# nubcico/EAV

Measured on AMD Instinct MI355X. Metric: EEGNet training samples/sec (fwd+CE+bwd+Adam), whole job, higher is better.
Workload: dtype f32; 1 GPU; EEGNet_tor(5, Chans=30, Samples=10000, kernLength=300, F1=8, D=8, F2=64) train step on x[64,1,30,10000] fp32 per GPU (BASELINE.json configs[1]); global_batch=64, per_gpu_batch=64, parallelism=dp1

## Files before the change

eav_amd/_lib.py:

```python
from __future__ import annotations

import ctypes as C
import os

_HERE = os.path.dirname(os.path.abspath(__file__))
LIB_PATH = os.environ.get("EAV_LIB_PATH") or os.path.join(_HERE, "libeav_hip.so")


class EavError(RuntimeError):
    pass


_p = C.c_void_p
_i = C.c_int
_i64 = C.c_int64
_u64 = C.c_uint64
_f = C.c_float
_d = C.c_double

SIGNATURES = {
    "eav_reduce_partials": [_p, _i, _i64, _i, _f, _p, _p],
    "eav_bn_finalize": [_p, _i, _i, _d, _p, _p, _p, _p, _i, _f, _f, _p, _p, _p, _p, _p],
    "eav_bn_bwd_finalize": [_p, _i, _i, _d, _i, _p, _p, _p, _p, _p],
    "eav_reduce_and_bn_bwd_finalize": [_p, _i, _i64, _i, _p, _p, _i, _i, _d, _i, _p, _p, _p, _p, _p, _i, _i, _d, _i, _p, _p, _p,
                                       _p, _p],
    "eav_renorm_rows": [_p, _i, _i, _f, _p],
    "eav_renorm_rows2": [_p, _i, _i, _p, _i, _i, _f, _p],
    "eav_eegnet_step_prologue": [_p, _p, _p, _p, _p, _p, _p, _p],
    "eav_eegnet_fir_fwd": [_p, _p, _p, _p, _i, _i, _i, _i, _p],
    "eav_eegnet_fir_wgrad": [_p, _p, _p, _p, _p, _i, _i, _i, _i, _p],
    "eav_eegnet_fir_fwd_indexed": [_p, _p, _p, _p, _p, _i, _i, _i, _i, _p],
    "eav_eegnet_fir_fwd_fft": [_p, _p, _p, _p, _p, _i, _i, _i, _i, _p],
    "eav_eegnet_fir_wgrad_fft": [_p, _p, _p, _p, _p, _p, _p, _i, _i, _i, _i, _p],
    "eav_eegnet_fir_wgrad_indexed": [_p, _p, _p, _p, _p, _p, _i, _i, _i, _i, _p],
    "eav_eegnet_dw_fwd": [_p, _p, _p, _p, _p, _i, _i, _i, _p],
    "eav_eegnet_dw_fwd_pool_eval": [_p, _p, _p, _p, _p, _p, _p, _i, _i, _i, _p],
    "eav_eegnet_dw_bwd": [_p, _p, _p, _p, _p, _p, _p, _i, _i, _i, _p],
    "eav_eegnet_dw_bwd_fused": [_p, _p, _p, _p, _p, _p, _p, _p, _p, _i, _i, _i, _f, _u64, _p, _p, _p],
    "eav_eegnet_dw_bwd_fused_eval": [_p, _p, _p, _p, _p, _p, _p, _p, _p, _p, _i, _i, _i, _f, _u64, _p, _p, _p],
    "eav_bn_elu_pool_fwd": [_p, _p, _p, _i, _i, _i, _i, _f, _u64, _p, _p, _p],
    "eav_bn_elu_pool_bwd_reduce": [_p, _p, _p, _p, _i, _i, _i, _i, _f, _u64, _p, _p, _p],
    "eav_bn_elu_pool_bwd_apply": [_p, _p, _p, _p, _p, _i, _i, _i, _i, _f, _u64, _p, _p, _p],
    "eav_bn_elu_pool_bwd_eval": [_p, _p, _p, _p, _p, _i, _i, _i, _i, _f, _u64, _p, _p, _p],
    "eav_conv64_prep_weights": [_p, _p, _p, _p],
    "eav_conv64_fwd": [_p, _p, _p, _p, _i, _i, _i, _p],
    "eav_conv64_wgrad": [_p, _p, _p, _i, _i, _i, _p],
    "eav_conv64_fft_fwd": [_p, _p, _p, _p, _p, _i, _i, _i, _p],
    "eav_conv64_fft_wgrad": [_p, _p, _p, _i, _i, _p],
    "eav_dense_softmax_fwd": [_p, _p, _p, _p, _p, _i, _i, _i, _p],
    "eav_dense_softmax_bwd": [_p, _p, _p, _p, _p, _p, _p, _i, _i, _i, _p],
    "eav_ce_fwd_bwd": [_p, _p, _p, _p, _p, _p, _i, _i, _p],
    "eav_scale_by_scalar": [_p, _p, _i64, _p],
    "eav_adam_step": [_p, _p, _p, _p, _i64, _f, _f, _f, _f, _f, _i64, _i, _p, _p],
    "eav_counter_inc": [_p, _p],
    "eav_counter_inc4": [_p, _p, _p, _p, _p],
    "eav_step_begin": [_p, _p, _p, _p, _p, _p, _p, _p, _i, _p],
    "eav_gather_rows": [_p, _p, _p, _i, _i64, _p],
    "eav_gather_i64": [_p, _p, _p, _i, _p],
    "eav_gemm_f32": [_p, _p, _p, _i, _i, _i, _i, _i, _i, _i, _i, _i, _i, _i64, _i64, _i64, _i64, _i64, _i64, _f, _p,
                     _i, _p, _p, _i, _i, _p],
    "eav_gemm_f32_splitk": [_p, _p, _p, _p, _i, _i, _i, _i, _i, _i, _i, _p],
    "eav_sp_absmax": [_p, _i, _i, _i64, _p, _p],
    "eav_sp_convert": [_p, _i, _i, _i64, _p, _p, _p, _p],
    "eav_sp_convert_gelu": [_p, _i, _i, _i64, _p, _p, _p, _p],
    "eav_sp_convert_colsum": [_p, _i, _i, _i64, _p, _p, _p, _p, _p],
    "eav_layernorm_fwd_amax": [_p, _p, _p, _p, _p, _p, _i, _i, _f, _p, _p],
    "eav_layernorm_bwd_amax": [_p, _p, _p, _p, _p, _p, _i, _p, _i, _i, _p, _p],
    "eav_layernorm_bwd_planes": [_p, _p, _p, _p, _p, _p, _i, _p, _i, _i, _p, _p, _p, _p, _p, _p],
    "eav_layernorm_bwd_bound": [_p, _p, _p, _p, _p, _i, _i, _p, _p],
    "eav_gelu_bwd_amax": [_p, _p, _i64, _p, _p],
    "eav_gemm_sp": [_p, _p, _p, _p, _p, _i, _i, _i, _i, _i, _i64, _i64, _f, _p, _i, _p, _p, _i, _i, _p, _p],
    "eav_gemm_sp_x1": [_p, _p, _p, _p, _p, _i, _i, _i, _i, _i, _i64, _i64, _f, _p, _i, _p, _p, _i, _i, _p, _p],
    "eav_gemm_sp_splitk_x1": [_p, _p, _p, _p, _p, _p, _i, _i, _i, _i, _p],
    "eav_gemm_sp_splitk_x2": [_p, _p, _p, _p, _p, _p, _i, _i, _i, _i, _p],
    "eav_gemm_sp_ex": [_p, _p, _p, _p, _p, _i, _i, _i, _i, _i, _i64, _i64, _f, _p, _i, _p, _p, _i, _i, _p, _p, _p, _p, _i, _p],
    "eav_colnorm_max": [_p, _i, _i, _i64, _p, _p],
    "eav_norm_max_multi": [_p, _i, _i, _p],
    "eav_sp_bound_scale": [_p, _p, _p, _f, _p],
    "eav_gemm_sp_planes": [_p, _p, _p, _p, _p, _i, _i, _i, _i, _i, _i64, _i64, _f, _p, _i, _p, _p, _i, _i, _p, _p, _p, _p],
    "eav_layernorm_fwd_planes": [_p, _p, _p, _p, _p, _p, _p, _p, _i, _i, _f, _p],
    "eav_sp_refresh_planes": [_p, _i, _i, _i, _p],
    "eav_rownorm_max": [_p, _i, _i, _i64, _p, _p],
    "eav_tf_forward_scales": [_p, _i64, _i, _i, _i, _i, _i, _i, _i, _i, _p, _p, _i64, _i, _i, _i, _p],
    "eav_gemm_sp_splitk": [_p, _p, _p, _p, _p, _p, _i, _i, _i, _i, _p],
    "eav_attn_sp_prep": [_p, _p, _p, _p, _i, _i, _i, _i, C.c_uint, _p],
    "eav_attn_fwd_sp": [_p, _p, _p, _p, _p, _p, _i, _i, _i, _i, _f, _p],
    "eav_tf_forward_scales_qkv": [_p, _i64, _i, _i, _i, _i, _i, _i, _i, _i, _i, _p, _p, _p, _i64, _i, _i, _i, _i, _p],
    "eav_attn_fwd_sp_planes": [_p, _p, _p, _p, _p, _p, _p, _p, _i, _i, _i, _i, _f, _p],
    "eav_attn_bwd_sp": [_p, _p, _p, _p, _p, _p, _p, _p, _p, _p, _p, _p, _p, _i, _i, _i, _i, _f, _p],
    "eav_attn_bwd_sp_planes": [_p, _p, _p, _p, _p, _p, _p, _p, _p, _p, _p, _p, _p, _p, _p, _p, _p, _p, _i, _i, _i, _i, _f, _p],
    "eav_attn_dqkv_bound": [_p, _p, _p, _i, _f, _p],
    "eav_attn_fwd": [_p, _p, _p, _i, _i, _i, _i, _f, _p],
    "eav_attn_bwd": [_p, _p, _p, _p, _p, _p, _i, _i, _i, _i, _f, _p],
    "eav_attn_fwd_dropout": [_p, _p, _p, _i, _i, _i, _i, _f, _f, _u64, _p, _p, _p],
    "eav_attn_bwd_dropout": [_p, _p, _p, _p, _p, _p, _i, _i, _i, _i, _f, _f, _u64, _p, _p, _p],
    "eav_attn_fwd_sp_dropout": [_p, _p, _p, _p, _p, _i, _i, _i, _i, _f, _f, _u64, _p, _p, _p],
    "eav_attn_bwd_sp_dropout": [_p, _p, _p, _p, _p, _p, _p, _p, _p, _p, _p, _i, _i, _i, _i, _f, _f, _u64, _p, _p, _p],
    "eav_tf_dropout_mask": [_p, _i64, _f, _u64, _p, _p],
    "eav_tf_dropout_add": [_p, _p, _p, _i64, _f, _u64, _p, _p, _p],
    "eav_softmax_dropout_fwd": [_p, _p, _i64, _i, _i, _f, _u64, _p, _p, _p],
    "eav_softmax_dropout_bwd": [_p, _p, _p, _i64, _i, _i, _f, _u64, _p, _p, _p],
    "eav_layernorm_fwd": [_p, _p, _p, _p, _p, _p, _i, _i, _f, _p],
    "eav_layernorm_bwd": [_p, _p, _p, _p, _p, _p, _i, _p, _i, _i, _p],
    "eav_softmax_fwd": [_p, _i64, _i, _i, _p],
    "eav_softmax_bwd": [_p, _p, _i64, _i, _i, _p],
    "eav_gelu_bwd": [_p, _p, _i64, _p],
    "eav_colsum": [_p, _p, _i, _i, _i, _p],
    "eav_im2col": [_p, _p, _i, _i, _i, _i, _i, _i, _i, _i, _p],
    "eav_embed_finish": [_p, _p, _p, _p, _i, _i, _i, _i, _p],
    "eav_embed_bwd": [_p, _p, _p, _i, _i, _i, _i, _p],
    "eav_token_rows": [_p, _p, _i, _i, _i, _i, _i, _p],
    "eav_pair_mean": [_p, _p, _i, _i, _i, _p],
    "eav_ast_fbank": [_p, _p, _p, _p, _p, _i, _i, _i, _i, _d, _d, _f, _f, _p],
    "eav_decimate_fir_f64": [_p, _p, _p, _i, _i64, _i64, _i, _i, _i, _p],
    "eav_sosfilt_f64": [_p, _p, _p, _p, _p, _p, _p, _i, _i64, _i, _i, _p],
    "eav_eegnet_block1_infer": [_p, _p, _p, _p, _p, _p, _p, _i, _i, _i, _i, _p],
    "eav_tconv_fwd": [_p, _p, _p, _p, _i, _i, _i, _i, _i, _p],
    "eav_tconv_wgrad": [_p, _p, _p, _p, _p, _i, _i, _i, _i, _i, _p],
    "eav_spatial_fwd": [_p, _p, _p, _p, _p, _i, _i, _i, _i, _i, _i, _p],
    "eav_spatial_bwd": [_p, _p, _p, _p, _p, _p, _p, _i, _i, _i, _i, _i, _i, _p],
    "eav_dconv_fwd": [_p, _p, _p, _p, _i, _i, _i, _i, _i, _i, _p],
    "eav_dconv_wgrad": [_p, _p, _p, _i, _i, _i, _i, _i, _p],
    "eav_sepconv_fwd": [_p, _p, _p, _p, _p, _p, _i, _i, _i, _i, _i, _p],
    "eav_pointwise_bwd": [_p, _p, _p, _p, _p, _i, _i, _i, _i, _p],
    "eav_dwt_bwd": [_p, _p, _p, _p, _p, _i, _i, _i, _i, _p],
    "eav_shallow_embed_fwd": [_p, _p, _p, _i, _p, _p, _i, _i, _i, _i, _i, _p],
    "eav_shallow_embed_bwd": [_p, _p, _p, _p, _p, _p, _i, _i, _i, _i, _i, _p],
    "eav_relu_dropout": [_p, _i64, _f, _u64, _p, _p, _p],
    "eav_relu_dropout_bwd": [_p, _p, _i64, _f, _p],
    "eav_dropout_add": [_p, _p, _p, _i64, _f, _u64, _p, _p, _p],
    "eav_add_strided": [_p, _i, _p, _i, _p, _i, _i64, _i, _p],
    "eav_colstats": [_p, _p, _i64, _i, _i, _p],
    "eav_sqpool_log_fwd": [_p, _p, _p, _p, _i, _i, _i, _i, _i, _i, _f, _f, _f, _u64, _p, _p, _p],
    "eav_sqpool_log_bwd": [_p, _p, _p, _p, _p, _p, _i, _i, _i, _i, _i, _i, _f, _f, _f, _u64, _p, _p, _p],
    "eav_bn_rows_bwd": [_p, _p, _p, _p, _i64, _i, _p],
    "eav_peak_mfma_f32": [_p, _i, _i, _p],
    "eav_peak_copy": [_p, _p, _i64, _p],
    "eav_peak_mfma_f16": [_p, _i, _i, _p],
    "eav_peak_copy_variant": [_p, _p, _i64, _i, _i, _p],
    "eav_peak_l2_read": [_p, _i, _i, _i, _i, _p, _p],
    "eav_resize_normalize_u8": [_p, _p, _p, _p, _p, _p, _i, _i, _i, _i, _i, _i, _i, _i, _d, _p, _p, _p],
    "eav_audio_conv5_fwd": [_p, _p, _p, _p, _p, _i, _i, _i, _i, _i, _i, _f, _u64, _p, _p, _p],
    "eav_audio_conv5_dgrad": [_p, _p, _f, _p, _p, _p, _p, _f, _i, _i, _i, _i, _i, _i, _p],
    "eav_audio_conv5_wgrad": [_p, _p, _f, _p, _p, _i, _i, _i, _i, _i, _i, _p],
    "eav_video_conv_relayout": [_p, _p, _p, _i, _i, _i, _p],
    "eav_video_conv_fwd": [_p, _p, _p, _i, _i, _i, _i, _i, _i, _i, _i, _i, _i, _i, _i, _p],
    "eav_video_conv_dgrad": [_p, _p, _p, _p, _i, _i, _i, _i, _i, _i, _i, _i, _i, _i, _i, _p],
    "eav_video_conv_wgrad": [_p, _p, _p, _i, _i, _i, _i, _i, _i, _i, _i, _i, _i, _i, _i, _i, _p],
    "eav_video_bn_stats": [_p, _p, _i64, _i, _p],
    "eav_video_bn_apply": [_p, _p, _p, _p, _p, _p, _p, _i64, _i, _i, _p],
    "eav_video_bn_bwd": [_p, _p, _p, _p, _p, _p, _i64, _i, _p],
    "eav_video_maxpool_fwd": [_p, _p, _p, _i, _i, _i, _i, _i, _i, _i, _i, _i, _p],
    "eav_video_maxpool_bwd": [_p, _p, _p, _i, _i, _i, _i, _i, _i, _i, _i, _i, _p],
    "eav_video_head_pool": [_p, _p, _p, _i, _i, _i, _p],
    "eav_video_head_scale_pool": [_p, _p, _p, _p, _i, _i, _i, _p],
    "eav_video_head_attn_bwd": [_p, _p, _p, _i, _i, _i, _p],
    "eav_video_head_feat_bwd": [_p, _p, _p, _p, _p, _i, _i, _i, _p],
    "eav_video_counters_inc": [_p, _i, _p],
}
PLAIN = {
    "eav_abi_version": ([], _i),
    "eav_last_error": ([], C.c_char_p),
    "eav_eegnet_fir_fwd_nparts": ([_i, _i, _i], _i),
    "eav_eegnet_fir_fwd_fft_nparts": ([_i, _i, _i], _i),
    "eav_eegnet_fir_wgrad_fft_ws_floats": ([_i, _i, _i], _i64),
    "eav_eegnet_fir_fft_max_taps": ([], _i),
    "eav_eegnet_fir_wgrad_nparts": ([_i, _i, _i], _i),
    "eav_conv64_ntiles": ([_i], _i),
    "eav_tconv_fwd_nparts": ([_i, _i, _i, _i, _i], _i),
    "eav_shallow_embed_nparts": ([_i, _i], _i),
    "eav_colstats_nparts": ([_i64], _i),
    "eav_tconv_wgrad_nparts": ([_i, _i, _i, _i, _i], _i),
    "eav_spatial_nparts": ([_i, _i], _i),
    "eav_dconv_fwd_nparts": ([_i, _i], _i),
    "eav_sepconv_fwd_nparts": ([_i, _i], _i),
    "eav_pointwise_bwd_nparts": ([_i, _i], _i),
    "eav_conv64_fwd_nparts": ([_i, _i], _i),
    "eav_conv64_fft_nparts": ([_i, _i], _i),
    "eav_conv64_fft_ws_floats": ([_i, _i], _i64),
    "eav_conv64_wgrad_nparts": ([_i, _i], _i),
    "eav_layernorm_bwd_nparts": ([_i], _i),
    "eav_gemm_f32_splitk_plan": ([_i, _i, _i], _i),
    "eav_colsum_nparts": ([_i], _i),
    "eav_sp_kpad": ([_i], _i),
    "eav_sp_convert_colsum_nparts": ([_i], _i),
    "eav_attn_sp_npad": ([_i], _i),
    "eav_gemm_sp_splitk_plan": ([_i, _i, _i], _i),
    "eav_audio_wgrad_nparts": ([_i, _i, _i, _i], _i),
    "eav_video_wgrad_nparts": ([_i, _i, _i, _i64], _i),
    "eav_video_bn_nparts": ([_i64], _i),
}

EXPORTS = sorted(list(SIGNATURES) + list(PLAIN))

TUNING = {"eav_gemm_sp_set_tile": [_i], "eav_gemm_sp_set_splitk": [_i], "eav_sp_set_convert_blocks": [_i],
          "eav_attn_sp_set_nw4_above": [_i]}

EXTRAS_PATH = os.path.join(_HERE, "libeav_extras.so")
EXTRAS = {
    "eav_gemm_bf16": [_p, _p, _p, _i, _i, _i, _i, _i, _i, _i, _i, _i, _i, _i64, _i64, _i64, _i64, _i64, _i64, _f, _p,
                      _i, _p, _p, _i, _i, _p],
    "eav_gemm_bf16_splitk": [_p, _p, _p, _p, _i, _i, _i, _i, _i, _i, _i, _p],
}
_extras = None

_lib = None


def load():
    global _lib
    if _lib is not None:
        return _lib
    if not os.path.exists(LIB_PATH):
        raise EavError(
            f"{LIB_PATH} is missing - the HIP extension is not built. Run "
            "`python -c 'import __graft_entry__ as g; g.build()'` (or `make -C eav_amd/csrc`). "
            "There is no CPU fallback.")
    import torch
    lib = C.CDLL(LIB_PATH)
    for name, args in SIGNATURES.items():
        fn = getattr(lib, name)
        fn.argtypes = args
        fn.restype = _i
    for name, (args, res) in PLAIN.items():
        fn = getattr(lib, name)
        fn.argtypes = args
        fn.restype = res
    for name, args in TUNING.items():
        fn = getattr(lib, name)
        fn.argtypes = args
        fn.restype = _i
    _lib = lib
    return lib


def ptr(t):
    return None if t is None else t.data_ptr()


def stream_ptr():
    import torch
    return torch.cuda.current_stream().cuda_stream


def have_extras():
    return os.path.exists(EXTRAS_PATH)


def load_extras():
    global _extras
    if _extras is None:
        if not have_extras():
            raise EavError(f"{EXTRAS_PATH} is missing - {sorted(EXTRAS)} are comparison-only kernels: build them with "
                           "`make -C eav_amd/csrc BENCH_EXTRAS=1`")
        load()
        lib = C.CDLL(EXTRAS_PATH)
        for name, args in EXTRAS.items():
            fn = getattr(lib, name)
            fn.argtypes = args
            fn.restype = _i
        lib.eav_last_error.restype = C.c_char_p
        _extras = lib
    return _extras


TRACE = None


def call(name, *args):
    lib = load_extras() if name in EXTRAS else load()
    if TRACE is not None:
        import torch
        a, b = torch.cuda.Event(enable_timing=True), torch.cuda.Event(enable_timing=True)
        a.record()
        rc = getattr(lib, name)(*args)
        b.record()
        TRACE.setdefault(name, []).append((a, b))
    else:
        rc = getattr(lib, name)(*args)
    if rc != 0:
        raise EavError(f"{name} failed ({rc}): {lib.eav_last_error().decode()}")


def plain(name, *args):
    return getattr(load(), name)(*args)
```

eav_amd/csrc/eav_common.hip:

```cpp
#include "eav_common.h"

#include <stdarg.h>
#include <stdio.h>

#include "../../include/eav_hip.h"

static thread_local char g_err[512] = "";

int eav_set_error(int code, const char* fmt, ...) {
  va_list ap;
  va_start(ap, fmt);
  vsnprintf(g_err, sizeof(g_err), fmt, ap);
  va_end(ap);
  return code;
}

extern "C" const char* eav_last_error(void) { return g_err; }
extern "C" int eav_abi_version(void) { return EAV_ABI_VERSION; }

__global__ __launch_bounds__(256) void reduce_partials_kernel(const float* __restrict__ part, int nparts,
                                                              int64_t stride, int n, float scale,
                                                              float* __restrict__ out) {
  __shared__ double sh[16][17];
  const int ol = threadIdx.x & 15, pl = threadIdx.x >> 4;
  const int i = blockIdx.x * 16 + ol;
  double s = 0.0;
  if (i < n) {
    const float* src = part + i;
    int p = pl;
    for (; p + 48 < nparts; p += 64) {
      float a = src[(int64_t)p * stride], b = src[(int64_t)(p + 16) * stride];
      float c = src[(int64_t)(p + 32) * stride], d = src[(int64_t)(p + 48) * stride];
      s += ((double)a + (double)b) + ((double)c + (double)d);
    }
    for (; p < nparts; p += 16) s += (double)src[(int64_t)p * stride];
  }
  sh[pl][ol] = s;
  __syncthreads();
  if (threadIdx.x < 16 && i < n) {
    double t = 0.0;
#pragma unroll
    for (int k = 0; k < 16; ++k) t += sh[k][threadIdx.x];
    out[i] = (float)(t * (double)scale);
  }
}

template <int CL>
__device__ __forceinline__ void reduce_partials_vec_body(const float* __restrict__ part, int nparts, int64_t stride, int n4,
                                                         float scale, float* __restrict__ out, int bid) {
  constexpr int PL = 256 / CL;
  __shared__ double sh[PL][4 * CL + 1];
  const int cl = threadIdx.x % CL, pl = threadIdx.x / CL;
  const int c4 = bid * CL + cl;
  double a = 0.0, b = 0.0, c = 0.0, d = 0.0;
  if (c4 < n4) {
    const float* src = part + 4 * (int64_t)c4;
    int p = pl;
    for (; p + 3 * PL < nparts; p += 4 * PL) {
      const float4 v0 = *reinterpret_cast<const float4*>(src + (int64_t)p * stride);
      const float4 v1 = *reinterpret_cast<const float4*>(src + (int64_t)(p + PL) * stride);
      const float4 v2 = *reinterpret_cast<const float4*>(src + (int64_t)(p + 2 * PL) * stride);
      const float4 v3 = *reinterpret_cast<const float4*>(src + (int64_t)(p + 3 * PL) * stride);
      a += ((double)v0.x + (double)v1.x) + ((double)v2.x + (double)v3.x);
      b += ((double)v0.y + (double)v1.y) + ((double)v2.y + (double)v3.y);
      c += ((double)v0.z + (double)v1.z) + ((double)v2.z + (double)v3.z);
      d += ((double)v0.w + (double)v1.w) + ((double)v2.w + (double)v3.w);
    }
    for (; p < nparts; p += PL) {
      const float4 v = *reinterpret_cast<const float4*>(src + (int64_t)p * stride);
      a += (double)v.x; b += (double)v.y; c += (double)v.z; d += (double)v.w;
    }
  }
  sh[pl][4 * cl] = a; sh[pl][4 * cl + 1] = b; sh[pl][4 * cl + 2] = c; sh[pl][4 * cl + 3] = d;
  __syncthreads();
  if (threadIdx.x < 4 * CL && 4 * bid * CL + threadIdx.x < 4 * n4) {
    double t = 0.0;
#pragma unroll
    for (int k = 0; k < PL; ++k) t += sh[k][threadIdx.x];
    out[4 * (int64_t)bid * CL + threadIdx.x] = (float)(t * (double)scale);
  }
}

template <int CL>
__global__ __launch_bounds__(256) void reduce_partials_vec_kernel(const float* __restrict__ part, int nparts,
                                                                  int64_t stride, int n4, float scale,
                                                                  float* __restrict__ out) {
  reduce_partials_vec_body<CL>(part, nparts, stride, n4, scale, out, blockIdx.x);
}

extern "C" int eav_reduce_partials(const float* part, int nparts, int64_t stride, int n, float scale, float* out,
                                   void* stream) {
  EAV_REQUIRE(part && out && nparts > 0 && n > 0, "eav_reduce_partials: bad arguments");
  const bool vec = (n & 3) == 0 && (stride & 3) == 0 && (((uintptr_t)part | (uintptr_t)out) & 15) == 0;
  if (vec && n >= 8192)
    hipLaunchKernelGGL(reduce_partials_vec_kernel<16>, dim3(cdiv(n / 4, 16)), dim3(256), 0, (hipStream_t)stream, part,
                       nparts, stride, n / 4, scale, out);
  else if (vec)
    hipLaunchKernelGGL(reduce_partials_vec_kernel<8>, dim3(cdiv(n / 4, 8)), dim3(256), 0, (hipStream_t)stream, part,
                       nparts, stride, n / 4, scale, out);
  else
    hipLaunchKernelGGL(reduce_partials_kernel, dim3(cdiv(n, 16)), dim3(256), 0, (hipStream_t)stream, part, nparts,
                       stride, n, scale, out);
  EAV_CHECK_LAUNCH("eav_reduce_partials");
  return EAV_OK;
}

__global__ void bn_finalize_kernel(const float* __restrict__ part, int nparts, int nch, double count,
                                   const float* __restrict__ gamma, const float* __restrict__ beta,
                                   float* __restrict__ rmean, float* __restrict__ rvar, int training, float momentum,
                                   float eps, float* __restrict__ mean_o, float* __restrict__ invstd_o,
                                   float* __restrict__ scale_o, float* __restrict__ shift_o) {
  const int c = blockIdx.x;
  __shared__ double shs[256], shq[256];
  float mean, var;
  if (training) {
    double s = 0.0, q = 0.0;
    for (int p = threadIdx.x; p < nparts; p += 256) {
      s += (double)part[(int64_t)p * 2 * nch + c];
      q += (double)part[(int64_t)p * 2 * nch + nch + c];
    }
    shs[threadIdx.x] = s;
    shq[threadIdx.x] = q;
    __syncthreads();
    for (int o = 128; o > 0; o >>= 1) {
      if (threadIdx.x < o) {
        shs[threadIdx.x] += shs[threadIdx.x + o];
        shq[threadIdx.x] += shq[threadIdx.x + o];
      }
      __syncthreads();
    }
    if (threadIdx.x != 0) return;
    s = shs[0];
    q = shq[0];
    double m = s / count;
    double v = q / count - m * m;
    if (v < 0.0) v = 0.0;
    mean = (float)m;
    var = (float)v;
    double unb = count > 1.0 ? v * (count / (count - 1.0)) : v;
    rmean[c] = (1.f - momentum) * rmean[c] + momentum * mean;
    rvar[c] = (1.f - momentum) * rvar[c] + momentum * (float)unb;
  } else {
    if (threadIdx.x != 0) return;
    mean = rmean[c];
    var = rvar[c];
  }
  float invstd = 1.0f / sqrtf(var + eps);
  float sc = gamma[c] * invstd;
  mean_o[c] = mean;
  invstd_o[c] = invstd;
  scale_o[c] = sc;
  shift_o[c] = beta[c] - mean * sc;
}

extern "C" int eav_bn_finalize(const float* part, int nparts, int nch, double count, const float* gamma,
                               const float* beta, float* running_mean, float* running_var, int training,
                               float momentum, float eps, float* mean, float* invstd, float* scale, float* shift,
                               void* stream) {
  EAV_REQUIRE(nch > 0 && gamma && beta && running_mean && running_var && mean && invstd && scale && shift,
              "eav_bn_finalize: bad arguments");
  EAV_REQUIRE(!training || (part && nparts > 0 && count > 0), "eav_bn_finalize: training needs partials");
  hipLaunchKernelGGL(bn_finalize_kernel, dim3(nch), dim3(256), 0, (hipStream_t)stream, part, nparts, nch,
                     count, gamma, beta, running_mean, running_var, training, momentum, eps, mean, invstd, scale,
                     shift);
  EAV_CHECK_LAUNCH("eav_bn_finalize");
  return EAV_OK;
}

__device__ __forceinline__ void bn_bwd_finalize_body(const float* __restrict__ part, int nparts, int nch, double count,
                                                     int training, float* __restrict__ dgamma, float* __restrict__ dbeta,
                                                     float* __restrict__ m1, float* __restrict__ m2, int c) {
  __shared__ double shs[256], shq[256];
  double s = 0.0, q = 0.0;
  for (int p = threadIdx.x; p < nparts; p += 256) {
    s += (double)part[(int64_t)p * 2 * nch + c];
    q += (double)part[(int64_t)p * 2 * nch + nch + c];
  }
  shs[threadIdx.x] = s;
  shq[threadIdx.x] = q;
  __syncthreads();
  for (int o = 128; o > 0; o >>= 1) {
    if (threadIdx.x < o) {
      shs[threadIdx.x] += shs[threadIdx.x + o];
      shq[threadIdx.x] += shq[threadIdx.x + o];
    }
    __syncthreads();
  }
  if (threadIdx.x != 0) return;
  s = shs[0];
  q = shq[0];
  dbeta[c] = (float)s;
  dgamma[c] = (float)q;
  m1[c] = training ? (float)(s / count) : 0.f;
  m2[c] = training ? (float)(q / count) : 0.f;
}

__global__ void bn_bwd_finalize_kernel(const float* __restrict__ part, int nparts, int nch, double count,
                                       int training, float* __restrict__ dgamma, float* __restrict__ dbeta,
                                       float* __restrict__ m1, float* __restrict__ m2) {
  bn_bwd_finalize_body(part, nparts, nch, count, training, dgamma, dbeta, m1, m2, blockIdx.x);
}

struct BnBwdJob {
  const float* part;
  int nparts, nch, training;
  double count;
  float *dgamma, *dbeta, *m1, *m2;
};

__global__ __launch_bounds__(256) void finish_jobs_kernel(const float* __restrict__ part, int nparts, int64_t stride, int n4,
                                                          float scale, float* __restrict__ out, int nred, BnBwdJob a,
                                                          BnBwdJob b) {
  const int bid = blockIdx.x;
  if (bid < nred) {
    reduce_partials_vec_body<8>(part, nparts, stride, n4, scale, out, bid);
    return;
  }
  const int c = bid - nred;
  const BnBwdJob& j = c < a.nch ? a : b;
  bn_bwd_finalize_body(j.part, j.nparts, j.nch, j.count, j.training, j.dgamma, j.dbeta, j.m1, j.m2, c < a.nch ? c : c - a.nch);
}

extern "C" int eav_reduce_and_bn_bwd_finalize(const float* part, int nparts, int64_t stride, int n, float* out,
                                              const float* part_a, int nparts_a, int nch_a, double count_a, int training_a,
                                              float* dgamma_a, float* dbeta_a, float* m1_a, float* m2_a,
                                              const float* part_b, int nparts_b, int nch_b, double count_b, int training_b,
                                              float* dgamma_b, float* dbeta_b, float* m1_b, float* m2_b, void* stream) {
  EAV_REQUIRE(part && out && nparts > 0 && n > 0, "eav_reduce_and_bn_bwd_finalize: bad reduction arguments");
  EAV_REQUIRE(part_a && nparts_a > 0 && nch_a > 0 && count_a > 0 && dgamma_a && dbeta_a && m1_a && m2_a,
              "eav_reduce_and_bn_bwd_finalize: bad BatchNorm arguments");
  EAV_REQUIRE(!part_b || (nparts_b > 0 && nch_b > 0 && count_b > 0 && dgamma_b && dbeta_b && m1_b && m2_b),
              "eav_reduce_and_bn_bwd_finalize: bad second BatchNorm arguments");
  const bool vec8 = (n & 3) == 0 && (stride & 3) == 0 && (((uintptr_t)part | (uintptr_t)out) & 15) == 0 && n < 8192;
  if (!vec8) {
    int rc = eav_reduce_partials(part, nparts, stride, n, 1.f, out, stream);
    if (rc == EAV_OK)
      rc = eav_bn_bwd_finalize(part_a, nparts_a, nch_a, count_a, training_a, dgamma_a, dbeta_a, m1_a, m2_a, stream);
    if (rc == EAV_OK && part_b)
      rc = eav_bn_bwd_finalize(part_b, nparts_b, nch_b, count_b, training_b, dgamma_b, dbeta_b, m1_b, m2_b, stream);
    return rc;
  }
  BnBwdJob a{part_a, nparts_a, nch_a, training_a, count_a, dgamma_a, dbeta_a, m1_a, m2_a};
  BnBwdJob b{part_b, nparts_b, part_b ? nch_b : 0, training_b, count_b, dgamma_b, dbeta_b, m1_b, m2_b};
  const int nred = cdiv(n / 4, 8);
  hipLaunchKernelGGL(finish_jobs_kernel, dim3(nred + a.nch + b.nch), dim3(256), 0, (hipStream_t)stream, part, nparts, stride,
                     n / 4, 1.f, out, nred, a, b);
  EAV_CHECK_LAUNCH("eav_reduce_and_bn_bwd_finalize");
  return EAV_OK;
}

extern "C" int eav_bn_bwd_finalize(const float* part, int nparts, int nch, double count, int training,
                                   float* dgamma, float* dbeta, float* m1, float* m2, void* stream) {
  EAV_REQUIRE(part && nparts > 0 && nch > 0 && count > 0 && dgamma && dbeta && m1 && m2,
              "eav_bn_bwd_finalize: bad arguments");
  hipLaunchKernelGGL(bn_bwd_finalize_kernel, dim3(nch), dim3(256), 0, (hipStream_t)stream, part, nparts,
                     nch, count, training, dgamma, dbeta, m1, m2);
  EAV_CHECK_LAUNCH("eav_bn_bwd_finalize");
  return EAV_OK;
}

__global__ void renorm_rows_kernel(float* __restrict__ w, int rows, int cols, float maxnorm, float* __restrict__ w_b,
                                   int cols_b) {
  __shared__ float red[8];
  int r = blockIdx.x;
  if (r >= rows) {
    r -= rows;
    w = w_b;
    cols = cols_b;
  }
  float* row = w + (int64_t)r * cols;
  const bool vec = (cols & 3) == 0 && (reinterpret_cast<uintptr_t>(row) & 15) == 0;
  float v[1] = {0.f};
  if (vec) {
    const float4* row4 = reinterpret_cast<const float4*>(row);
    const int n4 = cols >> 2;
    float a[4] = {0.f, 0.f, 0.f, 0.f};
    for (int i0 = threadIdx.x; i0 < n4; i0 += 1024) {
      float4 q[4];
#pragma unroll
      for (int u = 0; u < 4; ++u) q[u] = i0 + 256 * u < n4 ? row4[i0 + 256 * u] : make_float4(0.f, 0.f, 0.f, 0.f);
#pragma unroll
      for (int u = 0; u < 4; ++u) a[u] += (q[u].x * q[u].x + q[u].y * q[u].y) + (q[u].z * q[u].z + q[u].w * q[u].w);
    }
    v[0] = (a[0] + a[1]) + (a[2] + a[3]);
  } else {
    for (int i = threadIdx.x; i < cols; i += 256) v[0] += row[i] * row[i];
  }
  block_sum_256<1>(v, red);
  __shared__ float sc;
  if (threadIdx.x == 0) {
    float norm = sqrtf(v[0]);
    sc = norm > maxnorm ? maxnorm / (norm + 1e-7f) : 1.f;
  }
  __syncthreads();
  float s = sc;
  if (s == 1.f) return;
  if (vec) {
    float4* row4 = reinterpret_cast<float4*>(row);
    const int n4 = cols >> 2;
    for (int i0 = threadIdx.x; i0 < n4; i0 += 1024) {
      float4 q[4];
#pragma unroll
      for (int u = 0; u < 4; ++u) q[u] = i0 + 256 * u < n4 ? row4[i0 + 256 * u] : make_float4(0.f, 0.f, 0.f, 0.f);
#pragma unroll
      for (int u = 0; u < 4; ++u)
        if (i0 + 256 * u < n4) row4[i0 + 256 * u] = make_float4(q[u].x * s, q[u].y * s, q[u].z * s, q[u].w * s);
    }
  } else {
    for (int i = threadIdx.x; i < cols; i += 256) row[i] *= s;
  }
}

extern "C" int eav_renorm_rows(float* w, int rows, int cols, float maxnorm, void* stream) {
  EAV_REQUIRE(w && rows > 0 && cols > 0, "eav_renorm_rows: bad arguments");
  hipLaunchKernelGGL(renorm_rows_kernel, dim3(rows), dim3(256), 0, (hipStream_t)stream, w, rows, cols, maxnorm,
                     (float*)nullptr, 0);
  EAV_CHECK_LAUNCH("eav_renorm_rows");
  return EAV_OK;
}

extern "C" int eav_renorm_rows2(float* w_a, int rows_a, int cols_a, float* w_b, int rows_b, int cols_b, float maxnorm,
                                void* stream) {
  EAV_REQUIRE(w_a && rows_a > 0 && cols_a > 0 && w_b && rows_b > 0 && cols_b > 0, "eav_renorm_rows2: bad arguments");
  hipLaunchKernelGGL(renorm_rows_kernel, dim3(rows_a + rows_b), dim3(256), 0, (hipStream_t)stream, w_a, rows_a, cols_a,
                     maxnorm, w_b, cols_b);
  EAV_CHECK_LAUNCH("eav_renorm_rows2");
  return EAV_OK;
}
```

eav_amd/csrc/eegnet_block.hip:

```cpp
#include "eav_common.h"
#include "../../include/eav_hip.h"

namespace {

constexpr int F1 = 8, DD = 8, CHMAX = 32;

__device__ __forceinline__ void ld4(const float* p, int i, int n, bool vec, float (&v)[4]) {
  if (vec && i + 3 < n) {
    float4 a = *reinterpret_cast<const float4*>(p + i);
    v[0] = a.x; v[1] = a.y; v[2] = a.z; v[3] = a.w;
  } else {
#pragma unroll
    for (int e = 0; e < 4; ++e) v[e] = (i + e < n) ? p[i + e] : 0.f;
  }
}
__device__ __forceinline__ void ld4s(const float* p, int i, int n, bool vec, float (&v)[4]) {
  if (vec && i + 3 < n) {
    const f32x4 a = __builtin_nontemporal_load(reinterpret_cast<const f32x4*>(p + i));
    v[0] = a[0]; v[1] = a[1]; v[2] = a[2]; v[3] = a[3];
  } else {
#pragma unroll
    for (int e = 0; e < 4; ++e) v[e] = (i + e < n) ? p[i + e] : 0.f;
  }
}
__device__ __forceinline__ void st4s(float* p, int i, int n, bool vec, const float (&v)[4]) {
  if (vec && i + 3 < n) {
    __builtin_nontemporal_store((f32x4){v[0], v[1], v[2], v[3]}, reinterpret_cast<f32x4*>(p + i));
  } else {
#pragma unroll
    for (int e = 0; e < 4; ++e)
      if (i + e < n) p[i + e] = v[e];
  }
}
__device__ __forceinline__ void st4(float* p, int i, int n, bool vec, const float (&v)[4]) {
  if (vec && i + 3 < n) {
    *reinterpret_cast<float4*>(p + i) = make_float4(v[0], v[1], v[2], v[3]);
  } else {
#pragma unroll
    for (int e = 0; e < 4; ++e)
      if (i + e < n) p[i + e] = v[e];
  }
}

template <int NT, int NV>
__device__ __forceinline__ void block_sum_nt(float (&v)[NV], float* red) {
  if constexpr (NT == 256) {
    block_sum_256<NV>(v, red);
  } else {
    const int lane = threadIdx.x & 63, wave = threadIdx.x >> 6;
#pragma unroll
    for (int k = 0; k < NV; ++k) {
      const float s = wave_sum(v[k]);
      if (lane == 0) red[wave * NV + k] = s;
    }
    __syncthreads();
    if ((int)threadIdx.x < NV) {
      float t = red[threadIdx.x];
#pragma unroll
      for (int w = 1; w < NT / 64; ++w) t += red[w * NV + threadIdx.x];
      v[0] = t;
    }
    __syncthreads();
  }
}

template <int CG, int NT>
__global__ __launch_bounds__(NT) void dw_fwd_kernel(const float* __restrict__ y1, const float* __restrict__ bn1,
                                                     const float* __restrict__ w2, float* __restrict__ z,
                                                     float* __restrict__ part, int C, int S,
                                                     const float* __restrict__ bn2, float* __restrict__ p2) {
  __shared__ float wsh[DD * CHMAX];
  __shared__ float red[NT / 64 * 16];
  __shared__ float xsum[CG > 1 ? (CG - 1) * DD * 4 * (NT / CG) : 1];
  constexpr int TPG = NT / CG;
  const int chunk = blockIdx.x, f = blockIdx.y, b = blockIdx.z;
  const int cg = CG > 1 ? threadIdx.x / TPG : 0, tl = CG > 1 ? threadIdx.x % TPG : threadIdx.x;
  for (int i = threadIdx.x; i < DD * C; i += NT) wsh[i] = w2[f * DD * C + i];
  __syncthreads();
  const float sc = bn1[16 + f], sh = bn1[24 + f];
  const bool vec = (S & 3) == 0;
  const int t = chunk * (4 * TPG) + tl * 4;
  float acc[DD][4];
#pragma unroll
  for (int d = 0; d < DD; ++d)
#pragma unroll
    for (int e = 0; e < 4; ++e) acc[d][e] = 0.f;
  if (t < S) {
    const float* src = y1 + ((int64_t)b * F1 + f) * C * S;
    float nx[2][4];
    ld4s(src + (int64_t)(CG > 1 ? min(cg, C - 1) : 0) * S, t, S, vec, nx[0]);
    ld4s(src + (int64_t)min(cg + CG, C - 1) * S, t, S, vec, nx[1]);
    for (int c = cg; c < C; c += CG) {
      float v[4];
#pragma unroll
      for (int e = 0; e < 4; ++e) { v[e] = nx[0][e]; nx[0][e] = nx[1][e]; }
      ld4s(src + (int64_t)min(c + 2 * CG, C - 1) * S, t, S, vec, nx[1]);
#pragma unroll
      for (int e = 0; e < 4; ++e) v[e] = elu_f(sc * v[e] + sh);
#pragma unroll
      for (int d = 0; d < DD; ++d) {
        const float w = wsh[d * C + c];
#pragma unroll
        for (int e = 0; e < 4; ++e) acc[d][e] += w * v[e];
      }
    }
  }
  if (CG > 1) {
    if (cg > 0)
#pragma unroll
      for (int d = 0; d < DD; ++d)
#pragma unroll
        for (int e = 0; e < 4; ++e) xsum[(((cg - 1) * DD + d) * 4 + e) * TPG + tl] = acc[d][e];
    __syncthreads();
    if (cg == 0)
#pragma unroll
      for (int g = 1; g < CG; ++g)
#pragma unroll
        for (int d = 0; d < DD; ++d)
#pragma unroll
          for (int e = 0; e < 4; ++e) acc[d][e] += xsum[(((g - 1) * DD + d) * 4 + e) * TPG + tl];
  }
  const bool mine = CG == 1 || cg == 0;
  float st[16];
#pragma unroll
  for (int d = 0; d < DD; ++d) {
    float s = 0.f, q = 0.f;
#pragma unroll
    for (int e = 0; e < 4; ++e) {
      float v = (mine && t + e < S) ? acc[d][e] : 0.f;
      s += v;
      q += v * v;
    }
    st[d] = s;
    st[8 + d] = q;
    if (mine && t < S) st4s(z + ((int64_t)b * F1 * DD + f * DD + d) * S, t, S, vec, acc[d]);
    if (p2 && mine && t + 3 < S) {
      const int ch = f * DD + d, CH = F1 * DD;
      const float sc2 = bn2[2 * CH + ch], sh2 = bn2[3 * CH + ch];
      float ps = 0.f;
#pragma unroll
      for (int e = 0; e < 4; ++e) ps += elu_f(sc2 * acc[d][e] + sh2);
      p2[((int64_t)b * CH + ch) * (S / 4) + t / 4] = ps * 0.25f;
    }
  }
  block_sum_nt<NT, 16>(st, red);
  if (threadIdx.x < 16) {
    const int nch = F1 * DD;
    float* dst = part + ((int64_t)b * gridDim.x + chunk) * 2 * nch;
    const int d = threadIdx.x & 7;
    dst[(threadIdx.x < 8 ? 0 : nch) + f * DD + d] = st[0];
  }
}

template <int P>
__global__ __launch_bounds__(256) void pool_fwd_kernel(const float* __restrict__ in, const float* __restrict__ bn,
                                                       float* __restrict__ out, int CH, int T, float drop_p,
                                                       uint64_t seed_in,
    const uint8_t* __restrict__ mask, const uint64_t* __restrict__ seed_dev) {
  const uint64_t seed = dropout_seed(seed_in, seed_dev);
  const int row = blockIdx.x, ch = row % CH;
  const float sc = bn[2 * CH + ch], sh = bn[3 * CH + ch];
  const int To = T / P;
  const float* src = in + (int64_t)row * T;
  const bool vec = (T & 3) == 0;
  for (int to = threadIdx.x; to < To; to += 256) {
    float s = 0.f;
#pragma unroll
    for (int j = 0; j < P; j += 4) {
      float v[4];
      ld4(src, to * P + j, T, vec, v);
#pragma unroll
      for (int e = 0; e < 4; ++e) s += elu_f(sc * v[e] + sh);
    }
    const uint64_t oi = (uint64_t)row * To + to;
    out[oi] = s * (1.0f / P) * dropout_mult_row(drop_p, seed, mask, oi, (uint64_t)row);
  }
}

template <int P>
__global__ __launch_bounds__(256) void pool_bwd_reduce_kernel(const float* __restrict__ dp,
                                                              const float* __restrict__ u,
                                                              const float* __restrict__ bn, float* __restrict__ part,
                                                              int CH, int T, float drop_p, uint64_t seed_in,
    const uint8_t* __restrict__ mask, const uint64_t* __restrict__ seed_dev) {
  const uint64_t seed = dropout_seed(seed_in, seed_dev);
  __shared__ float red[8];
  const int row = blockIdx.x, ch = row % CH, b = row / CH;
  const float mean = bn[ch], invstd = bn[CH + ch], sc = bn[2 * CH + ch], sh = bn[3 * CH + ch];
  const int To = T / P;
  const float* src = u + (int64_t)row * T;
  const bool vec = (T & 3) == 0;
  float st[2] = {0.f, 0.f};
  for (int to = threadIdx.x; to < To; to += 256) {
    const uint64_t oi = (uint64_t)row * To + to;
    const float go = dp[oi] * (1.0f / P) * dropout_mult_row(drop_p, seed, mask, oi, (uint64_t)row);
#pragma unroll
    for (int j = 0; j < P; j += 4) {
      float v[4];
      ld4(src, to * P + j, T, vec, v);
#pragma unroll
      for (int e = 0; e < 4; ++e) {
        const float pre = sc * v[e] + sh;
        const float g = go * elu_grad_from_out(pre, elu_f(pre));
        st[0] += g;
        st[1] += g * ((v[e] - mean) * invstd);
      }
    }
  }
  block_sum_256<2>(st, red);
  if (threadIdx.x < 2) part[(int64_t)b * 2 * CH + threadIdx.x * CH + ch] = st[0];
}

template <int P>
__global__ __launch_bounds__(256) void pool_bwd_apply_kernel(const float* __restrict__ dp,
                                                             const float* __restrict__ u,
                                                             const float* __restrict__ bn,
                                                             const float* __restrict__ m12, float* __restrict__ du,
                                                             int CH, int T, float drop_p, uint64_t seed_in,
    const uint8_t* __restrict__ mask, const uint64_t* __restrict__ seed_dev, float* __restrict__ part) {
  const uint64_t seed = dropout_seed(seed_in, seed_dev);
  __shared__ float red[8];
  const int row = blockIdx.x, ch = row % CH;
  const float mean = bn[ch], invstd = bn[CH + ch], sc = bn[2 * CH + ch], sh = bn[3 * CH + ch];
  const float m1 = m12 ? m12[ch] : 0.f, m2 = m12 ? m12[CH + ch] : 0.f;
  float st[2] = {0.f, 0.f};
  const int To = T / P;
  const float* src = u + (int64_t)row * T;
  float* dst = du + (int64_t)row * T;
  const bool vec = (T & 3) == 0;
  for (int q = threadIdx.x; q < (T + 3) / 4; q += 256) {
    const int t = 4 * q;
    const int to = t / P;
    float go = 0.f;
    if (to < To) {
      const uint64_t oi = (uint64_t)row * To + to;
      go = dp[oi] * (1.0f / P) * dropout_mult_row(drop_p, seed, mask, oi, (uint64_t)row);
    }
    float v[4], o[4];
    ld4(src, t, T, vec, v);
#pragma unroll
    for (int e = 0; e < 4; ++e) {
      const float pre = sc * v[e] + sh;
      const float g = go * elu_grad_from_out(pre, elu_f(pre));
      o[e] = sc * (g - m1 - (v[e] - mean) * invstd * m2);
      if (t + e < T) {
        st[0] += g;
        st[1] += g * ((v[e] - mean) * invstd);
      }
    }
    st4(dst, t, T, vec, o);
  }
  if (part) {
    block_sum_256<2>(st, red);
    if (threadIdx.x < 2) part[(int64_t)(row / CH) * 2 * CH + threadIdx.x * CH + ch] = st[0];
  }
}

template <int CTRL, int BANK_MASK>
__device__ __forceinline__ float dpp_f(float old, float src) {
  return __int_as_float(__builtin_amdgcn_update_dpp(__float_as_int(old), __float_as_int(src), CTRL, 0xf, BANK_MASK, false));
}

template <int CTRL, int ROW_MASK, bool BOUND>
__device__ __forceinline__ float dpp_row(float src) {
  return __int_as_float(__builtin_amdgcn_update_dpp(0, __float_as_int(src), CTRL, ROW_MASK, 0xf, BOUND));
}
__device__ __forceinline__ float wave_total_dpp(float a) {
  a += dpp_row<0x111, 0xf, true>(a);
  a += dpp_row<0x112, 0xf, true>(a);
  a += dpp_row<0x114, 0xf, true>(a);
  a += dpp_row<0x118, 0xf, true>(a);
  a += dpp_row<0x142, 0xa, false>(a);
  a += dpp_row<0x143, 0xc, false>(a);
  return __int_as_float(__builtin_amdgcn_readlane(__float_as_int(a), 63));
}

struct DwFuse {
  const float* z; const float* dp2; const float* bn2;
  float drop_p; uint64_t seed; const uint8_t* mask; const uint64_t* seed_dev;
  float* part2;
};

#ifndef DWB_WPE
#define DWB_WPE 0
#endif
#ifndef DWB_PF
#define DWB_PF 2
#endif
template <bool FUSED, int CG, int NT, bool SUMS2 = false>
__global__ __launch_bounds__(NT, DWB_WPE) void dw_bwd_kernel(const float* __restrict__ y1, const float* __restrict__ dz,
                                                     const float* __restrict__ bn1, const float* __restrict__ w2,
                                                     float* __restrict__ g1, float* __restrict__ part_st,
                                                     float* __restrict__ part_w, int C, int S, DwFuse fu) {
  __shared__ float wsh[DD * CHMAX];
  __shared__ float red[NT / 64 * 8];
  __shared__ float red2[SUMS2 ? NT / 64 * 2 * DD : 1];
  __shared__ float wacc[NT / 64 * DD * CHMAX];
  constexpr int TPG = NT / CG;
#ifdef DWB_ASC
  const int chunk = blockIdx.x, f = blockIdx.y, b = blockIdx.z;
#else
  const int chunk = blockIdx.x, f = blockIdx.y, b = gridDim.z - 1 - blockIdx.z;
#endif
  const int lane = threadIdx.x & 63, wave = threadIdx.x >> 6;
  const int cg = CG > 1 ? threadIdx.x / TPG : 0, tl = CG > 1 ? threadIdx.x % TPG : threadIdx.x;
  for (int i = threadIdx.x; i < DD * C; i += NT) wsh[i] = w2[f * DD * C + i];
  if (CG > 1)
    for (int i = threadIdx.x; i < NT / 64 * DD * CHMAX; i += NT) wacc[i] = 0.f;
  __syncthreads();
  const float mean = bn1[f], invstd = bn1[8 + f], sc = bn1[16 + f], sh = bn1[24 + f];
  const bool vec = (S & 3) == 0;
  const int t = chunk * (4 * TPG) + tl * 4;
  float dzv[DD][4];
  if (FUSED) {
    float st2[2 * DD];
#pragma unroll
    for (int k = 0; k < 2 * DD; ++k) st2[k] = 0.f;
    const uint64_t seed = dropout_seed(fu.seed, fu.seed_dev);
    const int To = S / 4, to = t / 4;
#pragma unroll
    for (int d = 0; d < DD; ++d) {
      const int ch = f * DD + d, CH = F1 * DD;
      const int64_t row = (int64_t)b * CH + ch;
      const float mean2 = fu.bn2[ch], invstd2 = fu.bn2[CH + ch], sc2 = fu.bn2[2 * CH + ch], sh2 = fu.bn2[3 * CH + ch];
      const float m1 = SUMS2 ? 0.f : fu.bn2[4 * CH + ch], m2 = SUMS2 ? 0.f : fu.bn2[5 * CH + ch];
      float go = 0.f;
      if (to < To) {
        const uint64_t oi = (uint64_t)row * To + to;
        go = fu.dp2[oi] * 0.25f * dropout_mult_row(fu.drop_p, seed, fu.mask, oi, (uint64_t)row);
      }
      float v[4];
      ld4s(fu.z + row * S, t < S ? t : S, S, vec, v);
#pragma unroll
      for (int e = 0; e < 4; ++e) {
        const float pre = sc2 * v[e] + sh2;
        const float g = go * elu_grad_from_out(pre, elu_f(pre));
        dzv[d][e] = (t + e < S) ? sc2 * (g - m1 - (v[e] - mean2) * invstd2 * m2) : 0.f;
        if (SUMS2 && t + e < S) {
          st2[d] += g;
          st2[DD + d] += g * ((v[e] - mean2) * invstd2);
        }
      }
    }
    if constexpr (SUMS2) {
#pragma unroll
      for (int k = 0; k < 2 * DD; ++k) {
        const float tot = wave_total_dpp(st2[k]);
        if (lane == 0) red2[wave * 2 * DD + k] = tot;
      }
    }
  } else {
#pragma unroll
    for (int d = 0; d < DD; ++d) ld4(dz + ((int64_t)b * F1 * DD + f * DD + d) * S, t < S ? t : S, S, vec, dzv[d]);
  }
  float st[2] = {0.f, 0.f};
  const int64_t base = ((int64_t)b * F1 + f) * C * S;
  constexpr int PF = DWB_PF;
  float nx[PF][4];
#pragma unroll
  for (int q = 0; q < PF; ++q)
    ld4s(y1 + base + (int64_t)min(cg + q * CG, C - 1) * S, t < S ? t : S, S, vec, nx[q]);
  for (int c = cg; c < C; c += CG) {
    float v[4], g[4], a[4];
#pragma unroll
    for (int e = 0; e < 4; ++e) {
      v[e] = nx[0][e];
#pragma unroll
      for (int q = 0; q + 1 < PF; ++q) nx[q][e] = nx[q + 1][e];
    }
    ld4s(y1 + base + (int64_t)min(c + PF * CG, C - 1) * S, t < S ? t : S, S, vec, nx[PF - 1]);
    float wd[DD];
#pragma unroll
    for (int d = 0; d < DD; ++d) wd[d] = wsh[d * C + c];
#pragma unroll
    for (int e = 0; e < 4; ++e) {
      const float pre = sc * v[e] + sh;
      a[e] = elu_f(pre);
      float da = 0.f;
#pragma unroll
      for (int d = 0; d < DD; ++d) da += wd[d] * dzv[d][e];
      g[e] = da * elu_grad_from_out(pre, a[e]);
      st[0] += g[e];
      st[1] += g[e] * ((v[e] - mean) * invstd);
    }
    if (t < S) st4s(g1 + base + (int64_t)c * S, t, S, vec, g);
    float r[DD];
#pragma unroll
    for (int d = 0; d < DD; ++d)
      r[d] = __builtin_fmaf(dzv[d][0], a[0], dzv[d][1] * a[1]) + __builtin_fmaf(dzv[d][2], a[2], dzv[d][3] * a[3]);
    float r4[4], r2[2], r1;
#ifdef DWB_ABL_NORED
    r1 = r[0] + r[1] + r[2] + r[3] + r[4] + r[5] + r[6] + r[7];
#else
    {
      const bool hi = lane & 1;
#pragma unroll
      for (int k = 0; k < 4; ++k) {
        float mine = hi ? r[4 + k] : r[k], other = hi ? r[k] : r[4 + k];
        r4[k] = mine + dpp_f<0xB1, 0xf>(0.f, other);
      }
    }
    {
      const bool hi = lane & 2;
#pragma unroll
      for (int k = 0; k < 2; ++k) {
        float mine = hi ? r4[2 + k] : r4[k], other = hi ? r4[k] : r4[2 + k];
        r2[k] = mine + dpp_f<0x4E, 0xf>(0.f, other);
      }
    }
    {
      const bool hi = lane & 4;
      float mine = hi ? r2[1] : r2[0], other = hi ? r2[0] : r2[1];
      float part = dpp_f<0x104, 0x5>(0.f, other);
      part = dpp_f<0x114, 0xA>(part, other);
      r1 = mine + part;
    }
    r1 += dpp_f<0x128, 0xf>(0.f, r1);
    {
      auto q = __builtin_amdgcn_permlane16_swap(__float_as_uint(r1), __float_as_uint(r1), false, false);
      r1 = __uint_as_float(q[0]) + __uint_as_float(q[1]);
      auto h = __builtin_amdgcn_permlane32_swap(__float_as_uint(r1), __float_as_uint(r1), false, false);
      r1 = __uint_as_float(h[0]) + __uint_as_float(h[1]);
    }
#endif
    if (lane < 8) {
      const int d = 4 * (lane & 1) + 2 * ((lane >> 1) & 1) + ((lane >> 2) & 1);
      wacc[wave * DD * CHMAX + d * C + c] = r1;
    }
  }
  block_sum_nt<NT, 2>(st, red);
  if (threadIdx.x < 2) part_st[((int64_t)b * gridDim.x + chunk) * 16 + threadIdx.x * 8 + f] = st[0];
  __syncthreads();
  if (FUSED && SUMS2 && threadIdx.x < 2 * DD) {
    constexpr int NWG = NT / 64 / CG;
    float t = red2[threadIdx.x];
#pragma unroll
    for (int w = 1; w < NWG; ++w) t += red2[w * 2 * DD + threadIdx.x];
    const int nch = F1 * DD;
    float* dst2 = fu.part2 + ((int64_t)b * gridDim.x + chunk) * 2 * nch;
    dst2[(threadIdx.x < DD ? 0 : nch) + f * DD + (threadIdx.x & (DD - 1))] = t;
  }
  float* dst = part_w + ((int64_t)b * gridDim.x + chunk) * (F1 * DD * C) + f * DD * C;
  for (int i = threadIdx.x; i < DD * C; i += NT) {
    float w = (wacc[i] + wacc[DD * CHMAX + i]) + (wacc[2 * DD * CHMAX + i] + wacc[3 * DD * CHMAX + i]);
    if constexpr (NT == 512)
      w += (wacc[4 * DD * CHMAX + i] + wacc[5 * DD * CHMAX + i]) + (wacc[6 * DD * CHMAX + i] + wacc[7 * DD * CHMAX + i]);
    dst[i] = w;
  }
}

}

static int dw_fwd_launch(const float* y1, const float* bn1, const float* w2, float* z, float* stat_part, int B, int C,
                         int S, const float* bn2, float* p2, void* stream) {
  dim3 grid(cdiv(S, 1024), F1, B);
  if (S <= 256)
    hipLaunchKernelGGL((dw_fwd_kernel<4, 256>), grid, dim3(256), 0, (hipStream_t)stream, y1, bn1, w2, z, stat_part, C, S,
                       bn2, p2);
  else if (S <= 512)
    hipLaunchKernelGGL((dw_fwd_kernel<4, 512>), grid, dim3(512), 0, (hipStream_t)stream, y1, bn1, w2, z, stat_part, C, S,
                       bn2, p2);
  else
    hipLaunchKernelGGL((dw_fwd_kernel<1, 256>), grid, dim3(256), 0, (hipStream_t)stream, y1, bn1, w2, z, stat_part, C, S,
                       bn2, p2);
  return EAV_OK;
}

extern "C" int eav_eegnet_dw_fwd(const float* y1, const float* bn1, const float* w2, float* z, float* stat_part,
                                 int B, int C, int S, void* stream) {
  EAV_REQUIRE(y1 && bn1 && w2 && z && stat_part && B > 0 && C > 0 && C <= CHMAX && S > 0,
              "eav_eegnet_dw_fwd: bad arguments (Chans must be <= %d)", CHMAX);
  dw_fwd_launch(y1, bn1, w2, z, stat_part, B, C, S, nullptr, nullptr, stream);
  EAV_CHECK_LAUNCH("eav_eegnet_dw_fwd");
  return EAV_OK;
}

extern "C" int eav_eegnet_dw_fwd_pool_eval(const float* y1, const float* bn1, const float* w2, float* z, float* stat_part,
                                           const float* bn2, float* p2, int B, int C, int S, void* stream) {
  EAV_REQUIRE(y1 && bn1 && w2 && z && stat_part && bn2 && p2 && B > 0 && C > 0 && C <= CHMAX && S > 0 && (S & 3) == 0,
              "eav_eegnet_dw_fwd_pool_eval: bad arguments (Chans <= %d, Samples %% 4 == 0)", CHMAX);
  dw_fwd_launch(y1, bn1, w2, z, stat_part, B, C, S, bn2, p2, stream);
  EAV_CHECK_LAUNCH("eav_eegnet_dw_fwd_pool_eval");
  return EAV_OK;
}

extern "C" int eav_eegnet_dw_bwd(const float* y1, const float* dz, const float* bn1, const float* w2, float* g1,
                                 float* stat_part, float* w_part, int B, int C, int S, void* stream) {
  EAV_REQUIRE(y1 && dz && bn1 && w2 && g1 && stat_part && w_part && B > 0 && C > 0 && C <= CHMAX && S > 0,
              "eav_eegnet_dw_bwd: bad arguments (Chans must be <= %d)", CHMAX);
  dim3 grid(cdiv(S, 1024), F1, B);
  hipLaunchKernelGGL((dw_bwd_kernel<false, 1, 256>), grid, dim3(256), 0, (hipStream_t)stream, y1, dz, bn1, w2, g1,
                     stat_part, w_part, C, S, DwFuse{});
  EAV_CHECK_LAUNCH("eav_eegnet_dw_bwd");
  return EAV_OK;
}

static int dw_bwd_fused_launch(const char* name, const float* y1, const float* z, const float* dp2, const float* bn2,
                               const float* bn1, const float* w2, float* g1, float* stat_part, float* w_part, float* bn2_part,
                               int B, int C, int S, float drop_p, uint64_t seed, const uint8_t* mask,
                               const uint64_t* seed_dev, void* stream) {
  EAV_REQUIRE(y1 && z && dp2 && bn2 && bn1 && w2 && g1 && stat_part && w_part && B > 0 && C > 0 && C <= CHMAX && S >= 4,
              "%s: bad arguments (Chans must be <= %d)", name, CHMAX);
  EAV_REQUIRE(drop_p > -1.f && drop_p < 1.f, "%s: dropout %f outside (-1,1)", name, drop_p);
  dim3 grid(cdiv(S, 1024), F1, B);
  DwFuse fu{z, dp2, bn2, drop_p, seed, mask, seed_dev, bn2_part};
#define DWB_LAUNCH(CG, NT, SUMS)                                                                                        \
  hipLaunchKernelGGL((dw_bwd_kernel<true, CG, NT, SUMS>), grid, dim3(NT), 0, (hipStream_t)stream, y1, nullptr, bn1, w2, g1, \
                     stat_part, w_part, C, S, fu)
  if (bn2_part) {
    if (S <= 256) DWB_LAUNCH(4, 256, true);
    else if (S <= 512) DWB_LAUNCH(4, 512, true);
    else DWB_LAUNCH(1, 256, true);
  } else {
    if (S <= 256) DWB_LAUNCH(4, 256, false);
    else if (S <= 512) DWB_LAUNCH(4, 512, false);
    else DWB_LAUNCH(1, 256, false);
  }
#undef DWB_LAUNCH
  EAV_CHECK_LAUNCH(name);
  return EAV_OK;
}

extern "C" int eav_eegnet_dw_bwd_fused(const float* y1, const float* z, const float* dp2, const float* bn2,
                                       const float* bn1, const float* w2, float* g1, float* stat_part, float* w_part,
                                       int B, int C, int S, float drop_p, uint64_t seed, const uint8_t* mask,
                                       const uint64_t* seed_dev, void* stream) {
  return dw_bwd_fused_launch("eav_eegnet_dw_bwd_fused", y1, z, dp2, bn2, bn1, w2, g1, stat_part, w_part, nullptr, B, C, S,
                             drop_p, seed, mask, seed_dev, stream);
}

extern "C" int eav_eegnet_dw_bwd_fused_eval(const float* y1, const float* z, const float* dp2, const float* bn2,
                                            const float* bn1, const float* w2, float* g1, float* stat_part, float* w_part,
                                            float* bn2_part, int B, int C, int S, float drop_p, uint64_t seed,
                                            const uint8_t* mask, const uint64_t* seed_dev, void* stream) {
  EAV_REQUIRE(bn2_part, "eav_eegnet_dw_bwd_fused_eval: bad arguments");
  return dw_bwd_fused_launch("eav_eegnet_dw_bwd_fused_eval", y1, z, dp2, bn2, bn1, w2, g1, stat_part, w_part, bn2_part, B, C,
                             S, drop_p, seed, mask, seed_dev, stream);
}

extern "C" int eav_bn_elu_pool_fwd(const float* in, const float* bn, float* out, int B, int CH, int T, int P,
                                   float drop_p, uint64_t seed, const uint8_t* mask, const uint64_t* seed_dev, void* stream) {
  EAV_REQUIRE(in && bn && out && B > 0 && CH > 0 && T >= P, "eav_bn_elu_pool_fwd: bad arguments");
  EAV_REQUIRE(P == 4 || P == 8, "eav_bn_elu_pool_fwd: pool %d not in {4,8}", P);
  EAV_REQUIRE(drop_p > -1.f && drop_p < 1.f, "eav_bn_elu_pool_fwd: dropout %f outside (-1,1)", drop_p);
  if (P == 4)
    hipLaunchKernelGGL(pool_fwd_kernel<4>, dim3(B * CH), dim3(256), 0, (hipStream_t)stream, in, bn, out, CH, T,
                       drop_p, seed, mask, seed_dev);
  else
    hipLaunchKernelGGL(pool_fwd_kernel<8>, dim3(B * CH), dim3(256), 0, (hipStream_t)stream, in, bn, out, CH, T,
                       drop_p, seed, mask, seed_dev);
  EAV_CHECK_LAUNCH("eav_bn_elu_pool_fwd");
  return EAV_OK;
}

extern "C" int eav_bn_elu_pool_bwd_reduce(const float* dp, const float* u, const float* bn, float* part, int B,
                                          int CH, int T, int P, float drop_p, uint64_t seed, const uint8_t* mask,
                                          const uint64_t* seed_dev, void* stream) {
  EAV_REQUIRE(dp && u && bn && part && B > 0 && CH > 0 && T >= P, "eav_bn_elu_pool_bwd_reduce: bad arguments");
  EAV_REQUIRE(P == 4 || P == 8, "eav_bn_elu_pool_bwd_reduce: pool %d not in {4,8}", P);
  if (P == 4)
    hipLaunchKernelGGL(pool_bwd_reduce_kernel<4>, dim3(B * CH), dim3(256), 0, (hipStream_t)stream, dp, u, bn, part,
                       CH, T, drop_p, seed, mask, seed_dev);
  else
    hipLaunchKernelGGL(pool_bwd_reduce_kernel<8>, dim3(B * CH), dim3(256), 0, (hipStream_t)stream, dp, u, bn, part,
                       CH, T, drop_p, seed, mask, seed_dev);
  EAV_CHECK_LAUNCH("eav_bn_elu_pool_bwd_reduce");
  return EAV_OK;
}

static int pool_bwd_apply_launch(const char* name, const float* dp, const float* u, const float* bn, const float* m12,
                                 float* du, float* part, int B, int CH, int T, int P, float drop_p, uint64_t seed,
                                 const uint8_t* mask, const uint64_t* seed_dev, void* stream) {
  EAV_REQUIRE(dp && u && bn && (m12 || part) && du && B > 0 && CH > 0 && T >= P, "%s: bad arguments", name);
  EAV_REQUIRE(P == 4 || P == 8, "%s: pool %d not in {4,8}", name, P);
  if (P == 4)
    hipLaunchKernelGGL(pool_bwd_apply_kernel<4>, dim3(B * CH), dim3(256), 0, (hipStream_t)stream, dp, u, bn, m12, du,
                       CH, T, drop_p, seed, mask, seed_dev, part);
  else
    hipLaunchKernelGGL(pool_bwd_apply_kernel<8>, dim3(B * CH), dim3(256), 0, (hipStream_t)stream, dp, u, bn, m12, du,
                       CH, T, drop_p, seed, mask, seed_dev, part);
  EAV_CHECK_LAUNCH(name);
  return EAV_OK;
}

extern "C" int eav_bn_elu_pool_bwd_apply(const float* dp, const float* u, const float* bn, const float* m12,
                                         float* du, int B, int CH, int T, int P, float drop_p, uint64_t seed,
                                         const uint8_t* mask, const uint64_t* seed_dev, void* stream) {
  EAV_REQUIRE(m12, "eav_bn_elu_pool_bwd_apply: bad arguments");
  return pool_bwd_apply_launch("eav_bn_elu_pool_bwd_apply", dp, u, bn, m12, du, nullptr, B, CH, T, P, drop_p, seed, mask,
                               seed_dev, stream);
}

extern "C" int eav_bn_elu_pool_bwd_eval(const float* dp, const float* u, const float* bn, float* du, float* part, int B,
                                        int CH, int T, int P, float drop_p, uint64_t seed, const uint8_t* mask,
                                        const uint64_t* seed_dev, void* stream) {
  EAV_REQUIRE(part, "eav_bn_elu_pool_bwd_eval: bad arguments");
  return pool_bwd_apply_launch("eav_bn_elu_pool_bwd_eval", dp, u, bn, nullptr, du, part, B, CH, T, P, drop_p, seed, mask,
                               seed_dev, stream);
}
```

eav_amd/csrc/eegnet_conv64_fft.hip:

```cpp
#include <algorithm>

#include "eav_common.h"
#include "../../include/eav_hip.h"

namespace {

constexpr int NCH = 64, KT = 16, NB = 64, LV = NB - KT + 1;
typedef float v2f __attribute__((ext_vector_type(2)));
constexpr float C64[50] = {1.0f, 0.995184727f, 0.98078528f, 0.956940336f, 0.923879533f, 0.881921264f, 0.831469612f, 0.773010453f, 0.707106781f, 0.634393284f, 0.555570233f, 0.471396737f, 0.382683432f, 0.290284677f, 0.195090322f, 0.0980171403f, 0.0f, -0.0980171403f, -0.195090322f, -0.290284677f, -0.382683432f, -0.471396737f, -0.555570233f, -0.634393284f, -0.707106781f, -0.773010453f, -0.831469612f, -0.881921264f, -0.923879533f, -0.956940336f, -0.98078528f, -0.995184727f, -1.0f, -0.995184727f, -0.98078528f, -0.956940336f, -0.923879533f, -0.881921264f, -0.831469612f, -0.773010453f, -0.707106781f, -0.634393284f, -0.555570233f, -0.471396737f, -0.382683432f, -0.290284677f, -0.195090322f, -0.0980171403f, 0.0f, 0.0980171403f};
constexpr float S64[50] = {0.0f, 0.0980171403f, 0.195090322f, 0.290284677f, 0.382683432f, 0.471396737f, 0.555570233f, 0.634393284f, 0.707106781f, 0.773010453f, 0.831469612f, 0.881921264f, 0.923879533f, 0.956940336f, 0.98078528f, 0.995184727f, 1.0f, 0.995184727f, 0.98078528f, 0.956940336f, 0.923879533f, 0.881921264f, 0.831469612f, 0.773010453f, 0.707106781f, 0.634393284f, 0.555570233f, 0.471396737f, 0.382683432f, 0.290284677f, 0.195090322f, 0.0980171403f, 0.0f, -0.0980171403f, -0.195090322f, -0.290284677f, -0.382683432f, -0.471396737f, -0.555570233f, -0.634393284f, -0.707106781f, -0.773010453f, -0.831469612f, -0.881921264f, -0.923879533f, -0.956940336f, -0.98078528f, -0.995184727f, -1.0f, -0.995184727f};

__device__ __forceinline__ v2f cmul(v2f a, v2f b) { return a.xx * b + a.yy * (v2f){-b.y, b.x}; }
__device__ __forceinline__ v2f cmulc(v2f a, v2f b) { return a.xx * (v2f){b.x, -b.y} + a.yy * (v2f){b.y, b.x}; }
template <bool INV>
__device__ __forceinline__ v2f twmul(v2f a, v2f w) { return INV ? cmulc(a, w) : cmul(a, w); }
template <bool INV>
__device__ __forceinline__ v2f rot(v2f a) { return INV ? (v2f){-a.y, a.x} : (v2f){a.y, -a.x}; }

template <bool INV>
__device__ __forceinline__ void dft4(v2f& a0, v2f& a1, v2f& a2, v2f& a3) {
  const v2f t0 = a0 + a2, t1 = a0 - a2, t2 = a1 + a3, t3 = rot<INV>(a1 - a3);
  a0 = t0 + t2; a1 = t1 + t3; a2 = t0 - t2; a3 = t1 - t3;
}

template <bool INV>
__device__ __forceinline__ void dft8(v2f& a0, v2f& a1, v2f& a2, v2f& a3, v2f& a4, v2f& a5, v2f& a6, v2f& a7) {
  constexpr float R = 0.70710678118654752f;
  dft4<INV>(a0, a2, a4, a6);
  dft4<INV>(a1, a3, a5, a7);
  const v2f t0 = a1, t1 = twmul<INV>(a3, (v2f){R, -R}), t2 = rot<INV>(a5), t3 = twmul<INV>(a7, (v2f){-R, -R});
  const v2f e0 = a0, e1 = a2, e2 = a4, e3 = a6;
  a0 = e0 + t0; a1 = e1 + t1; a2 = e2 + t2; a3 = e3 + t3;
  a4 = e0 - t0; a5 = e1 - t1; a6 = e2 - t2; a7 = e3 - t3;
}

__host__ __device__ constexpr int pos64(int k) { return 8 * (k & 7) + (k >> 3); }

template <bool INV>
__device__ __forceinline__ void fft64(v2f (&x)[64]) {
#pragma unroll
  for (int n2 = 0; n2 < 8; ++n2)
    dft8<INV>(x[n2], x[8 + n2], x[16 + n2], x[24 + n2], x[32 + n2], x[40 + n2], x[48 + n2], x[56 + n2]);
#pragma unroll
  for (int k1 = 1; k1 < 8; ++k1)
#pragma unroll
    for (int n2 = 1; n2 < 8; ++n2) x[8 * k1 + n2] = twmul<INV>(x[8 * k1 + n2], (v2f){C64[n2 * k1], -S64[n2 * k1]});
#pragma unroll
  for (int k1 = 0; k1 < 8; ++k1)
    dft8<INV>(x[8 * k1], x[8 * k1 + 1], x[8 * k1 + 2], x[8 * k1 + 3], x[8 * k1 + 4], x[8 * k1 + 5], x[8 * k1 + 6],
              x[8 * k1 + 7]);
}

struct Geo {
  int B, T, padl, nblk, npair, ncol, ncolp;
};

Geo geometry(int B, int T, int padl) {
  Geo g;
  g.B = B; g.T = T; g.padl = padl;
  g.nblk = cdiv(T, LV);
  g.npair = cdiv(g.nblk, 2);
  g.ncol = B * g.npair;
  g.ncolp = cdiv(g.ncol, 128) * 128;
  return g;
}

__global__ __launch_bounds__(64) void c64_spectra_kernel(const float* __restrict__ w, float* __restrict__ Bm0, int bwd0) {
  const int in = blockIdx.x, lane = threadIdx.x;
  const int bwd = bwd0 + blockIdx.y;
  float* Bm = Bm0 + (int64_t)blockIdx.y * 64 * 128 * 128;
  v2f x[64];
#pragma unroll
  for (int n = 0; n < 64; ++n) {
    float t = 0.f;
    if (n < KT) t = bwd ? w[((int64_t)in * NCH + lane) * KT + (KT - 1 - n)] : w[((int64_t)lane * NCH + in) * KT + n];
    x[n] = (v2f){t, 0.f};
  }
  fft64<false>(x);
#pragma unroll
  for (int m = 0; m < 64; ++m) {
    const v2f W = x[pos64(m)];
    const float gr = W.x * (1.0f / NB), gi = -W.y * (1.0f / NB);
    float* row0 = Bm + ((int64_t)m * 128 + in) * 128;
    float* row1 = Bm + ((int64_t)m * 128 + 64 + in) * 128;
    row0[lane] = gr;   row0[64 + lane] = gi;
    row1[lane] = -gi;  row1[64 + lane] = gr;
  }
}

constexpr int TS = 65;

__global__ __launch_bounds__(256) void c64_pack_fft_kernel(const float* __restrict__ in, float* __restrict__ Z, Geo g,
                                                           int vonly) {
  __shared__ float tiles[4][64 * TS];
  const int lane = threadIdx.x & 63, wave = threadIdx.x >> 6;
  float* tile = tiles[wave];
  const int nwaves = gridDim.x * 4;
  for (int col = blockIdx.x * 4 + wave; col < g.ncolp; col += nwaves) {
    if (col >= g.ncol) {
      float* dz = Z + (int64_t)col * 128 + lane;
#pragma unroll 8
      for (int m = 0; m < 64; ++m) {
        dz[(int64_t)m * g.ncolp * 128] = 0.f;
        dz[(int64_t)m * g.ncolp * 128 + 64] = 0.f;
      }
      continue;
    }
    const int b = col / g.npair, pr = col - b * g.npair;
    v2f x[64];
#pragma unroll
    for (int half = 0; half < 2; ++half) {
      const int blk = 2 * pr + half;
      const int t = blk * LV - (vonly ? 0 : g.padl) + lane;
      const bool ok = blk < g.nblk && t >= 0 && t < g.T && (!vonly || lane < LV);
      const float* src = in + (int64_t)b * NCH * g.T + t;
#pragma unroll
      for (int ch = 0; ch < NCH; ++ch) {
        const float v = ok ? src[(int64_t)ch * g.T] : 0.f;
        if (half == 0) x[ch].x = v; else x[ch].y = v;
      }
    }
#pragma unroll
    for (int half = 0; half < 2; ++half) {
#pragma unroll
      for (int ch = 0; ch < NCH; ++ch) tile[ch * TS + lane] = half == 0 ? x[ch].x : x[ch].y;
      asm volatile("s_waitcnt lgkmcnt(0)" ::: "memory");
      float r[64];
#pragma unroll
      for (int n = 0; n < 64; ++n) r[n] = tile[lane * TS + n];
      asm volatile("s_waitcnt lgkmcnt(0)" ::: "memory");
#pragma unroll
      for (int n = 0; n < 64; ++n) {
        if (half == 0) x[n].x = r[n]; else x[n].y = r[n];
      }
    }
    fft64<false>(x);
    float* dst = Z + (int64_t)col * 128 + lane;
#pragma unroll
    for (int m = 0; m < 64; ++m) {
      dst[(int64_t)m * g.ncolp * 128] = x[pos64(m)].x;
      dst[(int64_t)m * g.ncolp * 128 + 64] = x[pos64(m)].y;
    }
  }
}

constexpr int XS = 129;

#ifndef C64V_WPE
#define C64V_WPE 0
#endif
__global__ __launch_bounds__(256, C64V_WPE) void c64_bin_gemm_kernel(const float* __restrict__ Z, const float* __restrict__ Bm,
                                                           float* __restrict__ C, int ncolp) {
  __shared__ float xs[2][32 * XS];
  const int bin = blockIdx.y, lane = threadIdx.x & 63, wave = threadIdx.x >> 6;
  const int n = lane & 31, kk = lane >> 5;
  float wreg[64];
  {
    const float* bp = Bm + ((int64_t)bin * 128 + kk) * 128 + 32 * wave + n;
#pragma unroll
    for (int ks = 0; ks < 64; ++ks) wreg[ks] = bp[(int64_t)2 * ks * 128];
  }
  const int ntiles = ncolp >> 5;
  const float* zb = Z + (int64_t)bin * ncolp * 128;
  float* cb = C + (int64_t)bin * ncolp * 128;
  float4 pre[4];
  auto fetch = [&](int tile) {
    const float4* src = reinterpret_cast<const float4*>(zb + (int64_t)tile * 32 * 128);
#pragma unroll
    for (int i = 0; i < 4; ++i) pre[i] = src[threadIdx.x + 256 * i];
  };
  auto commit = [&](int buf) {
#pragma unroll
    for (int i = 0; i < 4; ++i) {
      const int idx4 = threadIdx.x + 256 * i, col = idx4 >> 5, k4 = idx4 & 31;
      float* d = xs[buf] + col * XS + 4 * k4;
      d[0] = pre[i].x; d[1] = pre[i].y; d[2] = pre[i].z; d[3] = pre[i].w;
    }
  };
  int tile = blockIdx.x, buf = 0;
  if (tile < ntiles) {
    fetch(tile);
    commit(0);
  }
  __syncthreads();
  for (; tile < ntiles; tile += gridDim.x) {
    const int nxt = tile + gridDim.x;
#ifndef C64V_ABL_NOFETCH
    if (nxt < ntiles) fetch(nxt);
#endif
    f32x16 acc;
#pragma unroll
    for (int r = 0; r < 16; ++r) acc[r] = 0.f;
    const float* ap = xs[buf] + n * XS + kk;
    float av[64];
#pragma unroll
#ifdef C64V_ABL_NOLDS
    for (int ks = 0; ks < 64; ++ks) av[ks] = 1.0f + ks;
#else
    for (int ks = 0; ks < 64; ++ks) av[ks] = ap[2 * ks];
#endif
    __builtin_amdgcn_sched_barrier(0);
    asm volatile("s_waitcnt lgkmcnt(0)" ::: "memory");
    __builtin_amdgcn_sched_barrier(0);
#pragma unroll
    for (int ks = 0; ks < 64; ++ks) acc = __builtin_amdgcn_mfma_f32_32x32x2f32(av[ks], wreg[ks], acc, 0, 0, 0);
    float* dst = cb + ((int64_t)tile * 32) * 128 + 32 * wave + n;
#ifdef C64V_ABL_NOSTORE
    if (acc[0] == 12345.f)
#endif
#pragma unroll
    for (int r = 0; r < 16; ++r) dst[(int64_t)((r & 3) + 8 * (r >> 2) + 4 * kk) * 128] = acc[r];
#ifndef C64V_ABL_NOFETCH
    if (nxt < ntiles) commit(buf ^ 1);
#endif
    asm volatile("s_waitcnt lgkmcnt(0)" ::: "memory");
    __builtin_amdgcn_s_barrier();
    buf ^= 1;
  }
}

__global__ __launch_bounds__(256) void c64_ifft_unpack_kernel(const float* __restrict__ Y, float* __restrict__ out,
                                                              float* __restrict__ part, Geo g) {
  __shared__ float tiles[4][64 * TS];
  const int lane = threadIdx.x & 63, wave = threadIdx.x >> 6;
  float* tile = tiles[wave];
  const int nwaves = gridDim.x * 4, wg = blockIdx.x * 4 + wave;
  float s1 = 0.f, s2 = 0.f;
  for (int col = wg; col < g.ncol; col += nwaves) {
    const int b = col / g.npair, pr = col - b * g.npair;
    v2f x[64];
    const float* src = Y + (int64_t)col * 128 + lane;
#pragma unroll
    for (int m = 0; m < 64; ++m) {
      x[m].x = src[(int64_t)m * g.ncolp * 128];
      x[m].y = src[(int64_t)m * g.ncolp * 128 + 64];
    }
    fft64<true>(x);
#pragma unroll
    for (int half = 0; half < 2; ++half) {
      const int blk = 2 * pr + half, t0 = blk * LV;
      if (blk >= g.nblk) break;
#pragma unroll
      for (int j = 0; j < LV; ++j) {
        const float v = half == 0 ? x[pos64(j)].x : x[pos64(j)].y;
        tile[lane * TS + j] = v;
        if (t0 + j < g.T) {
          s1 += v;
          s2 += v * v;
        }
      }
      asm volatile("s_waitcnt lgkmcnt(0)" ::: "memory");
      float* dst = out + (int64_t)b * NCH * g.T + t0 + lane;
      const bool ok = lane < LV && t0 + lane < g.T;
#pragma unroll 8
      for (int ch = 0; ch < NCH; ++ch) {
        const float v = tile[ch * TS + lane];
        if (ok) dst[(int64_t)ch * g.T] = v;
      }
      asm volatile("s_waitcnt lgkmcnt(0)" ::: "memory");
    }
  }
  if (part) {
    part[(int64_t)wg * 128 + lane] = s1;
    part[(int64_t)wg * 128 + 64 + lane] = s2;
  }
}


#ifndef C64V_WCH
#define C64V_WCH 4
#endif
#ifndef C64V_PF
#define C64V_PF 8
#endif
#ifndef C64V_GW
#define C64V_GW 8
#endif
constexpr int WCH = C64V_WCH;

__global__ __launch_bounds__(256) void c64_bin_wgemm_kernel(const float* __restrict__ D, const float* __restrict__ Z,
                                                            float* __restrict__ Pp, int ncolp, int cpc) {
  const int bin = blockIdx.y, chunk = blockIdx.x, lane = threadIdx.x & 63, wave = threadIdx.x >> 6;
  const int n = lane & 31, kk = lane >> 5;
  const int c0 = chunk * cpc;
  f32x16 acc[4];
#pragma unroll
  for (int j = 0; j < 4; ++j)
#pragma unroll
    for (int r = 0; r < 16; ++r) acc[j][r] = 0.f;
  const float* dp = D + ((int64_t)bin * ncolp + c0 + kk) * 128 + 32 * wave + n;
  const float* zp = Z + ((int64_t)bin * ncolp + c0 + kk) * 128 + n;
  const int nks = cpc >> 1;
  constexpr int PF = C64V_PF;
  float ra[PF], rb[PF][4];
#pragma unroll
  for (int p = 0; p < PF; ++p) {
    ra[p] = dp[(int64_t)p * 256];
#pragma unroll
    for (int j = 0; j < 4; ++j) rb[p][j] = zp[(int64_t)p * 256 + 32 * j];
  }
  for (int ks0 = 0; ks0 < nks; ks0 += PF) {
#pragma unroll
    for (int p = 0; p < PF; ++p) {
      const float a = ra[p];
      const float b0 = rb[p][0], b1 = rb[p][1], b2 = rb[p][2], b3 = rb[p][3];
#ifndef C64V_ABL_NOLOAD
      const int64_t o = (int64_t)min(ks0 + PF + p, nks - 1) * 256;
      ra[p] = dp[o];
      rb[p][0] = zp[o]; rb[p][1] = zp[o + 32]; rb[p][2] = zp[o + 64]; rb[p][3] = zp[o + 96];
#endif
      acc[0] = __builtin_amdgcn_mfma_f32_32x32x2f32(a, b0, acc[0], 0, 0, 0);
      acc[1] = __builtin_amdgcn_mfma_f32_32x32x2f32(a, b1, acc[1], 0, 0, 0);
      acc[2] = __builtin_amdgcn_mfma_f32_32x32x2f32(a, b2, acc[2], 0, 0, 0);
      acc[3] = __builtin_amdgcn_mfma_f32_32x32x2f32(a, b3, acc[3], 0, 0, 0);
    }
  }
  float* out = Pp + (((int64_t)chunk * 64 + bin) * 128 + 32 * wave) * 128 + n;
#pragma unroll
  for (int j = 0; j < 4; ++j)
#pragma unroll
    for (int r = 0; r < 16; ++r) out[(int64_t)((r & 3) + 8 * (r >> 2) + 4 * kk) * 128 + 32 * j] = acc[j][r];
}

__global__ __launch_bounds__(64) void c64_wsum_kernel(const float* __restrict__ Pp, float* __restrict__ Acc, int nchunk) {
  const int m = blockIdx.x, o = blockIdx.y, lane = threadIdx.x;
  float prr = 0.f, pii = 0.f, pri = 0.f, pir = 0.f;
  for (int c = 0; c < nchunk; ++c) {
    const float* p = Pp + (((int64_t)c * 64 + m) * 128) * 128;
    prr += p[(int64_t)o * 128 + lane];
    pri += p[(int64_t)o * 128 + 64 + lane];
    pir += p[(int64_t)(64 + o) * 128 + lane];
    pii += p[(int64_t)(64 + o) * 128 + 64 + lane];
  }
  *reinterpret_cast<v2f*>(Acc + 2 * (((int64_t)m * 64 + o) * 64 + lane)) = (v2f){prr + pii, pri - pir};
}

__global__ __launch_bounds__(64) void c64_wfinish_kernel(const float* __restrict__ Acc, float* __restrict__ dW) {
  const int o = blockIdx.x, lane = threadIdx.x;
  v2f x[64];
#pragma unroll
  for (int m = 0; m < 64; ++m) x[m] = *reinterpret_cast<const v2f*>(Acc + 2 * (((int64_t)m * 64 + o) * 64 + lane));
  fft64<true>(x);
#pragma unroll
  for (int k = 0; k < KT; ++k) dW[((int64_t)o * NCH + lane) * KT + k] = x[pos64(k)].x * (1.0f / NB);
}

int pack_grid(const Geo& g) { return std::max(1, std::min(512, cdiv(g.ncolp, 4))); }

}

extern "C" int64_t eav_conv64_fft_ws_floats(int B, int T) {
  const Geo g = geometry(B, T, 7);
  return (int64_t)2 * 64 * 128 * 128 + (int64_t)3 * 64 * g.ncolp * 128 + (int64_t)WCH * 64 * 128 * 128 +
         (int64_t)64 * 64 * 64 * 2;
}

extern "C" int eav_conv64_fft_nparts(int B, int T) {
  const Geo g = geometry(B, T, 7);
  return pack_grid(g) * 4;
}

extern "C" int eav_conv64_fft_fwd(const float* in, const float* w, float* out, float* stat_part, float* ws, int B, int T,
                                  int bwd, void* stream) {
  EAV_REQUIRE(in && w && out && ws && B > 0 && T > 0, "eav_conv64_fft_fwd: bad arguments");
  EAV_REQUIRE(((uintptr_t)ws & 15) == 0, "eav_conv64_fft_fwd: the workspace must be 16-byte aligned");
  const Geo g = geometry(B, T, bwd ? 8 : 7);
  EAV_REQUIRE(bwd >= 0 && bwd <= 2, "eav_conv64_fft_fwd: bwd must be 0, 1 or 2");
  hipStream_t st = (hipStream_t)stream;
  float* Bm = ws + (bwd ? (int64_t)64 * 128 * 128 : 0);
  const bool prepared = bwd == 2;
  if (bwd == 2) bwd = 1;
  float* Z = ws + (int64_t)2 * 64 * 128 * 128 + (bwd ? (int64_t)64 * g.ncolp * 128 : 0);
  float* Y = ws + (int64_t)2 * 64 * 128 * 128 + (int64_t)2 * 64 * g.ncolp * 128;
  if (!prepared) {
    hipLaunchKernelGGL(c64_spectra_kernel, dim3(NCH, bwd ? 1 : 2), dim3(64), 0, st, w, Bm, bwd);
    EAV_CHECK_LAUNCH("eav_conv64_fft_fwd(spectra)");
  }
  hipLaunchKernelGGL(c64_pack_fft_kernel, dim3(pack_grid(g)), dim3(256), 0, st, in, Z, g, 0);
  EAV_CHECK_LAUNCH("eav_conv64_fft_fwd(fft)");
  hipLaunchKernelGGL(c64_bin_gemm_kernel, dim3(std::min(C64V_GW, g.ncolp / 32), 64), dim3(256), 0, st, Z, Bm, Y, g.ncolp);
  EAV_CHECK_LAUNCH("eav_conv64_fft_fwd(gemm)");
  hipLaunchKernelGGL(c64_ifft_unpack_kernel, dim3(pack_grid(g)), dim3(256), 0, st, Y, out, stat_part, g);
  EAV_CHECK_LAUNCH("eav_conv64_fft_fwd(ifft)");
  return EAV_OK;
}

extern "C" int eav_conv64_fft_wgrad(const float* du, float* dW, float* ws, int B, int T, void* stream) {
  EAV_REQUIRE(du && dW && ws && B > 0 && T > 0, "eav_conv64_fft_wgrad: bad arguments");
  const Geo g = geometry(B, T, 7);
  hipStream_t st = (hipStream_t)stream;
  float* Z = ws + (int64_t)2 * 64 * 128 * 128;
  float* D = Z + (int64_t)2 * 64 * g.ncolp * 128;
  float* Pp = Z + (int64_t)3 * 64 * g.ncolp * 128;
  float* Acc = Pp + (int64_t)WCH * 64 * 128 * 128;
  hipLaunchKernelGGL(c64_pack_fft_kernel, dim3(pack_grid(g)), dim3(256), 0, st, du, D, g, 1);
  EAV_CHECK_LAUNCH("eav_conv64_fft_wgrad(fft)");
  const int cpc = g.ncolp / WCH;
  hipLaunchKernelGGL(c64_bin_wgemm_kernel, dim3(WCH, 64), dim3(256), 0, st, D, Z, Pp, g.ncolp, cpc);
  EAV_CHECK_LAUNCH("eav_conv64_fft_wgrad(gemm)");
  hipLaunchKernelGGL(c64_wsum_kernel, dim3(64, 64), dim3(64), 0, st, Pp, Acc, WCH);
  EAV_CHECK_LAUNCH("eav_conv64_fft_wgrad(sum)");
  hipLaunchKernelGGL(c64_wfinish_kernel, dim3(NCH), dim3(64), 0, st, Acc, dW);
  EAV_CHECK_LAUNCH("eav_conv64_fft_wgrad(finish)");
  return EAV_OK;
}
```

eav_amd/csrc/head_optim.hip:

```cpp
#include "eav_common.h"
#include "../../include/eav_hip.h"

namespace {

constexpr int NCMAX = 16;

__global__ __launch_bounds__(1024) void dense_softmax_fwd_kernel(const float* __restrict__ in,
                                                                 const float* __restrict__ w,
                                                                 const float* __restrict__ bias,
                                                                 float* __restrict__ logits, float* __restrict__ probs,
                                                                 int NF, int NC) {
  __shared__ float red[16 * NCMAX];
  const int b = blockIdx.x;
  const int lane = threadIdx.x & 63, wave = threadIdx.x >> 6;
  const float* src = in + (int64_t)b * NF;
  float acc[NCMAX];
#pragma unroll
  for (int j = 0; j < NCMAX; ++j) acc[j] = 0.f;
  if ((NF & 3) == 0) {
    const int nq = NF >> 2;
    if (NC <= 5) {
      for (int i0 = threadIdx.x; i0 < nq; i0 += 4096) {
        float4 v[4], wv[4][5];
#pragma unroll
        for (int u = 0; u < 4; ++u) {
          const int i = i0 + 1024 * u;
          const bool ok = i < nq;
          v[u] = ok ? reinterpret_cast<const float4*>(src)[i] : make_float4(0.f, 0.f, 0.f, 0.f);
#pragma unroll
          for (int j = 0; j < 5; ++j)
            wv[u][j] = (ok && j < NC) ? reinterpret_cast<const float4*>(w + (int64_t)j * NF)[i] : make_float4(0.f, 0.f, 0.f, 0.f);
        }
#pragma unroll
        for (int u = 0; u < 4; ++u)
#pragma unroll
          for (int j = 0; j < 5; ++j)
            acc[j] += (wv[u][j].x * v[u].x + wv[u][j].y * v[u].y) + (wv[u][j].z * v[u].z + wv[u][j].w * v[u].w);
      }
    } else {
      for (int i = threadIdx.x; i < nq; i += 1024) {
        const float4 v = reinterpret_cast<const float4*>(src)[i];
#pragma unroll
        for (int j = 0; j < NCMAX; ++j)
          if (j < NC) {
            const float4 wv = reinterpret_cast<const float4*>(w + (int64_t)j * NF)[i];
            acc[j] += (wv.x * v.x + wv.y * v.y) + (wv.z * v.z + wv.w * v.w);
          }
      }
    }
  } else {
    for (int i = threadIdx.x; i < NF; i += 1024) {
      const float v = src[i];
#pragma unroll
      for (int j = 0; j < NCMAX; ++j)
        if (j < NC) acc[j] += w[(int64_t)j * NF + i] * v;
    }
  }
#pragma unroll
  for (int j = 0; j < NCMAX; ++j)
    if (j < NC) {
      float s = wave_sum(acc[j]);
      if (lane == 0) red[wave * NCMAX + j] = s;
    }
  __syncthreads();
  __shared__ float lg[NCMAX];
  if (threadIdx.x < NC) {
    float s = 0.f;
#pragma unroll
    for (int k = 0; k < 16; ++k) s += red[k * NCMAX + threadIdx.x];
    lg[threadIdx.x] = s + bias[threadIdx.x];
  }
  __syncthreads();
  if (threadIdx.x == 0) {
    float mx = lg[0];
    for (int j = 1; j < NC; ++j) mx = fmaxf(mx, lg[j]);
    float e[NCMAX], s = 0.f;
    for (int j = 0; j < NC; ++j) { e[j] = expf(lg[j] - mx); s += e[j]; }
    for (int j = 0; j < NC; ++j) {
      if (logits) logits[b * NC + j] = lg[j];
      if (probs) probs[b * NC + j] = e[j] / s;
    }
  }
}

__global__ __launch_bounds__(256) void dense_softmax_bwd_kernel(const float* __restrict__ dout,
                                                                const float* __restrict__ probs,
                                                                const float* __restrict__ in,
                                                                const float* __restrict__ w, float* __restrict__ dw,
                                                                float* __restrict__ dbias, float* __restrict__ din,
                                                                int B, int NF, int NC) {
  extern __shared__ float dl[];
  float* pw = dl + B * NC;
  for (int idx = threadIdx.x; idx < B * NC; idx += blockDim.x) {
    const int b = idx / NC;
    float v = dout[idx];
    if (probs) {
      float dot = 0.f;
      for (int j = 0; j < NC; ++j) dot += dout[b * NC + j] * probs[b * NC + j];
      v = probs[idx] * (v - dot);
    }
    dl[idx] = v;
  }
  __syncthreads();
  if (blockIdx.x == 0 && threadIdx.x < NC) {
    float s = 0.f;
    for (int b = 0; b < B; ++b) s += dl[b * NC + threadIdx.x];
    dbias[threadIdx.x] = s;
  }
  const int f = threadIdx.x & 63, slice = threadIdx.x >> 6;
  const int i = blockIdx.x * 64 + f;
  const bool live = i < NF;
  float wv[NCMAX], acc[NCMAX];
#pragma unroll
  for (int j = 0; j < NCMAX; ++j) {
    wv[j] = (live && j < NC) ? w[(int64_t)j * NF + i] : 0.f;
    acc[j] = 0.f;
  }
  for (int b0 = slice; b0 < B; b0 += 32) {
    float v[8];
#pragma unroll
    for (int u = 0; u < 8; ++u) v[u] = (live && b0 + 4 * u < B) ? in[(int64_t)(b0 + 4 * u) * NF + i] : 0.f;
#pragma unroll
    for (int u = 0; u < 8; ++u) {
      const int b = b0 + 4 * u;
      if (b < B) {
        float d = 0.f;
#pragma unroll
        for (int j = 0; j < NCMAX; ++j)
          if (j < NC) {
            const float g = dl[b * NC + j];
            acc[j] += g * v[u];
            d += wv[j] * g;
          }
        if (din && live) din[(int64_t)b * NF + i] = d;
      }
    }
  }
#pragma unroll
  for (int j = 0; j < NCMAX; ++j) pw[(slice * NCMAX + j) * 64 + f] = acc[j];
  __syncthreads();
  if (slice == 0 && live) {
#pragma unroll
    for (int j = 0; j < NCMAX; ++j)
      if (j < NC)
        dw[(int64_t)j * NF + i] = (pw[j * 64 + f] + pw[(NCMAX + j) * 64 + f]) + (pw[(2 * NCMAX + j) * 64 + f] + pw[(3 * NCMAX + j) * 64 + f]);
  }
}

__global__ __launch_bounds__(256) void ce_kernel(const float* __restrict__ in, const int64_t* __restrict__ y,
                                                 float* __restrict__ loss, float* __restrict__ din,
                                                 int* __restrict__ ncorrect, int* __restrict__ bad_label, int B,
                                                 int NC) {
  __shared__ float red[12];
  float nv[1] = {0.f};
  for (int b = threadIdx.x; b < B; b += 256) {
    const int64_t yl = y[b];
    nv[0] += (yl >= 0 && yl < NC) ? 1.f : 0.f;
  }
  block_sum_256<1>(nv, red);
  if (threadIdx.x == 0) red[8] = nv[0];
  __syncthreads();
  const float nvalid = red[8];
  float st[2] = {0.f, 0.f};
  for (int b = threadIdx.x; b < B; b += 256) {
    const float* r = in + (int64_t)b * NC;
    float mx = r[0];
    int am = 0;
    for (int j = 1; j < NC; ++j)
      if (r[j] > mx) { mx = r[j]; am = j; }
    float s = 0.f;
    for (int j = 0; j < NC; ++j) s += expf(r[j] - mx);
    const float lse = mx + logf(s);
    const int64_t yl = y[b];
    const bool ok = yl >= 0 && yl < NC;
    if (!ok && yl != -100 && bad_label)
      *bad_label = yl >= 0 ? (int)min(yl, (int64_t)0x7ffffffe) + 1 : (int)max(yl, (int64_t)-0x7fffffff);
    const int yy = ok ? (int)yl : -1;
    st[0] += ok ? lse - r[yy] : 0.f;
    st[1] += (am == yy) ? 1.f : 0.f;
    if (din)
      for (int j = 0; j < NC; ++j)
        din[(int64_t)b * NC + j] = ok ? (expf(r[j] - lse) - (j == yy ? 1.f : 0.f)) / nvalid : 0.f;
  }
  block_sum_256<2>(st, red);
  if (threadIdx.x == 0 && loss) *loss = nvalid > 0.f ? st[0] / nvalid : __builtin_nanf("");
  if (threadIdx.x == 1 && ncorrect) *ncorrect += (int)(st[0] + 0.5f);
}

__global__ __launch_bounds__(256) void adam_kernel(float* __restrict__ p, const float* __restrict__ g,
                                                   float* __restrict__ m, float* __restrict__ v, int64_t n, float lr,
                                                   float b1, float b2, float eps, float wd, float bc1,
                                                   float bc2_sqrt, int decoupled,
                                                   const int64_t* __restrict__ step_dev) {
  if (step_dev) {
    const double st = (double)*step_dev;
    bc1 = (float)(1.0 - pow((double)b1, st));
    bc2_sqrt = (float)sqrt(1.0 - pow((double)b2, st));
  }
  const int64_t stride = (int64_t)gridDim.x * 256;
  for (int64_t i = (int64_t)blockIdx.x * 256 + threadIdx.x; i < n; i += stride) {
    float pv = p[i], gv = g[i];
    if (wd != 0.f) {
      if (decoupled) pv *= 1.f - lr * wd; else gv += wd * pv;
    }
    const float mv = b1 * m[i] + (1.f - b1) * gv;
    const float vv = b2 * v[i] + (1.f - b2) * gv * gv;
    m[i] = mv;
    v[i] = vv;
    const float denom = sqrtf(vv) / bc2_sqrt + eps;
    p[i] = pv - (lr / bc1) * (mv / denom);
  }
}

}

extern "C" int eav_dense_softmax_fwd(const float* in, const float* w, const float* bias, float* logits, float* probs,
                                     int B, int NF, int NC, void* stream) {
  EAV_REQUIRE(in && w && bias && (logits || probs) && B > 0 && NF > 0 && NC > 0 && NC <= NCMAX,
              "eav_dense_softmax_fwd: bad arguments (classes <= %d)", NCMAX);
  hipLaunchKernelGGL(dense_softmax_fwd_kernel, dim3(B), dim3(1024), 0, (hipStream_t)stream, in, w, bias, logits, probs,
                     NF, NC);
  EAV_CHECK_LAUNCH("eav_dense_softmax_fwd");
  return EAV_OK;
}

extern "C" int eav_dense_softmax_bwd(const float* dout, const float* probs, const float* in, const float* w,
                                     float* dw, float* dbias, float* din, int B, int NF, int NC, void* stream) {
  EAV_REQUIRE(dout && in && w && dw && dbias && B > 0 && NF > 0 && NC > 0 && NC <= NCMAX,
              "eav_dense_softmax_bwd: bad arguments (classes <= %d)", NCMAX);
  EAV_REQUIRE((size_t)B * NC * sizeof(float) <= 40 * 1024, "eav_dense_softmax_bwd: batch %d too large", B);
  hipLaunchKernelGGL(dense_softmax_bwd_kernel, dim3(cdiv(NF, 64)), dim3(256),
                     (B * NC + 4 * NCMAX * 64) * sizeof(float), (hipStream_t)stream, dout, probs, in, w, dw, dbias, din, B,
                     NF, NC);
  EAV_CHECK_LAUNCH("eav_dense_softmax_bwd");
  return EAV_OK;
}

extern "C" int eav_ce_fwd_bwd(const float* in, const int64_t* y, float* loss, float* din, int* ncorrect,
                              int* bad_label, int B, int NC, void* stream) {
  EAV_REQUIRE(in && y && B > 0 && NC > 0, "eav_ce_fwd_bwd: bad arguments");
  hipLaunchKernelGGL(ce_kernel, dim3(1), dim3(256), 0, (hipStream_t)stream, in, y, loss, din, ncorrect, bad_label, B,
                     NC);
  EAV_CHECK_LAUNCH("eav_ce_fwd_bwd");
  return EAV_OK;
}

__global__ __launch_bounds__(256) void scale_by_scalar_kernel(float* __restrict__ v, const float* __restrict__ sc,
                                                              int64_t n) {
  const float s = *sc;
  if (s == 1.f) return;
  for (int64_t i = (int64_t)blockIdx.x * 256 + threadIdx.x; i < n; i += (int64_t)gridDim.x * 256) v[i] *= s;
}

extern "C" int eav_scale_by_scalar(float* v, const float* scalar, int64_t n, void* stream) {
  EAV_REQUIRE(v && scalar && n > 0, "eav_scale_by_scalar: bad arguments");
  int64_t blocks = cdiv64(n, 256);
  if (blocks > 1024) blocks = 1024;
  hipLaunchKernelGGL(scale_by_scalar_kernel, dim3((int)blocks), dim3(256), 0, (hipStream_t)stream, v, scalar, n);
  EAV_CHECK_LAUNCH("eav_scale_by_scalar");
  return EAV_OK;
}

extern "C" int eav_adam_step(float* p, const float* g, float* m, float* v, int64_t n, float lr, float beta1,
                             float beta2, float eps, float weight_decay, int64_t step, int decoupled,
                             const int64_t* step_dev, void* stream) {
  EAV_REQUIRE(p && g && m && v && n > 0 && (step >= 1 || step_dev), "eav_adam_step: bad arguments");
  if (step < 1) step = 1;
  const double bc1 = 1.0 - pow((double)beta1, (double)step);
  const double bc2 = 1.0 - pow((double)beta2, (double)step);
  int64_t blocks = cdiv64(n, 256);
  if (blocks > 4096) blocks = 4096;
  hipLaunchKernelGGL(adam_kernel, dim3((int)blocks), dim3(256), 0, (hipStream_t)stream, p, g, m, v, n, lr, beta1,
                     beta2, eps, weight_decay, (float)bc1, (float)sqrt(bc2), decoupled, step_dev);
  EAV_CHECK_LAUNCH("eav_adam_step");
  return EAV_OK;
}

__global__ void counter_inc_kernel(int64_t* p) { *p += 1; }

__global__ void counter_inc4_kernel(int64_t* a, int64_t* b, int64_t* c, int64_t* d) {
  int64_t* p = threadIdx.x == 0 ? a : threadIdx.x == 1 ? b : threadIdx.x == 2 ? c : d;
  if (p) *p += 1;
}

extern "C" int eav_counter_inc4(int64_t* c0, int64_t* c1, int64_t* c2, int64_t* c3, void* stream) {
  EAV_REQUIRE(c0 || c1 || c2 || c3, "eav_counter_inc4: no counter");
  hipLaunchKernelGGL(counter_inc4_kernel, dim3(1), dim3(4), 0, (hipStream_t)stream, c0, c1, c2, c3);
  EAV_CHECK_LAUNCH("eav_counter_inc4");
  return EAV_OK;
}

extern "C" int eav_counter_inc(int64_t* counter, void* stream) {
  EAV_REQUIRE(counter, "eav_counter_inc: null counter");
  hipLaunchKernelGGL(counter_inc_kernel, dim3(1), dim3(1), 0, (hipStream_t)stream, counter);
  EAV_CHECK_LAUNCH("eav_counter_inc");
  return EAV_OK;
}

__global__ __launch_bounds__(256) void gather_rows_kernel(const float* __restrict__ src, const int64_t* __restrict__ idx,
                                                          float* __restrict__ out, int64_t row_elems, int vec) {
  const int64_t r = idx[blockIdx.y];
  if (vec) {
    const float4* s = reinterpret_cast<const float4*>(src + r * row_elems);
    float4* d = reinterpret_cast<float4*>(out + (int64_t)blockIdx.y * row_elems);
    for (int64_t i = (int64_t)blockIdx.x * 256 + threadIdx.x; i < row_elems / 4; i += (int64_t)gridDim.x * 256) d[i] = s[i];
  } else {
    const float* s = src + r * row_elems;
    float* d = out + (int64_t)blockIdx.y * row_elems;
    for (int64_t i = (int64_t)blockIdx.x * 256 + threadIdx.x; i < row_elems; i += (int64_t)gridDim.x * 256) d[i] = s[i];
  }
}

__global__ void gather_i64_kernel(const int64_t* __restrict__ src, const int64_t* __restrict__ idx,
                                  int64_t* __restrict__ out, int n) {
  const int i = blockIdx.x * 256 + threadIdx.x;
  if (i < n) out[i] = src[idx[i]];
}

__global__ void step_begin_kernel(int64_t* c0, int64_t* c1, int64_t* c2, int64_t* c3, int64_t* c4,
                                  const int64_t* __restrict__ labels, const int64_t* __restrict__ idx,
                                  int64_t* __restrict__ out, int n) {
  const int i = blockIdx.x * 256 + threadIdx.x;
  if (i == 0) {
    if (c0) *c0 += 1;
    if (c1) *c1 += 1;
    if (c2) *c2 += 1;
    if (c3) *c3 += 1;
    if (c4) *c4 += 1;
  }
  if (i < n) out[i] = labels[idx[i]];
}

extern "C" int eav_step_begin(int64_t* c0, int64_t* c1, int64_t* c2, int64_t* c3, int64_t* c4, const int64_t* labels,
                              const int64_t* idx, int64_t* out, int n, void* stream) {
  EAV_REQUIRE(n >= 0 && (n == 0 || (labels && idx && out)), "eav_step_begin: bad arguments");
  EAV_REQUIRE(c0 || c1 || c2 || c3 || c4 || n > 0, "eav_step_begin: nothing to do");
  hipLaunchKernelGGL(step_begin_kernel, dim3(n > 0 ? cdiv(n, 256) : 1), dim3(256), 0, (hipStream_t)stream, c0, c1, c2, c3, c4,
                     labels, idx, out, n);
  EAV_CHECK_LAUNCH("eav_step_begin");
  return EAV_OK;
}

extern "C" int eav_gather_rows(const float* src, const int64_t* idx, float* out, int nrows, int64_t row_elems,
                               void* stream) {
  EAV_REQUIRE(src && idx && out && nrows > 0 && row_elems > 0, "eav_gather_rows: bad arguments");
  const int vec = (row_elems % 4 == 0) && ((((uintptr_t)src | (uintptr_t)out) & 15) == 0);
  int64_t per = vec ? row_elems / 4 : row_elems;
  int gx = (int)(cdiv64(per, 256) > 64 ? 64 : cdiv64(per, 256));
  hipLaunchKernelGGL(gather_rows_kernel, dim3(gx, nrows), dim3(256), 0, (hipStream_t)stream, src, idx, out, row_elems, vec);
  EAV_CHECK_LAUNCH("eav_gather_rows");
  return EAV_OK;
}

extern "C" int eav_gather_i64(const int64_t* src, const int64_t* idx, int64_t* out, int n, void* stream) {
  EAV_REQUIRE(src && idx && out && n > 0, "eav_gather_i64: bad arguments");
  hipLaunchKernelGGL(gather_i64_kernel, dim3(cdiv(n, 256)), dim3(256), 0, (hipStream_t)stream, src, idx, out, n);
  EAV_CHECK_LAUNCH("eav_gather_i64");
  return EAV_OK;
}
```

eav_amd/eegnet.py:

```python
from __future__ import annotations

import os

import torch
import torch.nn as nn

from . import _lib
from .optim import CrossEntropyLoss, FusedAdam
from .runtime import (DeviceLoader, GraphStep, KernelFn, KernelModule, cached_workspace, eager_step,
                      gather_batch)

_PARAM_ORDER = [
    "firstConv.weight", "firstBN.weight", "firstBN.bias",
    "depthwiseConv.weight", "depthwiseBN.weight", "depthwiseBN.bias",
    "separableConv.weight", "separableBN.weight", "separableBN.bias",
    "dense.weight", "dense.bias",
]


class _Workspace:

    def __init__(self, B, C, S, klen, nb, dev):
        f = lambda *shape: torch.empty(*shape, dtype=torch.float32, device=dev)
        self.key = (B, C, S)
        T2, T3 = S // 4, S // 4 // 8
        self.T2, self.T3, self.NF = T2, T3, 64 * T3
        nchunk = (S + 1023) // 1024
        self.nchunk = nchunk
        self.y1, self.g1 = f(B, 8, C, S), f(B, 8, C, S)
        self.z = f(B, 64, S)
        self.p2, self.dp2 = f(B, 64, T2), f(B, 64, T2)
        self.u3, self.du3 = f(B, 64, T2), f(B, 64, T2)
        self.p3, self.dp3 = f(B, 64 * T3), f(B, 64 * T3)
        self.bn1, self.bn2, self.bn3 = f(6 * 8), f(6 * 64), f(6 * 64)
        self.wTf, self.wTb = f(1024, 64), f(1024, 64)
        self.np_fir = _lib.plain("eav_eegnet_fir_fwd_nparts", B, C, S)
        self.np_fir_fft = _lib.plain("eav_eegnet_fir_fwd_fft_nparts", B, C, S)
        self.part_fir = f(max(self.np_fir, self.np_fir_fft), 16)
        self.fft_ws = None
        self.part_dw = f(B * nchunk, 128)
        self.np_c3 = _lib.plain("eav_conv64_fwd_nparts", B, T2)
        self.np_c3_fft = _lib.plain("eav_conv64_fft_nparts", B, T2)
        self.part_c3 = f(max(self.np_c3, self.np_c3_fft), 128)
        self.c64_ws = None
        self.part_pb = f(B, 128)
        self.part_dst = f(B * nchunk, 16)
        self.part_dw2 = f(B * nchunk, 64 * C)
        self.np_fw = _lib.plain("eav_eegnet_fir_wgrad_nparts", B, C, S)
        self.part_fw = f(self.np_fw, 8 * klen)
        self.np_cw = _lib.plain("eav_conv64_wgrad_nparts", B, T2)
        self.part_cw = f(self.np_cw, 64 * 1024)


class _GenericWorkspace:

    def __init__(self, m, B, dev):
        f = lambda *shape: torch.empty(*shape, dtype=torch.float32, device=dev)
        C, S, F1, C2, F2, K = m.Chans, m.Samples, m.F1, m.F1 * m.D, m.F2, m.kernLength
        T2, T3 = S // 4, S // 4 // 8
        self.T2, self.T3, self.NF = T2, T3, F2 * T3
        self.y1, self.g1 = f(B, F1, C, S), f(B, F1, C, S)
        self.z, self.dz = f(B, C2, S), f(B, C2, S)
        self.p2, self.dp2 = f(B, C2, T2), f(B, C2, T2)
        self.u3, self.du3 = f(B, F2, T2), f(B, F2, T2)
        self.p3, self.dp3 = f(B, F2 * T3), f(B, F2 * T3)
        self.bn1, self.bn2, self.bn3 = f(6 * F1), f(6 * C2), f(6 * F2)
        self.np_t = _lib.plain("eav_tconv_fwd_nparts", B, C, S, F1, K)
        self.part_t = f(self.np_t, 2 * F1)
        self.np_s = _lib.plain("eav_spatial_nparts", B, S)
        self.part_s = f(self.np_s, 2 * C2)
        self.np_c = _lib.plain("eav_dconv_fwd_nparts", B, T2)
        self.part_c = f(self.np_c, 2 * F2)
        self.part_pb = f(B, 2 * max(C2, F2))
        self.part_sst = f(self.np_s, 2 * F1)
        self.part_sw = f(self.np_s, C2 * C)
        self.np_tw = _lib.plain("eav_tconv_wgrad_nparts", B, C, S, F1, K)
        self.part_tw = f(self.np_tw, F1 * K)
        self.part_cw = f(B, F2 * C2 * 16)


class IndexedBatch:

    def __init__(self, data, idx):
        self.data, self.idx = data, idx
        self.shape = (idx.numel(),) + tuple(data.shape[1:])
        self.device = data.device


class _EEGNetFn(KernelFn):
    @staticmethod
    def forward(ctx, x, model, *params):
        out = KernelFn.forward(ctx, x, model, *params)
        ctx.probs_version = model._saved[-1]._version
        return out

    @staticmethod
    def backward(ctx, dprobs):
        saved = ctx.model._saved
        if saved is not None and saved[0] == ctx.token and saved[-1]._version != ctx.probs_version:
            raise _lib.EavError("EEGNet_tor: the scores returned by forward() were modified in place before backward(); "
                                "they alias the probabilities the backward reads - clone() them first")
        return KernelFn.backward(ctx, dprobs)


class EEGNet_tor(KernelModule):
    _PARAM_ORDER = _PARAM_ORDER

    def __init__(self, nb_classes, Chans=30, Samples=500, dropoutRate=0.5, kernLength=300, F1=8, D=8, F2=64,
                 norm_rate=1.0, dropoutType='Dropout'):
        super().__init__()
        self._generic = not (F1 == 8 and D == 8 and F2 == 64 and 1 <= kernLength <= 300 and 1 <= Chans <= 32)
        if not (1 <= F1 <= 16 and 1 <= D <= 8 and F1 * D <= 64 and 1 <= F2 <= 64 and 1 <= kernLength <= 1024
                and 1 <= Chans <= 256 and 1 <= nb_classes <= 16 and Samples >= 32):
            raise NotImplementedError("eav_amd.EEGNet_tor: the gfx950 kernels cover F1<=16, D<=8, F1*D<=64, F2<=64, "
                                      "kernLength<=1024, Chans<=256, nb_classes<=16, Samples>=32")
        self.dropout = nn.Dropout(dropoutRate) if dropoutType == 'Dropout' else nn.Dropout2d(dropoutRate)
        self.firstConv = nn.Conv2d(1, F1, (1, kernLength), padding='same', bias=False)
        self.firstBN = nn.BatchNorm2d(F1)
        self.elu = nn.ELU()
        self.depthwiseConv = nn.Conv2d(F1, F1 * D, (Chans, 1), groups=F1, padding=0, bias=False)
        self.depthwiseBN = nn.BatchNorm2d(F1 * D)
        self.depthwisePool = nn.AvgPool2d((1, 4))
        self.separableConv = nn.Conv2d(F1 * D, F2, (1, 16), padding='same', bias=False)
        self.separableBN = nn.BatchNorm2d(F2)
        self.separablePool = nn.AvgPool2d((1, 8))
        self.flatten = nn.Flatten()
        self.dense = nn.Linear(F2 * (Samples // 4 // 8), nb_classes)
        self.softmax = nn.Softmax(dim=1)

        self.nb_classes, self.Chans, self.Samples, self.kernLength = nb_classes, Chans, Samples, kernLength
        self.F1, self.D, self.F2 = F1, D, F2
        self.norm_rate, self.dropoutRate = float(norm_rate), float(dropoutRate)
        self.spatial_dropout = dropoutType != 'Dropout'
        self.dropout_seed = 0x0EA5EED
        self.apply_max_norm = True
        self.kernel_events = None
        self.fir_precision = "fp32"
        self.fir_algo = os.environ.get("EAV_FIR_ALGO", "auto")
        self.conv_algo = os.environ.get("EAV_CONV_ALGO", "auto")
        self._infer = False
        self._step_begin = None
        self.fused_eval = False

    def _use_fft(self):
        if self.fir_algo not in ("auto", "fft", "mfma"):
            raise ValueError(f"fir_algo {self.fir_algo!r}: expected 'auto', 'fft' or 'mfma'")
        if self.fir_algo == "mfma" or self.kernLength > _lib.plain("eav_eegnet_fir_fft_max_taps"):
            return False
        return self.fir_algo == "fft" or self.Samples >= 1408

    def _use_conv_fft(self, B):
        if self.conv_algo not in ("auto", "fft", "mfma"):
            raise ValueError(f"conv_algo {self.conv_algo!r}: expected 'auto', 'fft' or 'mfma'")
        if self.conv_algo == "mfma":
            return False
        return self.conv_algo == "fft" or B * (self.Samples // 4) >= 40000

    def forward(self, x):
        self._require_gpu(x)
        if x.dim() == 3:
            x = x.unsqueeze(1)
        if x.dim() != 4 or x.shape[1] != 1 or x.shape[2] != self.Chans or x.shape[3] != self.Samples:
            raise ValueError(f"expected input [B,1,{self.Chans},{self.Samples}], got {tuple(x.shape)}")
        self._require_same_device(x)
        x = x.contiguous().float()
        self._ensure_flat()
        self._infer = (not torch.is_grad_enabled()) and (not self.training)
        return _EEGNetFn.apply(x, self, *self._params())

    def forward_indexed(self, data, idx):
        if data.dim() != 4 or data.shape[1] != 1 or data.shape[2] != self.Chans or data.shape[3] != self.Samples or \
                not data.is_cuda or data.dtype != torch.float32 or not data.is_contiguous():
            raise ValueError(f"expected a contiguous fp32 device array [N,1,{self.Chans},{self.Samples}]")
        if idx.dtype != torch.int64 or idx.device != data.device or idx.dim() != 1:
            raise ValueError("idx must be a 1-D int64 tensor on the data's device")
        if self._generic:
            out = torch.empty((idx.numel(),) + tuple(data.shape[1:]), dtype=torch.float32, device=data.device)
            _lib.call("eav_gather_rows", data.data_ptr(), idx.data_ptr(), out.data_ptr(), idx.numel(), data[0].numel(),
                      _lib.stream_ptr())
            return self.forward(out)
        self._require_same_device(data)
        self._ensure_flat()
        self._infer = (not torch.is_grad_enabled()) and (not self.training)
        return _EEGNetFn.apply(IndexedBatch(data, idx), self, *self._params())

    def _call(self, name, *args):
        ev = self.kernel_events
        if ev is not None and name in ev:
            a, b = torch.cuda.Event(enable_timing=True), torch.cuda.Event(enable_timing=True)
            a.record()
            _lib.call(name, *args)
            b.record()
            ev[name].append((a, b))
        else:
            _lib.call(name, *args)

    def _forward_output(self):
        return self._saved[-1].detach()

    def forward_batch(self, xs, ys, idx, optimizer):
        if not (xs.is_cuda and xs.dim() == 4 and xs.is_contiguous()):
            return super().forward_batch(xs, ys, idx, optimizer)
        batch = idx.numel()
        targets = torch.empty(batch, dtype=torch.long, device=xs.device)
        optimizer.step_counted = False
        if not self._generic:
            cnt = optimizer.device_step_counter()
            self._step_begin = (cnt.data_ptr(), ys.data_ptr(), idx.data_ptr(), targets.data_ptr(), batch)
        scores = self.forward_indexed(xs, idx)
        merged = not self._generic and self._step_begin is None
        self._step_begin = None
        optimizer.step_counted = merged
        if not merged:
            _lib.call("eav_gather_i64", ys.data_ptr(), idx.data_ptr(), targets.data_ptr(), batch, _lib.stream_ptr())
        return scores, targets

    def _launch_forward(self, x):
        if self._generic:
            return self._launch_forward_generic(x)
        L, P, st = self._call, _lib.ptr, _lib.stream_ptr()
        B, C, S, K, nb = x.shape[0], self.Chans, self.Samples, self.kernLength, self.nb_classes
        ws = self._workspace((B, C, S, str(x.device)), lambda: _Workspace(B, C, S, K, nb, x.device))
        training = bool(self.training)
        w1, g1w, g1b, w2, g2w, g2b, w3, g3w, g3b, wd, bd = [P(p) for p in self._params()]
        bn1, bn2, bn3 = self.firstBN, self.depthwiseBN, self.separableBN
        drop = self.dropoutRate if training else 0.0
        if self.spatial_dropout:
            drop = -drop
        masks = self._dropout_masks if training else None
        self._token += 1
        seed1, seed2 = self.dropout_seed, self.dropout_seed + 1
        cnt = None
        if drop != 0.0 and masks is None:
            cnt = P(self._counter(x.device))
        m1 = P(masks[0]) if masks is not None else None
        m2 = P(masks[1]) if masks is not None else None

        def bnfin(part, nparts, nch, count, gw, gb, bn, buf):
            b0 = P(buf)
            L("eav_bn_finalize", P(part), nparts, nch, float(count), gw, gb, P(bn.running_mean), P(bn.running_var),
              int(training), float(bn.momentum), float(bn.eps), b0, b0 + 4 * nch, b0 + 8 * nch, b0 + 12 * nch, st)

        if self.fir_precision != "fp32":
            raise ValueError(f"fir_precision {self.fir_precision!r}: only 'fp32' exists (the split mode was retired)")
        counters = [cnt] + ([P(bn.num_batches_tracked) for bn in (bn1, bn2, bn3)] if training else [None] * 3)
        begin, self._step_begin = self._step_begin, None
        if not self._use_conv_fft(B):
            L("eav_eegnet_step_prologue", w3, P(ws.wTf), P(ws.wTb), *counters, st)
            self._step_begin = begin
        elif begin is not None:
            L("eav_step_begin", *counters, *begin, st)
        elif cnt is not None or training:
            L("eav_counter_inc4", *counters, st)
        np_fir = ws.np_fir
        infer = self.fused_eval and self._infer and not training and S % 4 == 0
        if infer:
            bnfin(ws.part_fir, ws.np_fir, 8, B * C * S, g1w, g1b, bn1, ws.bn1)
            bnfin(ws.part_dw, B * ws.nchunk, 64, B * S, g2w, g2b, bn2, ws.bn2)
            if isinstance(x, IndexedBatch):
                L("eav_eegnet_block1_infer", P(x.data), P(x.idx), w1, P(ws.bn1), w2, P(ws.bn2), P(ws.p2), B, C, S, K, st)
            else:
                L("eav_eegnet_block1_infer", P(x), None, w1, P(ws.bn1), w2, P(ws.bn2), P(ws.p2), B, C, S, K, st)
        elif self._use_fft():
            np_fir = ws.np_fir_fft
            pf = P(ws.part_fir) if training else None
            if isinstance(x, IndexedBatch):
                L("eav_eegnet_fir_fwd_fft", P(x.data), P(x.idx), w1, P(ws.y1), pf, B, C, S, K, st)
            else:
                L("eav_eegnet_fir_fwd_fft", P(x), None, w1, P(ws.y1), pf, B, C, S, K, st)
        else:
            if isinstance(x, IndexedBatch):
                L("eav_eegnet_fir_fwd_indexed", P(x.data), P(x.idx), w1, P(ws.y1), P(ws.part_fir), B, C, S, K, st)
            else:
                L("eav_eegnet_fir_fwd", P(x), w1, P(ws.y1), P(ws.part_fir), B, C, S, K, st)
        if not infer:
            bnfin(ws.part_fir, np_fir, 8, B * C * S, g1w, g1b, bn1, ws.bn1)
            if not training and drop == 0.0 and m1 is None and S % 4 == 0:
                bnfin(ws.part_dw, B * ws.nchunk, 64, B * S, g2w, g2b, bn2, ws.bn2)
                L("eav_eegnet_dw_fwd_pool_eval", P(ws.y1), P(ws.bn1), w2, P(ws.z), P(ws.part_dw), P(ws.bn2), P(ws.p2), B, C, S,
                  st)
            else:
                L("eav_eegnet_dw_fwd", P(ws.y1), P(ws.bn1), w2, P(ws.z), P(ws.part_dw), B, C, S, st)
                bnfin(ws.part_dw, B * ws.nchunk, 64, B * S, g2w, g2b, bn2, ws.bn2)
                L("eav_bn_elu_pool_fwd", P(ws.z), P(ws.bn2), P(ws.p2), B, 64, S, 4, drop, seed1, m1, cnt, st)
        np_c3 = ws.np_c3
        if self._use_conv_fft(B):
            if ws.c64_ws is None:
                ws.c64_ws = torch.zeros(_lib.plain("eav_conv64_fft_ws_floats", B, ws.T2), dtype=torch.float32,
                                        device=ws.y1.device)
            np_c3 = ws.np_c3_fft
            L("eav_conv64_fft_fwd", P(ws.p2), w3, P(ws.u3), P(ws.part_c3), P(ws.c64_ws), B, ws.T2, 0, st)
        else:
            L("eav_conv64_fwd", P(ws.p2), P(ws.wTf), P(ws.u3), P(ws.part_c3), B, ws.T2, 7, st)
        bnfin(ws.part_c3, np_c3, 64, B * ws.T2, g3w, g3b, bn3, ws.bn3)
        L("eav_bn_elu_pool_fwd", P(ws.u3), P(ws.bn3), P(ws.p3), B, 64, ws.T2, 8, drop, seed2, m2, cnt, st)
        probs = torch.empty(B, nb, dtype=torch.float32, device=x.device)
        L("eav_dense_softmax_fwd", P(ws.p3), wd, bd, None, P(probs), B, ws.NF, nb, st)
        if self.apply_max_norm:
            L("eav_renorm_rows2", w2, 64, C, wd, nb, ws.NF, self.norm_rate, st)
        self._saved = (self._token, x, training, drop, seed1, seed2, masks, cnt, ws, probs)
        return self._token

    def _launch_forward_generic(self, x):
        L, P, st = self._call, _lib.ptr, _lib.stream_ptr()
        B, C, S, K, nb = x.shape[0], self.Chans, self.Samples, self.kernLength, self.nb_classes
        F1, D, F2 = self.F1, self.D, self.F2
        C2 = F1 * D
        ws = self._workspace(("generic", B, C, S, str(x.device)), lambda: _GenericWorkspace(self, B, x.device))
        training = bool(self.training)
        w1, g1w, g1b, w2, g2w, g2b, w3, g3w, g3b, wd, bd = [P(p) for p in self._params()]
        bn1, bn2, bn3 = self.firstBN, self.depthwiseBN, self.separableBN
        drop = self.dropoutRate if training else 0.0
        if self.spatial_dropout:
            drop = -drop
        masks = self._dropout_masks if training else None
        self._token += 1
        seed1, seed2 = self.dropout_seed, self.dropout_seed + 1
        cnt = None
        if drop != 0.0 and masks is None:
            cnt = P(self._counter(x.device))
        if cnt is not None or training:
            L("eav_counter_inc4", cnt, *([P(bn.num_batches_tracked) for bn in (bn1, bn2, bn3)] if training else [None] * 3),
              st)
        m1 = P(masks[0]) if masks is not None else None
        m2 = P(masks[1]) if masks is not None else None

        def bnfin(part, nparts, nch, count, gw, gb, bn, buf):
            b0 = P(buf)
            L("eav_bn_finalize", P(part), nparts, nch, float(count), gw, gb, P(bn.running_mean), P(bn.running_var),
              int(training), float(bn.momentum), float(bn.eps), b0, b0 + 4 * nch, b0 + 8 * nch, b0 + 12 * nch, st)

        L("eav_tconv_fwd", P(x), w1, P(ws.y1), P(ws.part_t), B, C, S, F1, K, st)
        bnfin(ws.part_t, ws.np_t, F1, B * C * S, g1w, g1b, bn1, ws.bn1)
        L("eav_spatial_fwd", P(ws.y1), P(ws.bn1), w2, P(ws.z), P(ws.part_s), B, C, S, F1, D, 1, st)
        bnfin(ws.part_s, ws.np_s, C2, B * S, g2w, g2b, bn2, ws.bn2)
        L("eav_bn_elu_pool_fwd", P(ws.z), P(ws.bn2), P(ws.p2), B, C2, S, 4, drop, seed1, m1, cnt, st)
        L("eav_dconv_fwd", P(ws.p2), w3, P(ws.u3), P(ws.part_c), B, C2, F2, ws.T2, 16, 0, st)
        bnfin(ws.part_c, ws.np_c, F2, B * ws.T2, g3w, g3b, bn3, ws.bn3)
        L("eav_bn_elu_pool_fwd", P(ws.u3), P(ws.bn3), P(ws.p3), B, F2, ws.T2, 8, drop, seed2, m2, cnt, st)
        probs = torch.empty(B, nb, dtype=torch.float32, device=x.device)
        L("eav_dense_softmax_fwd", P(ws.p3), wd, bd, None, P(probs), B, ws.NF, nb, st)
        if self.apply_max_norm:
            L("eav_renorm_rows", w2, C2, C, self.norm_rate, st)
            L("eav_renorm_rows", wd, nb, ws.NF, self.norm_rate, st)
        self._saved = (self._token, x, training, drop, seed1, seed2, masks, cnt, False, ws, probs)
        return self._token

    def _launch_backward_generic(self, dprobs):
        L, P, st = self._call, _lib.ptr, _lib.stream_ptr()
        _, x, training, drop, seed1, seed2, masks, cnt, _, ws, probs = self._saved
        B, C, S, K, nb = x.shape[0], self.Chans, self.Samples, self.kernLength, self.nb_classes
        F1, D, F2 = self.F1, self.D, self.F2
        C2, T2, NF = F1 * D, ws.T2, ws.NF
        flat, gflat, offs = self._flat
        g = {k: gflat[offs[k][0]:offs[k][0] + offs[k][1]] for k in _PARAM_ORDER}
        w2, w3, wd = P(self.depthwiseConv.weight), P(self.separableConv.weight), P(self.dense.weight)
        m1 = P(masks[0]) if masks is not None else None
        m2 = P(masks[1]) if masks is not None else None
        tr = int(training)
        L("eav_dense_softmax_bwd", P(dprobs), P(probs), P(ws.p3), wd, P(g["dense.weight"]), P(g["dense.bias"]),
          P(ws.dp3), B, NF, nb, st)
        b3 = P(ws.bn3)
        L("eav_bn_elu_pool_bwd_reduce", P(ws.dp3), P(ws.u3), b3, P(ws.part_pb), B, F2, T2, 8, drop, seed2, m2, cnt, st)
        L("eav_bn_bwd_finalize", P(ws.part_pb), B, F2, float(B * T2), tr, P(g["separableBN.weight"]),
          P(g["separableBN.bias"]), b3 + 16 * F2, b3 + 20 * F2, st)
        L("eav_bn_elu_pool_bwd_apply", P(ws.dp3), P(ws.u3), b3, b3 + 16 * F2, P(ws.du3), B, F2, T2, 8, drop, seed2, m2,
          cnt, st)
        L("eav_dconv_fwd", P(ws.du3), w3, P(ws.dp2), None, B, F2, C2, T2, 16, 1, st)
        L("eav_dconv_wgrad", P(ws.du3), P(ws.p2), P(ws.part_cw), B, C2, F2, T2, 16, st)
        n3 = F2 * C2 * 16
        L("eav_reduce_partials", P(ws.part_cw), B, n3, n3, 1.0, P(g["separableConv.weight"]), st)
        b2 = P(ws.bn2)
        L("eav_bn_elu_pool_bwd_reduce", P(ws.dp2), P(ws.z), b2, P(ws.part_pb), B, C2, S, 4, drop, seed1, m1, cnt, st)
        L("eav_bn_bwd_finalize", P(ws.part_pb), B, C2, float(B * S), tr, P(g["depthwiseBN.weight"]),
          P(g["depthwiseBN.bias"]), b2 + 16 * C2, b2 + 20 * C2, st)
        L("eav_bn_elu_pool_bwd_apply", P(ws.dp2), P(ws.z), b2, b2 + 16 * C2, P(ws.dz), B, C2, S, 4, drop, seed1, m1,
          cnt, st)
        b1 = P(ws.bn1)
        L("eav_spatial_bwd", P(ws.y1), P(ws.dz), b1, w2, P(ws.g1), P(ws.part_sst), P(ws.part_sw), B, C, S, F1, D, 1, st)
        L("eav_reduce_partials", P(ws.part_sw), ws.np_s, C2 * C, C2 * C, 1.0, P(g["depthwiseConv.weight"]), st)
        L("eav_bn_bwd_finalize", P(ws.part_sst), ws.np_s, F1, float(B * C * S), tr, P(g["firstBN.weight"]),
          P(g["firstBN.bias"]), b1 + 16 * F1, b1 + 20 * F1, st)
        L("eav_tconv_wgrad", P(x), P(ws.y1), P(ws.g1), b1, P(ws.part_tw), B, C, S, F1, K, st)
        L("eav_reduce_partials", P(ws.part_tw), ws.np_tw, F1 * K, F1 * K, 1.0, P(g["firstConv.weight"]), st)
        named = dict(self.named_parameters())
        return [g[k].view(named[k].shape) if named[k].requires_grad else None for k in _PARAM_ORDER]

    def _launch_backward(self, dprobs, token):
        self._check_token(token)
        if self._generic:
            return self._launch_backward_generic(dprobs)
        L, P, st = self._call, _lib.ptr, _lib.stream_ptr()
        _, x, training, drop, seed1, seed2, masks, cnt, ws, probs = self._saved
        B, C, S, K, nb = x.shape[0], self.Chans, self.Samples, self.kernLength, self.nb_classes
        T2, NF = ws.T2, ws.NF
        flat, gflat, offs = self._flat
        g = {k: gflat[offs[k][0]:offs[k][0] + offs[k][1]] for k in _PARAM_ORDER}
        w2, wd = P(self.depthwiseConv.weight), P(self.dense.weight)
        m1 = P(masks[0]) if masks is not None else None
        m2 = P(masks[1]) if masks is not None else None
        tr = int(training)

        L("eav_dense_softmax_bwd", P(dprobs), P(probs), P(ws.p3), wd, P(g["dense.weight"]), P(g["dense.bias"]),
          P(ws.dp3), B, NF, nb, st)
        b3 = P(ws.bn3)
        if training:
            L("eav_bn_elu_pool_bwd_reduce", P(ws.dp3), P(ws.u3), b3, P(ws.part_pb), B, 64, T2, 8, drop, seed2, m2, cnt, st)
            L("eav_bn_bwd_finalize", P(ws.part_pb), B, 64, float(B * T2), tr, P(g["separableBN.weight"]),
              P(g["separableBN.bias"]), b3 + 4 * 256, b3 + 4 * 320, st)
            L("eav_bn_elu_pool_bwd_apply", P(ws.dp3), P(ws.u3), b3, b3 + 4 * 256, P(ws.du3), B, 64, T2, 8, drop, seed2, m2,
              cnt, st)
        else:
            L("eav_bn_elu_pool_bwd_eval", P(ws.dp3), P(ws.u3), b3, P(ws.du3), P(ws.part_pb), B, 64, T2, 8, drop, seed2, m2,
              cnt, st)
            L("eav_bn_bwd_finalize", P(ws.part_pb), B, 64, float(B * T2), tr, P(g["separableBN.weight"]),
              P(g["separableBN.bias"]), b3 + 4 * 256, b3 + 4 * 320, st)
        if self._use_conv_fft(B):
            L("eav_conv64_fft_fwd", P(ws.du3), P(self.separableConv.weight), P(ws.dp2), None, P(ws.c64_ws), B, T2, 2, st)
        else:
            L("eav_conv64_fwd", P(ws.du3), P(ws.wTb), P(ws.dp2), None, B, T2, 8, st)
        if self._use_conv_fft(B):
            L("eav_conv64_fft_wgrad", P(ws.du3), P(g["separableConv.weight"]), P(ws.c64_ws), B, T2, st)
        else:
            L("eav_conv64_wgrad", P(ws.du3), P(ws.p2), P(ws.part_cw), B, T2, 7, st)
            L("eav_reduce_partials", P(ws.part_cw), ws.np_cw, 65536, 65536, 1.0, P(g["separableConv.weight"]), st)
        b2 = P(ws.bn2)
        b1 = P(ws.bn1)
        if training:
            L("eav_bn_elu_pool_bwd_reduce", P(ws.dp2), P(ws.z), b2, P(ws.part_pb), B, 64, S, 4, drop, seed1, m1, cnt, st)
            L("eav_bn_bwd_finalize", P(ws.part_pb), B, 64, float(B * S), tr, P(g["depthwiseBN.weight"]),
              P(g["depthwiseBN.bias"]), b2 + 4 * 256, b2 + 4 * 320, st)
            L("eav_eegnet_dw_bwd_fused", P(ws.y1), P(ws.z), P(ws.dp2), b2, b1, w2, P(ws.g1), P(ws.part_dst),
              P(ws.part_dw2), B, C, S, drop, seed1, m1, cnt, st)
        else:
            L("eav_eegnet_dw_bwd_fused_eval", P(ws.y1), P(ws.z), P(ws.dp2), b2, b1, w2, P(ws.g1), P(ws.part_dst),
              P(ws.part_dw2), P(ws.part_dw), B, C, S, drop, seed1, m1, cnt, st)
        bn2job = (None, 0, 0, 0.0, 0, None, None, None, None) if training else \
            (P(ws.part_dw), B * ws.nchunk, 64, float(B * S), tr, P(g["depthwiseBN.weight"]), P(g["depthwiseBN.bias"]),
             b2 + 4 * 256, b2 + 4 * 320)
        L("eav_reduce_and_bn_bwd_finalize", P(ws.part_dw2), B * ws.nchunk, 64 * C, 64 * C, P(g["depthwiseConv.weight"]),
          P(ws.part_dst), B * ws.nchunk, 8, float(B * C * S), tr, P(g["firstBN.weight"]), P(g["firstBN.bias"]), b1 + 4 * 32,
          b1 + 4 * 40, *bn2job, st)
        if self._use_fft():
            if ws.fft_ws is None:
                ws.fft_ws = torch.empty(_lib.plain("eav_eegnet_fir_wgrad_fft_ws_floats", B, C, S), dtype=torch.float32,
                                        device=ws.y1.device)
            xi = isinstance(x, IndexedBatch)
            L("eav_eegnet_fir_wgrad_fft", P(x.data) if xi else P(x), P(x.idx) if xi else None,
              P(ws.y1) if training else None, P(ws.g1), b1, P(ws.fft_ws), P(g["firstConv.weight"]), B, C, S, K, st)
        else:
            if isinstance(x, IndexedBatch):
                L("eav_eegnet_fir_wgrad_indexed", P(x.data), P(x.idx), P(ws.y1) if training else None, P(ws.g1), b1,
                  P(ws.part_fw), B, C, S, K, st)
            else:
                L("eav_eegnet_fir_wgrad", P(x), P(ws.y1) if training else None, P(ws.g1), b1, P(ws.part_fw), B, C, S, K,
                  st)
            L("eav_reduce_partials", P(ws.part_fw), ws.np_fw, 8 * K, 8 * K, 1.0, P(g["firstConv.weight"]), st)
        named = dict(self.named_parameters())
        return [g[k].view(named[k].shape) if named[k].requires_grad else None for k in _PARAM_ORDER]


class Trainer_uni:
    def __init__(self, model, data, lr=1e-4, batch_size=32, num_epochs=10, device=None):
        self.lr = lr
        self.batch_size = batch_size
        self.num_epochs = num_epochs
        self.device = device if device else torch.device("cuda" if torch.cuda.is_available() else "cpu")
        self.device = torch.device(self.device)
        if self.device.type != "cuda":
            raise _lib.EavError("eav_amd.Trainer_uni needs an MI355X (torch device 'cuda' on ROCm); no CPU fallback")
        self.tr_x, self.tr_y, self.te_x, self.te_y = data
        self.train_dataloader = self._prepare_dataloader(self.tr_x, self.tr_y, shuffle=True)
        self.test_dataloader = self._prepare_dataloader(self.te_x, self.te_y, shuffle=False)

        self.model = model
        self.criterion = CrossEntropyLoss()
        self.optimizer = FusedAdam(self.model.parameters(), lr=self.lr, capturable=True)
        self.model.to(self.device)
        self.grad_sync = None
        self.use_graph = True
        self._graphs = {}

    def _prepare_dataloader(self, x, y, shuffle=False):
        return DeviceLoader(x, y, self.batch_size, shuffle, self.device)

    def train(self):
        self.model.train()
        dl = self.train_dataloader
        for epoch in range(self.num_epochs):
            for batch_idx, idx in enumerate(dl.index_batches()):
                if self.use_graph and len(idx) == self.batch_size:
                    key = (len(idx), bool(self.model.training))
                    if key not in self._graphs:
                        self._graphs[key] = GraphStep(self.model, self.optimizer, self.criterion, dl.x, dl.y,
                                                      len(idx), self.grad_sync)
                    scores, loss = self._graphs[key].run(idx)
                else:
                    scores, loss = eager_step(self.model, self.optimizer, self.criterion, *dl.gather(idx), self.grad_sync)
                if batch_idx % 100 == 0:
                    print(f"Epoch [{epoch+1}/{self.num_epochs}], Step [{batch_idx}/{len(self.train_dataloader)}], "
                          f"Loss: {loss.item():.4f}")
            self.criterion.check()
            if self.test_dataloader:
                self.validate()

    def validate(self):
        self.model.eval()
        nb = len(self.test_dataloader)
        losses = torch.zeros(max(nb, 1), dtype=torch.float32, device=self.device)
        correct = torch.zeros((), dtype=torch.int32, device=self.device)
        with torch.no_grad():
            for k, (data, targets) in enumerate(self.test_dataloader):
                scores = self.model(data)
                self.criterion.accumulate(scores, targets, losses[k], correct)
        total_loss = 0
        for v in losses[:nb].cpu().tolist():
            total_loss += v
        total_correct = int(correct.item())
        self.criterion.check()
        avg_loss = total_loss / len(self.test_dataloader)
        accuracy = total_correct / len(self.test_dataloader.dataset)
        print(f"Validation - Loss: {avg_loss:.4f}, Accuracy: {accuracy:.4f}")
```

include/eav_hip.h:

```cpp
#ifndef EAV_HIP_H
#define EAV_HIP_H
#include <stdint.h>

#ifdef __cplusplus
extern "C" {
#endif

#define EAV_ABI_VERSION 3

const char* eav_last_error(void);
int eav_abi_version(void);

int eav_reduce_partials(const float* part, int nparts, int64_t stride, int n, float scale, float* out, void* stream);

int eav_bn_finalize(const float* part, int nparts, int nch, double count, const float* gamma, const float* beta,
                    float* running_mean, float* running_var, int training, float momentum, float eps, float* mean,
                    float* invstd, float* scale, float* shift, void* stream);
int eav_bn_bwd_finalize(const float* part, int nparts, int nch, double count, int training, float* dgamma,
                        float* dbeta, float* m1, float* m2, void* stream);
int eav_reduce_and_bn_bwd_finalize(const float* part, int nparts, int64_t stride, int n, float* out,
                                   const float* part_a, int nparts_a, int nch_a, double count_a, int training_a,
                                   float* dgamma_a, float* dbeta_a, float* m1_a, float* m2_a,
                                   const float* part_b, int nparts_b, int nch_b, double count_b, int training_b,
                                   float* dgamma_b, float* dbeta_b, float* m1_b, float* m2_b, void* stream);
int eav_renorm_rows(float* w, int rows, int cols, float maxnorm, void* stream);
int eav_renorm_rows2(float* w_a, int rows_a, int cols_a, float* w_b, int rows_b, int cols_b, float maxnorm,
                     void* stream);

int eav_eegnet_fir_fwd_nparts(int B, int C, int S);
int eav_eegnet_fir_fwd(const float* x, const float* w1, float* y1, float* stat_part, int B, int C, int S, int klen,
                       void* stream);
int eav_eegnet_block1_infer(const float* x, const int64_t* xidx, const float* w1, const float* bn1, const float* w2,
                            const float* bn2, float* p2, int B, int C, int S, int klen, void* stream);
int eav_eegnet_fir_wgrad_nparts(int B, int C, int S);
int eav_eegnet_fir_wgrad(const float* x, const float* y1, const float* g1, const float* bn_params, float* part,
                         int B, int C, int S, int klen, void* stream);
int eav_eegnet_fir_fft_max_taps(void);
int eav_eegnet_fir_fwd_fft_nparts(int B, int C, int S);
int eav_eegnet_fir_fwd_fft(const float* x, const int64_t* xidx, const float* w1, float* y1, float* stat_part, int B, int C,
                           int S, int klen, void* stream);
int64_t eav_eegnet_fir_wgrad_fft_ws_floats(int B, int C, int S);
int eav_eegnet_fir_wgrad_fft(const float* x, const int64_t* xidx, const float* y1, const float* g1, const float* bn_params,
                             float* ws, float* dW, int B, int C, int S, int klen, void* stream);
int eav_eegnet_fir_fwd_indexed(const float* x, const int64_t* xidx, const float* w1, float* y1, float* stat_part, int B,
                               int C, int S, int klen, void* stream);
int eav_eegnet_fir_wgrad_indexed(const float* x, const int64_t* xidx, const float* y1, const float* g1,
                                 const float* bn_params, float* part, int B, int C, int S, int klen, void* stream);
int eav_eegnet_dw_fwd(const float* y1, const float* bn1, const float* w2, float* z, float* stat_part, int B, int C,
                      int S, void* stream);
int eav_eegnet_dw_fwd_pool_eval(const float* y1, const float* bn1, const float* w2, float* z, float* stat_part,
                                const float* bn2, float* p2, int B, int C, int S, void* stream);
int eav_eegnet_dw_bwd(const float* y1, const float* dz, const float* bn1, const float* w2, float* g1,
                      float* stat_part, float* w_part, int B, int C, int S, void* stream);

int eav_eegnet_dw_bwd_fused(const float* y1, const float* z, const float* dp2, const float* bn2, const float* bn1,
                            const float* w2, float* g1, float* stat_part, float* w_part, int B, int C, int S,
                            float drop_p, uint64_t seed, const uint8_t* mask, const uint64_t* seed_dev, void* stream);

int eav_eegnet_dw_bwd_fused_eval(const float* y1, const float* z, const float* dp2, const float* bn2, const float* bn1,
                                 const float* w2, float* g1, float* stat_part, float* w_part, float* bn2_part, int B, int C,
                                 int S, float drop_p, uint64_t seed, const uint8_t* mask, const uint64_t* seed_dev,
                                 void* stream);

int eav_bn_elu_pool_fwd(const float* in, const float* bn, float* out, int B, int CH, int T, int P, float drop_p,
                        uint64_t seed, const uint8_t* mask, const uint64_t* seed_dev, void* stream);
int eav_bn_elu_pool_bwd_reduce(const float* dp, const float* u, const float* bn, float* part , int B,
                               int CH, int T, int P, float drop_p, uint64_t seed, const uint8_t* mask,
                               const uint64_t* seed_dev, void* stream);
int eav_bn_elu_pool_bwd_apply(const float* dp, const float* u, const float* bn, const float* m12 ,
                              float* du, int B, int CH, int T, int P, float drop_p, uint64_t seed,
                              const uint8_t* mask, const uint64_t* seed_dev, void* stream);
int eav_bn_elu_pool_bwd_eval(const float* dp, const float* u, const float* bn, float* du, float* part , int B,
                             int CH, int T, int P, float drop_p, uint64_t seed, const uint8_t* mask,
                             const uint64_t* seed_dev, void* stream);

int eav_conv64_prep_weights(const float* w , float* wT_fwd , float* wT_bwd, void* stream);
int eav_eegnet_step_prologue(const float* w, float* wT_fwd, float* wT_bwd, int64_t* c0, int64_t* c1, int64_t* c2,
                             int64_t* c3, void* stream);
int eav_conv64_ntiles(int T);
int eav_conv64_fwd_nparts(int B, int T);
int eav_conv64_fwd(const float* in, const float* wT, float* out, float* stat_part, int B, int T, int padl,
                   void* stream);
int64_t eav_conv64_fft_ws_floats(int B, int T);
int eav_conv64_fft_nparts(int B, int T);
int eav_conv64_fft_fwd(const float* in, const float* w, float* out, float* stat_part, float* ws, int B, int T, int bwd,
                       void* stream);
int eav_conv64_fft_wgrad(const float* du, float* dW, float* ws, int B, int T, void* stream);
int eav_conv64_wgrad_nparts(int B, int T);
int eav_conv64_wgrad(const float* du, const float* in, float* part, int B, int T, int padl, void* stream);

int eav_tconv_fwd_nparts(int B, int C, int S, int F1, int K);
int eav_tconv_fwd(const float* x, const float* w, float* y1, float* stat_part, int B, int C, int S, int F1, int K,
                  void* stream);
int eav_tconv_wgrad_nparts(int B, int C, int S, int F1, int K);
int eav_tconv_wgrad(const float* x, const float* y1, const float* g1, const float* bn_params, float* part, int B,
                    int C, int S, int F1, int K, void* stream);
int eav_spatial_nparts(int B, int S);
int eav_spatial_fwd(const float* y1, const float* bn1, const float* wd, float* z, float* stat_part, int B, int C,
                    int S, int F1, int D, int elu, void* stream);
int eav_spatial_bwd(const float* y1, const float* dz, const float* bn1, const float* wd, float* g1, float* stat_part,
                    float* w_part, int B, int C, int S, int F1, int D, int elu, void* stream);
int eav_dconv_fwd_nparts(int B, int T);
int eav_dconv_fwd(const float* in, const float* w, float* out, float* stat_part, int B, int Cin, int Cout, int T,
                  int K, int transposed, void* stream);
int eav_dconv_wgrad(const float* dy, const float* x, float* part, int B, int Cin, int Cout, int T, int K, void* stream);
int eav_sepconv_fwd_nparts(int B, int T);
int eav_sepconv_fwd(const float* a, const float* wdw, const float* wp, float* d3, float* z, float* stat_part, int B,
                    int C2, int F2, int T, int K2, void* stream);
int eav_pointwise_bwd_nparts(int B, int T);
int eav_pointwise_bwd(const float* du, const float* d3, const float* wp, float* dd3, float* w_part, int B, int C2,
                      int F2, int T, void* stream);
int eav_dwt_bwd(const float* dd3, const float* a, const float* wdw, float* da, float* w_part, int B, int C2, int T,
                int K2, void* stream);

int eav_dense_softmax_fwd(const float* in, const float* w, const float* bias, float* logits, float* probs, int B,
                          int NF, int NC, void* stream);
int eav_dense_softmax_bwd(const float* dout, const float* probs, const float* in, const float* w, float* dw,
                          float* dbias, float* din, int B, int NF, int NC, void* stream);
int eav_ce_fwd_bwd(const float* in, const int64_t* y, float* loss, float* din, int* ncorrect, int* bad_label, int B,
                   int NC, void* stream);
int eav_scale_by_scalar(float* v, const float* scalar, int64_t n, void* stream);
int eav_adam_step(float* p, const float* g, float* m, float* v, int64_t n, float lr, float beta1, float beta2,
                  float eps, float weight_decay, int64_t step, int decoupled, const int64_t* step_dev, void* stream);
int eav_gather_rows(const float* src, const int64_t* idx, float* out, int nrows, int64_t row_elems, void* stream);
int eav_gather_i64(const int64_t* src, const int64_t* idx, int64_t* out, int n, void* stream);
int eav_counter_inc(int64_t* counter, void* stream);
int eav_counter_inc4(int64_t* c0, int64_t* c1, int64_t* c2, int64_t* c3, void* stream);
int eav_step_begin(int64_t* c0, int64_t* c1, int64_t* c2, int64_t* c3, int64_t* c4, const int64_t* labels,
                   const int64_t* idx, int64_t* out, int n, void* stream);

int eav_gemm_f32(const float* A, const float* B, float* C, int M, int N, int K, int lda, int ldb, int ldc,
                 int transA, int transB, int batch, int heads, int64_t sAb, int64_t sAh, int64_t sBb, int64_t sBh,
                 int64_t sCb, int64_t sCh, float alpha, const float* bias, int gelu, float* pre, const float* resid,
                 int ldr, int accumulate, void* stream);
int eav_gemm_f32_splitk_plan(int M, int N, int K);
int eav_gemm_f32_splitk(const float* A, const float* B, float* C, float* ws, int M, int N, int K, int lda, int ldb,
                        int transA, int transB, void* stream);
#define EAV_SP_SLOT 4128
int eav_sp_kpad(int K);
int eav_sp_absmax(const float* src, int R, int C, int64_t ld, float* slot, void* stream);
int eav_sp_convert(const float* src, int R, int C, int64_t ld, float* slot, void* dst, void* dstT, void* stream);
int eav_sp_convert_gelu(const float* src, int R, int C, int64_t ld, float* slot, void* dst, void* dstT, void* stream);
int eav_sp_convert_colsum_nparts(int R);
int eav_sp_convert_colsum(const float* src, int R, int C, int64_t ld, float* slot, void* dst, void* dstT,
                          float* colsum_part, void* stream);
typedef struct EavPlaneJob {
  const float* src;
  void* dst;
  void* dstT;
  float* slot;
  int R, C;
} EavPlaneJob;
int eav_sp_refresh_planes(const void* jobs, int n, int maxR, int maxC, void* stream);
int eav_layernorm_fwd_amax(const float* x, const float* gamma, const float* beta, float* y, float* mean, float* rstd,
                           int M, int D, float eps, float* amax_slot, void* stream);
int eav_layernorm_bwd_amax(const float* dy, const float* x, const float* gamma, const float* mean, const float* rstd,
                           float* dx, int accumulate, float* part, int M, int D, float* amax_slot, void* stream);
int eav_layernorm_bwd_planes(const float* dy, const float* x, const float* gamma, const float* mean, const float* rstd,
                             float* dx, int accumulate, float* part, int M, int D, float* slot, void* planes,
                             const float* slot_old, const float* slot_dy, const float* slot_rstd, void* stream);
int eav_layernorm_bwd_bound(float* slot_out, const float* slot_old, const float* slot_dy, const float* gamma,
                            const float* rstd, int M, int D, const float* slot_rstd, void* stream);
int eav_gelu_bwd_amax(float* dact, const float* pre, int64_t n, float* amax_slot, void* stream);
int eav_gemm_sp(const void* A, const void* B, float* C, const float* slotA, const float* slotB, int M, int N, int K,
                int ldc, int batch, int64_t sA_bytes, int64_t sC, float alpha, const float* bias, int gelu, float* pre,
                const float* resid, int ldr, int accumulate, float* amax_slot, void* stream);
int eav_gemm_sp_planes(const void* A, const void* B, float* C, const float* slotA, const float* slotB, int M, int N, int K,
                       int ldc, int batch, int64_t sA_bytes, int64_t sC, float alpha, const float* bias, int gelu,
                       float* pre, const float* resid, int ldr, int accumulate, float* amax_slot, void* planes_out,
                       const float* planes_slot, void* stream);
int eav_layernorm_fwd_planes(const float* x, const float* gamma, const float* beta, float* y, void* planes,
                             const float* scale_slot, float* mean, float* rstd, int M, int D, float eps, void* stream);
int eav_rownorm_max(const float* w, int R, int C, int64_t ld, float* out, void* stream);
int eav_colnorm_max(const float* w, int R, int C, int64_t ld, float* out, void* stream);
int eav_norm_max_multi(const void* jobs, int njobs, int max_blocks, void* stream);
int eav_sp_bound_scale(float* slot_out, const float* amax_slot, const float* norm, float factor, void* stream);
int eav_tf_forward_scales(const float* params, int64_t layer_stride, int layers, int off_g1, int off_b1, int off_g2,
                          int off_b2, int off_bfc1, int D, int FF, const float* wnorm_fc1, float* slots,
                          int64_t slot_stride, int k_y1, int k_y2, int k_act, void* stream);
int eav_tf_forward_scales_qkv(const float* params, int64_t layer_stride, int layers, int off_g1, int off_b1, int off_g2,
                              int off_b2, int off_bfc1, int off_bqkv, int D, int FF, const float* wnorm_fc1,
                              const float* wnorm_qkv, float* slots, int64_t slot_stride, int k_y1, int k_y2, int k_act,
                              int k_qkv, void* stream);
int eav_gemm_sp_splitk_plan(int M, int N, int K);
int eav_gemm_sp_splitk(const void* A, const void* B, float* C, float* ws, const float* slotA, const float* slotB, int M,
                       int N, int T, int accumulate, void* stream);
int eav_gemm_sp_x1(const void* A, const void* B, float* C, const float* slotA, const float* slotB, int M, int N, int K,
                   int ldc, int batch, int64_t sA_bytes, int64_t sC, float alpha, const float* bias, int gelu, float* pre,
                   const float* resid, int ldr, int accumulate, float* amax_slot, void* stream);
#define EAV_GEMM_ONE_TERM 1
#define EAV_GEMM_PLANES_NOLIFT 4
#define EAV_GEMM_NO_BLOCKMAX 8
#define EAV_GEMM_SHARED_GPU 2
int eav_gemm_sp_ex(const void* A, const void* B, float* C, const float* slotA, const float* slotB, int M, int N, int K,
                   int ldc, int batch, int64_t sA_bytes, int64_t sC, float alpha, const float* bias, int gelu, float* pre,
                   const float* resid, int ldr, int accumulate, float* amax_slot, void* planes_out,
                   const float* planes_slot, float* colsum_part, int flags, void* stream);
int eav_gemm_sp_splitk_x1(const void* A, const void* B, float* C, float* ws, const float* slotA, const float* slotB, int M,
                          int N, int T, int accumulate, void* stream);
int eav_gemm_sp_splitk_x2(const void* A, const void* B, float* C, float* ws, const float* slotA, const float* slotB, int M,
                          int N, int T, int accumulate, void* stream);
int eav_attn_sp_npad(int N);
int eav_attn_sp_prep(const float* src, float* slot, void* rowp, void* tp, int B, int N, int ncols, int secw,
                     unsigned tmask, void* stream);
int eav_attn_fwd_sp(const void* rowp, const void* tp, const float* slot, float* ao, float* lse, float* amax_slot, int B,
                    int H, int N, int head_dim, float scale, void* stream);
int eav_attn_fwd_sp_planes(const void* rowp, const void* tp, const float* slot, float* ao, float* lse, float* amax_slot,
                           void* ao_planes, float* ao_slot, int B, int H, int N, int head_dim, float scale, void* stream);
int eav_attn_bwd_sp(const void* rowp, const void* tp, const void* dorow, const void* dotp, const float* slot,
                    const float* slot_do, float* slot_ds, const float* ao, const float* dout, const float* lse,
                    float* delta, float* dqkv, float* amax_slot, int B, int H, int N, int head_dim, float scale,
                    void* stream);
int eav_attn_dqkv_bound(float* slot_out, const float* slot_do, const float* slot_qkv, int N, float scale, void* stream);
int eav_attn_bwd_sp_planes(const void* rowp, const void* tp, const void* dorow, const void* dotp, const float* slot,
                           const float* slot_do, float* slot_ds, const float* ao, const float* dout, const float* lse,
                           float* delta, float* dqkv, float* amax_slot, void* planes, float* planes_slot,
                           float* colsum_part, const void* ao_planes, const float* ao_slot, int B, int H, int N,
                           int head_dim, float scale, void* stream);
int eav_attn_fwd(const float* qkv, float* ao, float* lse, int B, int H, int N, int head_dim, float scale,
                 void* stream);
int eav_attn_bwd(const float* qkv, const float* ao, const float* dout, const float* lse, float* delta, float* dqkv,
                 int B, int H, int N, int head_dim, float scale, void* stream);
int eav_attn_fwd_dropout(const float* qkv, float* ao, float* lse, int B, int H, int N, int head_dim, float scale,
                         float drop_p, uint64_t seed, const uint8_t* mask, const uint64_t* seed_dev, void* stream);
int eav_attn_bwd_dropout(const float* qkv, const float* ao, const float* dout, const float* lse, float* delta,
                         float* dqkv, int B, int H, int N, int head_dim, float scale, float drop_p, uint64_t seed,
                         const uint8_t* mask, const uint64_t* seed_dev, void* stream);
int eav_attn_fwd_sp_dropout(const void* rowp, const float* slot, float* ao, float* lse, float* amax_slot, int B, int H,
                            int N, int head_dim, float scale, float drop_p, uint64_t seed, const uint8_t* mask,
                            const uint64_t* seed_dev, void* stream);
int eav_attn_bwd_sp_dropout(const void* rowp, const void* dorow, const float* slot, const float* slot_do, float* slot_ds,
                            const float* ao, const float* dout, const float* lse, float* delta, float* dqkv,
                            float* amax_slot, int B, int H, int N, int head_dim, float scale, float drop_p, uint64_t seed,
                            const uint8_t* mask, const uint64_t* seed_dev, void* stream);
int eav_tf_dropout_mask(uint8_t* mask, int64_t n, float drop_p, uint64_t seed, const uint64_t* seed_dev, void* stream);
int eav_tf_dropout_add(const float* y, const float* resid, float* out, int64_t n, float drop_p, uint64_t seed,
                       const uint8_t* mask, const uint64_t* seed_dev, void* stream);
int eav_softmax_dropout_fwd(float* s, float* pd, int64_t rows, int N, int ld, float drop_p, uint64_t seed,
                            const uint8_t* mask, const uint64_t* seed_dev, void* stream);
int eav_softmax_dropout_bwd(const float* P, float* dP, float* pd, int64_t rows, int N, int ld, float drop_p,
                            uint64_t seed, const uint8_t* mask, const uint64_t* seed_dev, void* stream);
int eav_layernorm_fwd(const float* x, const float* gamma, const float* beta, float* y, float* mean, float* rstd,
                      int M, int D, float eps, void* stream);
int eav_layernorm_bwd_nparts(int M);
int eav_layernorm_bwd(const float* dy, const float* x, const float* gamma, const float* mean, const float* rstd,
                      float* dx, int accumulate, float* part, int M, int D, void* stream);
int eav_softmax_fwd(float* s, int64_t rows, int N, int ld, void* stream);
int eav_softmax_bwd(const float* P, float* dP, int64_t rows, int N, int ld, void* stream);
int eav_gelu_bwd(float* dact, const float* pre, int64_t n, void* stream);
int eav_colsum_nparts(int M);
int eav_colsum(const float* dy, float* part, int M, int N, int ld, void* stream);
int eav_im2col(const float* x, float* col, int B, int C, int H, int W, int P, int sy, int sx, int transposed,
               void* stream);
int eav_embed_finish(float* h, const float* cls, const float* dist, const float* pos, int B, int ntok, int D,
                     int nextra, void* stream);
int eav_embed_bwd(const float* dh, float* dpos, float* demb, int B, int ntok, int D, int nextra, void* stream);
int eav_token_rows(float* h, float* rows, int B, int ntok, int D, int nextra, int scatter, void* stream);
int eav_pair_mean(float* seq, float* pooled, int B, int D, int backward, void* stream);

int eav_shallow_embed_nparts(int B, int S);
int eav_shallow_embed_fwd(const float* x, const float* wc, const float* wv , int ldv, float* u,
                          float* v, int B, int C, int S, int NF, int KC, void* stream);
int eav_shallow_embed_bwd(const float* dv, const float* x, const float* u, const float* wc, float* part_c,
                          float* part_v, int B, int C, int S, int NF, int KC, void* stream);
int eav_relu_dropout(float* h, int64_t n, float drop_p, uint64_t seed, const uint8_t* mask, const uint64_t* seed_dev,
                     void* stream);
int eav_relu_dropout_bwd(float* dact, const float* act, int64_t n, float drop_p, void* stream);
int eav_dropout_add(const float* y, const float* resid, float* out, int64_t n, float drop_p, uint64_t seed,
                    const uint8_t* mask, const uint64_t* seed_dev, void* stream);
int eav_add_strided(const float* a, int lda, const float* b, int ldb, float* out, int ldo, int64_t M, int n,
                    void* stream);
int eav_colstats_nparts(int64_t M);
int eav_colstats(const float* x, float* part, int64_t M, int N, int ld, void* stream);
int eav_sqpool_log_fwd(const float* v, const float* bn, float* pooled, float* out, int B, int T, int NF, int NP,
                       int win, int stride, float lo, float hi, float drop_p, uint64_t seed, const uint8_t* mask,
                       const uint64_t* seed_dev, void* stream);
int eav_sqpool_log_bwd(const float* dy, const float* pooled, const float* v, const float* bn, float* g, float* part,
                       int B, int T, int NF, int NP, int win, int stride, float lo, float hi, float drop_p,
                       uint64_t seed, const uint8_t* mask, const uint64_t* seed_dev, void* stream);
int eav_bn_rows_bwd(const float* g, const float* v, const float* bn, float* dx, int64_t M, int NF, void* stream);

int eav_resize_normalize_u8(const uint8_t* frames, const int* kx, const int* boundsx, const int* ky,
                            const int* boundsy, float* out, int n, int H, int W, int C, int OH, int OW, int ksize_x,
                            int ksize_y, double rescale, const float* mean3, const float* std3, void* stream);

int eav_ast_fbank(const float* wav, const double* window400, const double* twiddle256, const double* melT, float* out,
                  int n, int L, int max_len, int nmel, double preemph, double mel_floor, float mean, float std2,
                  void* stream);

int eav_decimate_fir_f64(const double* x, const double* h, double* y, int nch, int64_t n_in, int64_t n_out, int down,
                         int ntaps, int center, void* stream);
int eav_sosfilt_f64(const double* x, double* y, const double* sos, const double* H, const double* AL, double* zend,
                    double* zstart, int nch, int64_t n, int nsec, int Lc, void* stream);

int eav_audio_conv5_fwd(const float* in, const float* w, const float* bias, float* out, uint8_t* idx, int B, int C,
                        int N, int Lin, int Lout, int pool, float drop_p, uint64_t seed, const uint8_t* mask,
                        const uint64_t* seed_dev, void* stream);
int eav_audio_conv5_dgrad(const float* dout, const float* gate_in, float gscale_in, const float* w, float* din,
                          const float* aux, const uint8_t* idx, float gscale_out, int B, int C, int N, int Lin, int Lout,
                          int mode, void* stream);
int eav_audio_wgrad_nparts(int B, int Cact, int M, int Lout);
int eav_audio_conv5_wgrad(const float* dout, const float* gate, float gscale, const float* act, float* part, int B,
                          int Cact, int M, int Lact, int Lout, int nparts, void* stream);

int eav_video_conv_relayout(const float* w, float* wf, float* wd, int Co, int Ci, int KK, void* stream);
int eav_video_conv_fwd(const float* x, const float* wf, float* out, int B, int C, int H, int W, int N, int KH, int KW,
                       int S, int P, int OH, int OW, int nchw, void* stream);
int eav_video_conv_dgrad(const float* dout, const float* wd, const float* add, float* din, int B, int C, int H, int W,
                         int N, int KH, int KW, int S, int P, int OH, int OW, void* stream);
int eav_video_wgrad_nparts(int N, int C, int KK, int64_t M);
int eav_video_conv_wgrad(const float* dout, const float* x, float* part, int B, int C, int H, int W, int N, int KH, int KW,
                         int S, int P, int OH, int OW, int nchw, int nparts, void* stream);
int eav_video_bn_nparts(int64_t M);
int eav_video_bn_stats(const float* x, float* part, int64_t M, int C, void* stream);
int eav_video_bn_apply(const float* x, const float* scale, const float* shift, const float* res, const float* rscale,
                       const float* rshift, float* out, int64_t M, int C, int relu, void* stream);
int eav_video_bn_bwd(const float* dy, const float* y, const float* x, const float* bn, float* g, float* part, int64_t M,
                     int C, void* stream);
int eav_video_maxpool_fwd(const float* x, float* out, uint8_t* idx, int B, int H, int W, int C, int OH, int OW, int K,
                          int S, int P, void* stream);
int eav_video_maxpool_bwd(const float* dout, const uint8_t* idx, float* dx, int B, int H, int W, int C, int OH, int OW,
                          int K, int S, int P, void* stream);
int eav_video_head_pool(const float* y, float* pooled, uint8_t* idx, int B, int HW, int C, void* stream);
int eav_video_head_scale_pool(const float* y, const float* A, float* attn, float* z, int B, int HW, int C, void* stream);
int eav_video_head_attn_bwd(const float* y, const float* dz, float* dA, int B, int HW, int C, void* stream);
int eav_video_head_feat_bwd(const float* dz, const float* attn, const float* dP, const uint8_t* idx, float* dy, int B,
                            int HW, int C, void* stream);
int eav_video_counters_inc(int64_t* c, int n, void* stream);

int eav_peak_mfma_f32(float* sink, int blocks, int iters, void* stream);
int eav_peak_mfma_f16(float* sink, int blocks, int iters, void* stream);
int eav_peak_l2_read(const void* src, int footprint_kb, int mode, int iters, int blocks, float* sink, void* stream);
int eav_peak_copy_variant(const float* src, float* dst, int64_t n, int variant, int blocks, void* stream);
int eav_peak_copy(const float* src, float* dst, int64_t n, void* stream);

#ifdef __cplusplus
}
#endif
#endif
```

Before: 46820 samples/s.

## Fuse final BN-ELU-pool with dense head and overlap conv64 wgrad on side stream

Folds the dense-layer logit computation into the last BN+ELU+pool forward kernel as per-row partial logits, with a finishing kernel that does bias, softmax and max-norm renorm in one launch. In backward, the dense gradient and the pool-backward reduction run in one launch, with extra blocks computing dW/dbias while the others recompute dp3 from the weights. The separable-conv weight gradient is moved onto a forked side stream to overlap with the rest of backward. This saves launches and one pass over the pooled features, at the cost of added code paths, a per-row partial-logit buffer and cross-stream synchronisation.

New measurement: 47570 samples/s, median of 6. 1.6% higher.

```diff
diff --git a/eav_amd/_lib.py b/eav_amd/_lib.py
--- a/eav_amd/_lib.py
+++ b/eav_amd/_lib.py
@@ -40,6 +40,8 @@
     "eav_eegnet_dw_bwd_fused_eval": [_p, _p, _p, _p, _p, _p, _p, _p, _p, _p, _i, _i, _i, _f, _u64, _p, _p, _p],
     "eav_bn_elu_pool_fwd": [_p, _p, _p, _i, _i, _i, _i, _f, _u64, _p, _p, _p],
     "eav_bn_elu_pool_bwd_reduce": [_p, _p, _p, _p, _i, _i, _i, _i, _f, _u64, _p, _p, _p],
+    "eav_bn_elu_pool_fwd_dense": [_p, _p, _p, _p, _p, _i, _i, _i, _i, _i, _f, _u64, _p, _p, _p],
+    "eav_bn_elu_pool_bwd_reduce_dense": [_p, _p, _p, _p, _p, _p, _p, _p, _p, _p, _i, _i, _i, _i, _i, _f, _u64, _p, _p, _p],
     "eav_bn_elu_pool_bwd_apply": [_p, _p, _p, _p, _p, _i, _i, _i, _i, _f, _u64, _p, _p, _p],
     "eav_bn_elu_pool_bwd_eval": [_p, _p, _p, _p, _p, _i, _i, _i, _i, _f, _u64, _p, _p, _p],
     "eav_conv64_prep_weights": [_p, _p, _p, _p],
@@ -47,8 +49,10 @@
     "eav_conv64_wgrad": [_p, _p, _p, _i, _i, _i, _p],
     "eav_conv64_fft_fwd": [_p, _p, _p, _p, _p, _i, _i, _i, _p],
     "eav_conv64_fft_wgrad": [_p, _p, _p, _i, _i, _p],
+    "eav_conv64_fft_spectra": [_p, _p, _p],
     "eav_dense_softmax_fwd": [_p, _p, _p, _p, _p, _i, _i, _i, _p],
     "eav_dense_softmax_bwd": [_p, _p, _p, _p, _p, _p, _p, _i, _i, _i, _p],
+    "eav_dense_finish_softmax_renorm": [_p, _p, _p, _p, _i, _i, _i, _p, _i, _i, _p, _i, _i, _f, _p],
     "eav_ce_fwd_bwd": [_p, _p, _p, _p, _p, _p, _i, _i, _p],
     "eav_scale_by_scalar": [_p, _p, _i64, _p],
     "eav_adam_step": [_p, _p, _p, _p, _i64, _f, _f, _f, _f, _f, _i64, _i, _p, _p],
@@ -162,6 +166,7 @@
     "eav_abi_version": ([], _i),
     "eav_last_error": ([], C.c_char_p),
     "eav_eegnet_fir_fwd_nparts": ([_i, _i, _i], _i),
+    "eav_dense_max_classes": ([], _i),
     "eav_eegnet_fir_fwd_fft_nparts": ([_i, _i, _i], _i),
     "eav_eegnet_fir_wgrad_fft_ws_floats": ([_i, _i, _i], _i64),
     "eav_eegnet_fir_fft_max_taps": ([], _i),
diff --git a/eav_amd/csrc/dense_head.h b/eav_amd/csrc/dense_head.h
--- /dev/null
+++ b/eav_amd/csrc/dense_head.h
@@ -0,0 +1,115 @@
+#pragma once
+#include "eav_common.h"
+
+constexpr int EAV_HEAD_NCMAX = 16;
+
+__device__ __forceinline__ float dense_dot(const float* __restrict__ dout, const float* __restrict__ probs, int b, int NC) {
+  float dot = 0.f;
+  if (probs)
+    for (int k = 0; k < NC; ++k) dot += dout[b * NC + k] * probs[b * NC + k];
+  return dot;
+}
+__device__ __forceinline__ float dense_dl(const float* __restrict__ dout, const float* __restrict__ probs, int b, int j,
+                                          int NC, float dot) {
+  const float v = dout[b * NC + j];
+  return probs ? probs[b * NC + j] * (v - dot) : v;
+}
+
+template <int NCT>
+__device__ __forceinline__ void dense_bwd_body(const float* __restrict__ dout, const float* __restrict__ probs,
+                                               const float* __restrict__ in, const float* __restrict__ w,
+                                               float* __restrict__ dw, float* __restrict__ dbias, float* __restrict__ din,
+                                               int B, int NF, int NC, int blk, float* smem) {
+  float* dl = smem;
+  float* pw = dl + B * NC;
+  for (int idx = threadIdx.x; idx < B * NC; idx += blockDim.x) {
+    const int b = idx / NC;
+    dl[idx] = dense_dl(dout, probs, b, idx - b * NC, NC, dense_dot(dout, probs, b, NC));
+  }
+  __syncthreads();
+  if (blk == 0 && (int)threadIdx.x < NC) {
+    float s = 0.f;
+    for (int b = 0; b < B; ++b) s += dl[b * NC + threadIdx.x];
+    dbias[threadIdx.x] = s;
+  }
+  const int f = threadIdx.x & 63, slice = threadIdx.x >> 6;
+  const int i = blk * 64 + f;
+  const bool live = i < NF;
+  float wv[NCT], acc[NCT];
+#pragma unroll
+  for (int j = 0; j < NCT; ++j) {
+    wv[j] = (live && j < NC) ? w[(int64_t)j * NF + i] : 0.f;
+    acc[j] = 0.f;
+  }
+  for (int b0 = slice; b0 < B; b0 += 32) {
+    float v[8];
+#pragma unroll
+    for (int u = 0; u < 8; ++u) v[u] = (live && b0 + 4 * u < B) ? in[(int64_t)(b0 + 4 * u) * NF + i] : 0.f;
+#pragma unroll
+    for (int u = 0; u < 8; ++u) {
+      const int b = b0 + 4 * u;
+      if (b < B) {
+        float d = 0.f;
+#pragma unroll
+        for (int j = 0; j < NCT; ++j)
+          if (j < NC) {
+            const float g = dl[b * NC + j];
+            acc[j] += g * v[u];
+            d += wv[j] * g;
+          }
+        if (din && live) din[(int64_t)b * NF + i] = d;
+      }
+    }
+  }
+#pragma unroll
+  for (int j = 0; j < NCT; ++j) pw[(slice * NCT + j) * 64 + f] = acc[j];
+  __syncthreads();
+  if (slice == 0 && live) {
+#pragma unroll
+    for (int j = 0; j < NCT; ++j)
+      if (j < NC)
+        dw[(int64_t)j * NF + i] = (pw[j * 64 + f] + pw[(NCT + j) * 64 + f]) + (pw[(2 * NCT + j) * 64 + f] + pw[(3 * NCT + j) * 64 + f]);
+  }
+}
+
+__device__ __forceinline__ void renorm_row_body(float* __restrict__ row, int cols, float maxnorm, float* red) {
+  const bool vec = (cols & 3) == 0 && (reinterpret_cast<uintptr_t>(row) & 15) == 0;
+  float v[1] = {0.f};
+  if (vec) {
+    const float4* row4 = reinterpret_cast<const float4*>(row);
+    const int n4 = cols >> 2;
+    float a[4] = {0.f, 0.f, 0.f, 0.f};
+    for (int i0 = threadIdx.x; i0 < n4; i0 += 1024) {
+      float4 q[4];
+#pragma unroll
+      for (int u = 0; u < 4; ++u) q[u] = i0 + 256 * u < n4 ? row4[i0 + 256 * u] : make_float4(0.f, 0.f, 0.f, 0.f);
+#pragma unroll
+      for (int u = 0; u < 4; ++u) a[u] += (q[u].x * q[u].x + q[u].y * q[u].y) + (q[u].z * q[u].z + q[u].w * q[u].w);
+    }
+    v[0] = (a[0] + a[1]) + (a[2] + a[3]);
+  } else {
+    for (int i = threadIdx.x; i < cols; i += 256) v[0] += row[i] * row[i];
+  }
+  block_sum_256<1>(v, red);
+  if (threadIdx.x == 0) {
+    float norm = sqrtf(v[0]);
+    red[8] = norm > maxnorm ? maxnorm / (norm + 1e-7f) : 1.f;
+  }
+  __syncthreads();
+  const float s = red[8];
+  if (s == 1.f) return;
+  if (vec) {
+    float4* row4 = reinterpret_cast<float4*>(row);
+    const int n4 = cols >> 2;
+    for (int i0 = threadIdx.x; i0 < n4; i0 += 1024) {
+      float4 q[4];
+#pragma unroll
+      for (int u = 0; u < 4; ++u) q[u] = i0 + 256 * u < n4 ? row4[i0 + 256 * u] : make_float4(0.f, 0.f, 0.f, 0.f);
+#pragma unroll
+      for (int u = 0; u < 4; ++u)
+        if (i0 + 256 * u < n4) row4[i0 + 256 * u] = make_float4(q[u].x * s, q[u].y * s, q[u].z * s, q[u].w * s);
+    }
+  } else {
+    for (int i = threadIdx.x; i < cols; i += 256) row[i] *= s;
+  }
+}
diff --git a/eav_amd/csrc/eav_common.hip b/eav_amd/csrc/eav_common.hip
--- a/eav_amd/csrc/eav_common.hip
+++ b/eav_amd/csrc/eav_common.hip
@@ -1,4 +1,5 @@
 #include "eav_common.h"
+#include "dense_head.h"
 
 #include <stdarg.h>
 #include <stdio.h>
@@ -261,54 +262,14 @@
 
 __global__ void renorm_rows_kernel(float* __restrict__ w, int rows, int cols, float maxnorm, float* __restrict__ w_b,
                                    int cols_b) {
-  __shared__ float red[8];
+  __shared__ float red[9];
   int r = blockIdx.x;
   if (r >= rows) {
     r -= rows;
     w = w_b;
     cols = cols_b;
   }
-  float* row = w + (int64_t)r * cols;
-  const bool vec = (cols & 3) == 0 && (reinterpret_cast<uintptr_t>(row) & 15) == 0;
-  float v[1] = {0.f};
-  if (vec) {
-    const float4* row4 = reinterpret_cast<const float4*>(row);
-    const int n4 = cols >> 2;
-    float a[4] = {0.f, 0.f, 0.f, 0.f};
-    for (int i0 = threadIdx.x; i0 < n4; i0 += 1024) {
-      float4 q[4];
-#pragma unroll
-      for (int u = 0; u < 4; ++u) q[u] = i0 + 256 * u < n4 ? row4[i0 + 256 * u] : make_float4(0.f, 0.f, 0.f, 0.f);
-#pragma unroll
-      for (int u = 0; u < 4; ++u) a[u] += (q[u].x * q[u].x + q[u].y * q[u].y) + (q[u].z * q[u].z + q[u].w * q[u].w);
-    }
-    v[0] = (a[0] + a[1]) + (a[2] + a[3]);
-  } else {
-    for (int i = threadIdx.x; i < cols; i += 256) v[0] += row[i] * row[i];
-  }
-  block_sum_256<1>(v, red);
-  __shared__ float sc;
-  if (threadIdx.x == 0) {
-    float norm = sqrtf(v[0]);
-    sc = norm > maxnorm ? maxnorm / (norm + 1e-7f) : 1.f;
-  }
-  __syncthreads();
-  float s = sc;
-  if (s == 1.f) return;
-  if (vec) {
-    float4* row4 = reinterpret_cast<float4*>(row);
-    const int n4 = cols >> 2;
-    for (int i0 = threadIdx.x; i0 < n4; i0 += 1024) {
-      float4 q[4];
-#pragma unroll
-      for (int u = 0; u < 4; ++u) q[u] = i0 + 256 * u < n4 ? row4[i0 + 256 * u] : make_float4(0.f, 0.f, 0.f, 0.f);
-#pragma unroll
-      for (int u = 0; u < 4; ++u)
-        if (i0 + 256 * u < n4) row4[i0 + 256 * u] = make_float4(q[u].x * s, q[u].y * s, q[u].z * s, q[u].w * s);
-    }
-  } else {
-    for (int i = threadIdx.x; i < cols; i += 256) row[i] *= s;
-  }
+  renorm_row_body(w + (int64_t)r * cols, cols, maxnorm, red);
 }
 
 extern "C" int eav_renorm_rows(float* w, int rows, int cols, float maxnorm, void* stream) {
diff --git a/eav_amd/csrc/eegnet_block.hip b/eav_amd/csrc/eegnet_block.hip
--- a/eav_amd/csrc/eegnet_block.hip
+++ b/eav_amd/csrc/eegnet_block.hip
@@ -1,4 +1,5 @@
 #include "eav_common.h"
+#include "dense_head.h"
 #include "../../include/eav_hip.h"
 
 namespace {
@@ -153,6 +154,35 @@
 }
 
 template <int P>
+__device__ __forceinline__ float pool_window_sum(const float* src, int to, int T, bool vec, float sc, float sh) {
+  float s = 0.f;
+#pragma unroll
+  for (int j = 0; j < P; j += 4) {
+    float v[4];
+    ld4(src, to * P + j, T, vec, v);
+#pragma unroll
+    for (int e = 0; e < 4; ++e) s += elu_f(sc * v[e] + sh);
+  }
+  return s;
+}
+template <int P>
+__device__ __forceinline__ void pool_bwd_window_sums(const float* src, int to, int T, bool vec, float go, float sc, float sh,
+                                                     float mean, float invstd, float (&st)[2]) {
+#pragma unroll
+  for (int j = 0; j < P; j += 4) {
+    float v[4];
+    ld4(src, to * P + j, T, vec, v);
+#pragma unroll
+    for (int e = 0; e < 4; ++e) {
+      const float pre = sc * v[e] + sh;
+      const float g = go * elu_grad_from_out(pre, elu_f(pre));
+      st[0] += g;
+      st[1] += g * ((v[e] - mean) * invstd);
+    }
+  }
+}
+
+template <int P>
 __global__ __launch_bounds__(256) void pool_fwd_kernel(const float* __restrict__ in, const float* __restrict__ bn,
                                                        float* __restrict__ out, int CH, int T, float drop_p,
                                                        uint64_t seed_in,
@@ -164,14 +194,7 @@
   const float* src = in + (int64_t)row * T;
   const bool vec = (T & 3) == 0;
   for (int to = threadIdx.x; to < To; to += 256) {
-    float s = 0.f;
-#pragma unroll
-    for (int j = 0; j < P; j += 4) {
-      float v[4];
-      ld4(src, to * P + j, T, vec, v);
-#pragma unroll
-      for (int e = 0; e < 4; ++e) s += elu_f(sc * v[e] + sh);
-    }
+    const float s = pool_window_sum<P>(src, to, T, vec, sc, sh);
     const uint64_t oi = (uint64_t)row * To + to;
     out[oi] = s * (1.0f / P) * dropout_mult_row(drop_p, seed, mask, oi, (uint64_t)row);
   }
@@ -194,20 +217,88 @@
   for (int to = threadIdx.x; to < To; to += 256) {
     const uint64_t oi = (uint64_t)row * To + to;
     const float go = dp[oi] * (1.0f / P) * dropout_mult_row(drop_p, seed, mask, oi, (uint64_t)row);
-#pragma unroll
-    for (int j = 0; j < P; j += 4) {
-      float v[4];
-      ld4(src, to * P + j, T, vec, v);
-#pragma unroll
-      for (int e = 0; e < 4; ++e) {
-        const float pre = sc * v[e] + sh;
-        const float g = go * elu_grad_from_out(pre, elu_f(pre));
-        st[0] += g;
-        st[1] += g * ((v[e] - mean) * invstd);
-      }
-    }
+    pool_bwd_window_sums<P>(src, to, T, vec, go, sc, sh, mean, invstd, st);
   }
   block_sum_256<2>(st, red);
+  if (threadIdx.x < 2) part[(int64_t)b * 2 * CH + threadIdx.x * CH + ch] = st[0];
+}
+
+template <int P, int NCT>
+__global__ __launch_bounds__(256) void pool_fwd_dense_kernel(const float* __restrict__ in, const float* __restrict__ bn,
+                                                             float* __restrict__ out, int CH, int T, float drop_p,
+                                                             uint64_t seed_in, const uint8_t* __restrict__ mask,
+                                                             const uint64_t* __restrict__ seed_dev,
+                                                             const float* __restrict__ w, float* __restrict__ part_logit,
+                                                             int NC) {
+  const uint64_t seed = dropout_seed(seed_in, seed_dev);
+  __shared__ float red[4 * NCT];
+  const int row = blockIdx.x, ch = row % CH;
+  const float sc = bn[2 * CH + ch], sh = bn[3 * CH + ch];
+  const int To = T / P;
+  const int64_t NF = (int64_t)CH * To;
+  const float* src = in + (int64_t)row * T;
+  const float* wr = w + (int64_t)ch * To;
+  const bool vec = (T & 3) == 0;
+  float acc[NCT];
+#pragma unroll
+  for (int j = 0; j < NCT; ++j) acc[j] = 0.f;
+  for (int to = threadIdx.x; to < To; to += 256) {
+    float wv[NCT];
+#pragma unroll
+    for (int j = 0; j < NCT; ++j) wv[j] = j < NC ? wr[j * NF + to] : 0.f;
+    const float s = pool_window_sum<P>(src, to, T, vec, sc, sh);
+    const uint64_t oi = (uint64_t)row * To + to;
+    const float o = s * (1.0f / P) * dropout_mult_row(drop_p, seed, mask, oi, (uint64_t)row);
+    out[oi] = o;
+#pragma unroll
+    for (int j = 0; j < NCT; ++j) acc[j] += wv[j] * o;
+  }
+  block_sum_256<NCT>(acc, red);
+  if ((int)threadIdx.x < NC) part_logit[(int64_t)row * NC + threadIdx.x] = acc[0];
+}
+
+template <int P, int NCT>
+__global__ __launch_bounds__(256) void pool_bwd_reduce_dense_kernel(const float* __restrict__ dprobs,
+                                                                    const float* __restrict__ probs,
+                                                                    const float* __restrict__ feat,
+                                                                    const float* __restrict__ w, float* __restrict__ dw,
+                                                                    float* __restrict__ dbias, float* __restrict__ dp,
+                                                                    const float* __restrict__ u,
+                                                                    const float* __restrict__ bn, float* __restrict__ part,
+                                                                    int B, int CH, int T, int NC, int nwb, float drop_p,
+                                                                    uint64_t seed_in, const uint8_t* __restrict__ mask,
+                                                                    const uint64_t* __restrict__ seed_dev) {
+  extern __shared__ float smem[];
+  const int To = T / P;
+  const int NF = CH * To;
+  if ((int)blockIdx.x < nwb) {
+    dense_bwd_body<NCT>(dprobs, probs, feat, w, dw, dbias, nullptr, B, NF, NC, blockIdx.x, smem);
+    return;
+  }
+  const uint64_t seed = dropout_seed(seed_in, seed_dev);
+  const int row = blockIdx.x - nwb, ch = row % CH, b = row / CH;
+  const float mean = bn[ch], invstd = bn[CH + ch], sc = bn[2 * CH + ch], sh = bn[3 * CH + ch];
+  float dl[NCT];
+  {
+    const float dot = dense_dot(dprobs, probs, b, NC);
+#pragma unroll
+    for (int j = 0; j < NCT; ++j) dl[j] = j < NC ? dense_dl(dprobs, probs, b, j, NC, dot) : 0.f;
+  }
+  const float* src = u + (int64_t)row * T;
+  const float* wr = w + (int64_t)ch * To;
+  const bool vec = (T & 3) == 0;
+  float st[2] = {0.f, 0.f};
+  for (int to = threadIdx.x; to < To; to += 256) {
+    const uint64_t oi = (uint64_t)row * To + to;
+    float d = 0.f;
+#pragma unroll
+    for (int j = 0; j < NCT; ++j)
+      if (j < NC) d += wr[(int64_t)j * NF + to] * dl[j];
+    dp[oi] = d;
+    const float go = d * (1.0f / P) * dropout_mult_row(drop_p, seed, mask, oi, (uint64_t)row);
+    pool_bwd_window_sums<P>(src, to, T, vec, go, sc, sh, mean, invstd, st);
+  }
+  block_sum_256<2>(st, smem);
   if (threadIdx.x < 2) part[(int64_t)b * 2 * CH + threadIdx.x * CH + ch] = st[0];
 }
 
@@ -598,3 +689,43 @@
   return pool_bwd_apply_launch("eav_bn_elu_pool_bwd_eval", dp, u, bn, nullptr, du, part, B, CH, T, P, drop_p, seed, mask,
                                seed_dev, stream);
 }
+
+
+extern "C" int eav_bn_elu_pool_fwd_dense(const float* in, const float* bn, float* out, const float* w, float* part_logit,
+                                         int B, int CH, int T, int P, int NC, float drop_p, uint64_t seed,
+                                         const uint8_t* mask, const uint64_t* seed_dev, void* stream) {
+  EAV_REQUIRE(in && bn && out && w && part_logit && B > 0 && CH > 0 && T >= P, "eav_bn_elu_pool_fwd_dense: bad arguments");
+  EAV_REQUIRE(P == 8, "eav_bn_elu_pool_fwd_dense: pool %d is not 8", P);
+  EAV_REQUIRE(NC > 0 && NC <= EAV_HEAD_NCMAX, "eav_bn_elu_pool_fwd_dense: classes %d outside [1, %d]", NC, EAV_HEAD_NCMAX);
+  EAV_REQUIRE(drop_p > -1.f && drop_p < 1.f, "eav_bn_elu_pool_fwd_dense: dropout %f outside (-1,1)", drop_p);
+  if (NC <= 8)
+    hipLaunchKernelGGL((pool_fwd_dense_kernel<8, 8>), dim3(B * CH), dim3(256), 0, (hipStream_t)stream, in, bn, out, CH, T,
+                       drop_p, seed, mask, seed_dev, w, part_logit, NC);
+  else
+    hipLaunchKernelGGL((pool_fwd_dense_kernel<8, EAV_HEAD_NCMAX>), dim3(B * CH), dim3(256), 0, (hipStream_t)stream, in, bn, out,
+                       CH, T, drop_p, seed, mask, seed_dev, w, part_logit, NC);
+  EAV_CHECK_LAUNCH("eav_bn_elu_pool_fwd_dense");
+  return EAV_OK;
+}
+
+extern "C" int eav_bn_elu_pool_bwd_reduce_dense(const float* dprobs, const float* probs, const float* feat, const float* w,
+                                                float* dw, float* dbias, float* dp, const float* u, const float* bn,
+                                                float* part, int B, int CH, int T, int P, int NC, float drop_p,
+                                                uint64_t seed, const uint8_t* mask, const uint64_t* seed_dev,
+                                                void* stream) {
+  EAV_REQUIRE(dprobs && feat && w && dw && dbias && dp && u && bn && part && B > 0 && CH > 0 && T >= P,
+              "eav_bn_elu_pool_bwd_reduce_dense: bad arguments");
+  EAV_REQUIRE(P == 8, "eav_bn_elu_pool_bwd_reduce_dense: pool %d is not 8", P);
+  EAV_REQUIRE(NC > 0 && NC <= EAV_HEAD_NCMAX, "eav_bn_elu_pool_bwd_reduce_dense: classes %d outside [1, %d]", NC, EAV_HEAD_NCMAX);
+  EAV_REQUIRE((size_t)B * NC * sizeof(float) <= 40 * 1024, "eav_bn_elu_pool_bwd_reduce_dense: batch %d too large", B);
+  const int nwb = cdiv(CH * (T / P), 64), nct = NC <= 8 ? 8 : EAV_HEAD_NCMAX;
+  const size_t lds = (size_t)(B * NC + 4 * nct * 64) * sizeof(float);
+  if (NC <= 8)
+    hipLaunchKernelGGL((pool_bwd_reduce_dense_kernel<8, 8>), dim3(nwb + B * CH), dim3(256), lds, (hipStream_t)stream, dprobs,
+                       probs, feat, w, dw, dbias, dp, u, bn, part, B, CH, T, NC, nwb, drop_p, seed, mask, seed_dev);
+  else
+    hipLaunchKernelGGL((pool_bwd_reduce_dense_kernel<8, EAV_HEAD_NCMAX>), dim3(nwb + B * CH), dim3(256), lds, (hipStream_t)stream,
+                       dprobs, probs, feat, w, dw, dbias, dp, u, bn, part, B, CH, T, NC, nwb, drop_p, seed, mask, seed_dev);
+  EAV_CHECK_LAUNCH("eav_bn_elu_pool_bwd_reduce_dense");
+  return EAV_OK;
+}
diff --git a/eav_amd/csrc/eegnet_conv64_fft.hip b/eav_amd/csrc/eegnet_conv64_fft.hip
--- a/eav_amd/csrc/eegnet_conv64_fft.hip
+++ b/eav_amd/csrc/eegnet_conv64_fft.hip
@@ -349,29 +349,43 @@
 
 }
 
+namespace {
+constexpr int64_t TBL = (int64_t)64 * 128 * 128;
+int64_t spectra_floats(const Geo& g) { return (int64_t)64 * g.ncolp * 128; }
+int64_t off_pp(const Geo& g) { return 2 * TBL + 3 * spectra_floats(g); }
+int64_t off_acc(const Geo& g) { return off_pp(g) + WCH * TBL; }
+int64_t off_d(const Geo& g) { return off_acc(g) + (int64_t)64 * 64 * 64 * 2; }
+}
+
 extern "C" int64_t eav_conv64_fft_ws_floats(int B, int T) {
   const Geo g = geometry(B, T, 7);
-  return (int64_t)2 * 64 * 128 * 128 + (int64_t)3 * 64 * g.ncolp * 128 + (int64_t)WCH * 64 * 128 * 128 +
-         (int64_t)64 * 64 * 64 * 2;
+  return off_d(g) + spectra_floats(g);
 }
 
 extern "C" int eav_conv64_fft_nparts(int B, int T) {
   const Geo g = geometry(B, T, 7);
   return pack_grid(g) * 4;
+}
+
+extern "C" int eav_conv64_fft_spectra(const float* w, float* ws, void* stream) {
+  EAV_REQUIRE(w && ws, "eav_conv64_fft_spectra: bad arguments");
+  hipLaunchKernelGGL(c64_spectra_kernel, dim3(NCH, 2), dim3(64), 0, (hipStream_t)stream, w, ws, 0);
+  EAV_CHECK_LAUNCH("eav_conv64_fft_spectra");
+  return EAV_OK;
 }
 
 extern "C" int eav_conv64_fft_fwd(const float* in, const float* w, float* out, float* stat_part, float* ws, int B, int T,
                                   int bwd, void* stream) {
   EAV_REQUIRE(in && w && out && ws && B > 0 && T > 0, "eav_conv64_fft_fwd: bad arguments");
   EAV_REQUIRE(((uintptr_t)ws & 15) == 0, "eav_conv64_fft_fwd: the workspace must be 16-byte aligned");
+  EAV_REQUIRE(bwd >= 0 && bwd <= 3, "eav_conv64_fft_fwd: bwd must be 0, 1, 2 or 3");
+  const bool prepared = bwd >= 2;
+  bwd = bwd == 2 ? 1 : bwd == 3 ? 0 : bwd;
   const Geo g = geometry(B, T, bwd ? 8 : 7);
-  EAV_REQUIRE(bwd >= 0 && bwd <= 2, "eav_conv64_fft_fwd: bwd must be 0, 1 or 2");
   hipStream_t st = (hipStream_t)stream;
-  float* Bm = ws + (bwd ? (int64_t)64 * 128 * 128 : 0);
-  const bool prepared = bwd == 2;
-  if (bwd == 2) bwd = 1;
-  float* Z = ws + (int64_t)2 * 64 * 128 * 128 + (bwd ? (int64_t)64 * g.ncolp * 128 : 0);
-  float* Y = ws + (int64_t)2 * 64 * 128 * 128 + (int64_t)2 * 64 * g.ncolp * 128;
+  float* Bm = ws + (bwd ? TBL : 0);
+  float* Z = ws + 2 * TBL + (bwd ? spectra_floats(g) : 0);
+  float* Y = ws + 2 * TBL + 2 * spectra_floats(g);
   if (!prepared) {
     hipLaunchKernelGGL(c64_spectra_kernel, dim3(NCH, bwd ? 1 : 2), dim3(64), 0, st, w, Bm, bwd);
     EAV_CHECK_LAUNCH("eav_conv64_fft_fwd(spectra)");
@@ -389,10 +403,10 @@
   EAV_REQUIRE(du && dW && ws && B > 0 && T > 0, "eav_conv64_fft_wgrad: bad arguments");
   const Geo g = geometry(B, T, 7);
   hipStream_t st = (hipStream_t)stream;
-  float* Z = ws + (int64_t)2 * 64 * 128 * 128;
-  float* D = Z + (int64_t)2 * 64 * g.ncolp * 128;
-  float* Pp = Z + (int64_t)3 * 64 * g.ncolp * 128;
-  float* Acc = Pp + (int64_t)WCH * 64 * 128 * 128;
+  float* Z = ws + 2 * TBL;
+  float* D = ws + off_d(g);
+  float* Pp = ws + off_pp(g);
+  float* Acc = ws + off_acc(g);
   hipLaunchKernelGGL(c64_pack_fft_kernel, dim3(pack_grid(g)), dim3(256), 0, st, du, D, g, 1);
   EAV_CHECK_LAUNCH("eav_conv64_fft_wgrad(fft)");
   const int cpc = g.ncolp / WCH;
diff --git a/eav_amd/csrc/head_optim.hip b/eav_amd/csrc/head_optim.hip
--- a/eav_amd/csrc/head_optim.hip
+++ b/eav_amd/csrc/head_optim.hip
@@ -1,9 +1,10 @@
 #include "eav_common.h"
+#include "dense_head.h"
 #include "../../include/eav_hip.h"
 
 namespace {
 
-constexpr int NCMAX = 16;
+constexpr int NCMAX = EAV_HEAD_NCMAX;
 
 __global__ __launch_bounds__(1024) void dense_softmax_fwd_kernel(const float* __restrict__ in,
                                                                  const float* __restrict__ w,
@@ -89,61 +90,39 @@
                                                                 const float* __restrict__ w, float* __restrict__ dw,
                                                                 float* __restrict__ dbias, float* __restrict__ din,
                                                                 int B, int NF, int NC) {
-  extern __shared__ float dl[];
-  float* pw = dl + B * NC;
-  for (int idx = threadIdx.x; idx < B * NC; idx += blockDim.x) {
-    const int b = idx / NC;
-    float v = dout[idx];
-    if (probs) {
-      float dot = 0.f;
-      for (int j = 0; j < NC; ++j) dot += dout[b * NC + j] * probs[b * NC + j];
-      v = probs[idx] * (v - dot);
-    }
-    dl[idx] = v;
+  extern __shared__ float smem[];
+  dense_bwd_body<NCMAX>(dout, probs, in, w, dw, dbias, din, B, NF, NC, blockIdx.x, smem);
+}
+
+__global__ __launch_bounds__(256) void head_finish_kernel(const float* __restrict__ part, const float* __restrict__ bias,
+                                                          float* __restrict__ logits, float* __restrict__ probs, int B,
+                                                          int CH, int NC, float* __restrict__ w_a, int rows_a, int cols_a,
+                                                          float* __restrict__ w_b, int cols_b, float maxnorm) {
+  __shared__ float red[4 * NCMAX];
+  int r = blockIdx.x;
+  if (r >= B) {
+    r -= B;
+    if (r < rows_a) renorm_row_body(w_a + (int64_t)r * cols_a, cols_a, maxnorm, red);
+    else renorm_row_body(w_b + (int64_t)(r - rows_a) * cols_b, cols_b, maxnorm, red);
+    return;
+  }
+  const int lane = threadIdx.x & 63, wave = threadIdx.x >> 6;
+  for (int j = wave; j < NC; j += 4) {
+    float s = 0.f;
+    for (int ch = lane; ch < CH; ch += 64) s += part[((int64_t)r * CH + ch) * NC + j];
+    s = wave_sum(s);
+    if (lane == 0) red[j] = s + bias[j];
   }
   __syncthreads();
-  if (blockIdx.x == 0 && threadIdx.x < NC) {
-    float s = 0.f;
-    for (int b = 0; b < B; ++b) s += dl[b * NC + threadIdx.x];
-    dbias[threadIdx.x] = s;
-  }
-  const int f = threadIdx.x & 63, slice = threadIdx.x >> 6;
-  const int i = blockIdx.x * 64 + f;
-  const bool live = i < NF;
-  float wv[NCMAX], acc[NCMAX];
-#pragma unroll
-  for (int j = 0; j < NCMAX; ++j) {
-    wv[j] = (live && j < NC) ? w[(int64_t)j * NF + i] : 0.f;
-    acc[j] = 0.f;
-  }
-  for (int b0 = slice; b0 < B; b0 += 32) {
-    float v[8];
-#pragma unroll
-    for (int u = 0; u < 8; ++u) v[u] = (live && b0 + 4 * u < B) ? in[(int64_t)(b0 + 4 * u) * NF + i] : 0.f;
-#pragma unroll
-    for (int u = 0; u < 8; ++u) {
-      const int b = b0 + 4 * u;
-      if (b < B) {
-        float d = 0.f;
-#pragma unroll
-        for (int j = 0; j < NCMAX; ++j)
-          if (j < NC) {
-            const float g = dl[b * NC + j];
-            acc[j] += g * v[u];
-            d += wv[j] * g;
-          }
-        if (din && live) din[(int64_t)b * NF + i] = d;
-      }
-    }
-  }
-#pragma unroll
-  for (int j = 0; j < NCMAX; ++j) pw[(slice * NCMAX + j) * 64 + f] = acc[j];
-  __syncthreads();
-  if (slice == 0 && live) {
-#pragma unroll
-    for (int j = 0; j < NCMAX; ++j)
-      if (j < NC)
-        dw[(int64_t)j * NF + i] = (pw[j * 64 + f] + pw[(NCMAX + j) * 64 + f]) + (pw[(2 * NCMAX + j) * 64 + f] + pw[(3 * NCMAX + j) * 64 + f]);
+  if (threadIdx.x == 0) {
+    float mx = red[0];
+    for (int j = 1; j < NC; ++j) mx = fmaxf(mx, red[j]);
+    float e[NCMAX], s = 0.f;
+    for (int j = 0; j < NC; ++j) { e[j] = expf(red[j] - mx); s += e[j]; }
+    for (int j = 0; j < NC; ++j) {
+      if (logits) logits[r * NC + j] = red[j];
+      if (probs) probs[r * NC + j] = e[j] / s;
+    }
   }
 }
 
@@ -214,6 +193,8 @@
 
 }
 
+extern "C" int eav_dense_max_classes(void) { return NCMAX; }
+
 extern "C" int eav_dense_softmax_fwd(const float* in, const float* w, const float* bias, float* logits, float* probs,
                                      int B, int NF, int NC, void* stream) {
   EAV_REQUIRE(in && w && bias && (logits || probs) && B > 0 && NF > 0 && NC > 0 && NC <= NCMAX,
@@ -233,6 +214,20 @@
                      (B * NC + 4 * NCMAX * 64) * sizeof(float), (hipStream_t)stream, dout, probs, in, w, dw, dbias, din, B,
                      NF, NC);
   EAV_CHECK_LAUNCH("eav_dense_softmax_bwd");
+  return EAV_OK;
+}
+
+extern "C" int eav_dense_finish_softmax_renorm(const float* part, const float* bias, float* logits, float* probs, int B,
+                                               int CH, int NC, float* w_a, int rows_a, int cols_a, float* w_b, int rows_b,
+                                               int cols_b, float maxnorm, void* stream) {
+  EAV_REQUIRE(part && bias && (logits || probs) && B > 0 && CH > 0 && NC > 0 && NC <= NCMAX,
+              "eav_dense_finish_softmax_renorm: bad arguments (classes <= %d)", NCMAX);
+  EAV_REQUIRE(!w_a || (rows_a > 0 && cols_a > 0 && w_b && rows_b > 0 && cols_b > 0),
+              "eav_dense_finish_softmax_renorm: bad max-norm arguments");
+  if (!w_a) rows_a = rows_b = 0;
+  hipLaunchKernelGGL(head_finish_kernel, dim3(B + rows_a + rows_b), dim3(256), 0, (hipStream_t)stream, part, bias, logits,
+                     probs, B, CH, NC, w_a, rows_a, cols_a, w_b, cols_b, maxnorm);
+  EAV_CHECK_LAUNCH("eav_dense_finish_softmax_renorm");
   return EAV_OK;
 }
 
diff --git a/eav_amd/eegnet.py b/eav_amd/eegnet.py
--- a/eav_amd/eegnet.py
+++ b/eav_amd/eegnet.py
@@ -44,6 +44,7 @@
         self.part_c3 = f(max(self.np_c3, self.np_c3_fft), 128)
         self.c64_ws = None
         self.part_pb = f(B, 128)
+        self.part_lg = f(B * 64, 16)
         self.part_dst = f(B * nchunk, 16)
         self.part_dw2 = f(B * nchunk, 64 * C)
         self.np_fw = _lib.plain("eav_eegnet_fir_wgrad_nparts", B, C, S)
@@ -141,6 +142,9 @@
         self._infer = False
         self._step_begin = None
         self.fused_eval = False
+        self.overlap = True
+        self._side = None
+        self.fuse_head = True
 
     def _use_fft(self):
         if self.fir_algo not in ("auto", "fft", "mfma"):
@@ -197,6 +201,25 @@
 
     def _forward_output(self):
         return self._saved[-1].detach()
+
+    def _overlapped(self):
+        return bool(self.overlap) and _lib.TRACE is None and self.kernel_events is None
+
+    def _head_fused(self, T2):
+        return bool(self.fuse_head) and T2 % 4 == 0 and self.nb_classes <= _lib.plain("eav_dense_max_classes")
+
+    def _fork(self, dev):
+        index = dev.index if dev.index is not None else torch.cuda.current_device()
+        if self._side is None or self._side.device.index != index:
+            self._side = torch.cuda.Stream(device=index)
+        ready = torch.cuda.Event()
+        ready.record()
+        self._side.wait_event(ready)
+        return self._side
+
+    @staticmethod
+    def _join(side):
+        torch.cuda.current_stream().wait_stream(side)
 
     def forward_batch(self, xs, ys, idx, optimizer):
         if not (xs.is_cuda and xs.dim() == 4 and xs.is_contiguous()):
@@ -252,6 +275,9 @@
             L("eav_step_begin", *counters, *begin, st)
         elif cnt is not None or training:
             L("eav_counter_inc4", *counters, st)
+        if self._use_conv_fft(B) and ws.c64_ws is None:
+            ws.c64_ws = torch.zeros(_lib.plain("eav_conv64_fft_ws_floats", B, ws.T2), dtype=torch.float32,
+                                    device=ws.y1.device)
         np_fir = ws.np_fir
         infer = self.fused_eval and self._infer and not training and S % 4 == 0
         if infer:
@@ -285,19 +311,22 @@
                 L("eav_bn_elu_pool_fwd", P(ws.z), P(ws.bn2), P(ws.p2), B, 64, S, 4, drop, seed1, m1, cnt, st)
         np_c3 = ws.np_c3
         if self._use_conv_fft(B):
-            if ws.c64_ws is None:
-                ws.c64_ws = torch.zeros(_lib.plain("eav_conv64_fft_ws_floats", B, ws.T2), dtype=torch.float32,
-                                        device=ws.y1.device)
             np_c3 = ws.np_c3_fft
             L("eav_conv64_fft_fwd", P(ws.p2), w3, P(ws.u3), P(ws.part_c3), P(ws.c64_ws), B, ws.T2, 0, st)
         else:
             L("eav_conv64_fwd", P(ws.p2), P(ws.wTf), P(ws.u3), P(ws.part_c3), B, ws.T2, 7, st)
         bnfin(ws.part_c3, np_c3, 64, B * ws.T2, g3w, g3b, bn3, ws.bn3)
-        L("eav_bn_elu_pool_fwd", P(ws.u3), P(ws.bn3), P(ws.p3), B, 64, ws.T2, 8, drop, seed2, m2, cnt, st)
         probs = torch.empty(B, nb, dtype=torch.float32, device=x.device)
-        L("eav_dense_softmax_fwd", P(ws.p3), wd, bd, None, P(probs), B, ws.NF, nb, st)
-        if self.apply_max_norm:
-            L("eav_renorm_rows2", w2, 64, C, wd, nb, ws.NF, self.norm_rate, st)
+        if self._head_fused(ws.T2):
+            L("eav_bn_elu_pool_fwd_dense", P(ws.u3), P(ws.bn3), P(ws.p3), wd, P(ws.part_lg), B, 64, ws.T2, 8, nb, drop, seed2,
+              m2, cnt, st)
+            mn = (w2, 64, C, wd, nb, ws.NF) if self.apply_max_norm else (None, 0, 0, None, 0, 0)
+            L("eav_dense_finish_softmax_renorm", P(ws.part_lg), bd, None, P(probs), B, 64, nb, *mn, self.norm_rate, st)
+        else:
+            L("eav_bn_elu_pool_fwd", P(ws.u3), P(ws.bn3), P(ws.p3), B, 64, ws.T2, 8, drop, seed2, m2, cnt, st)
+            L("eav_dense_softmax_fwd", P(ws.p3), wd, bd, None, P(probs), B, ws.NF, nb, st)
+            if self.apply_max_norm:
+                L("eav_renorm_rows2", w2, 64, C, wd, nb, ws.NF, self.norm_rate, st)
         self._saved = (self._token, x, training, drop, seed1, seed2, masks, cnt, ws, probs)
         return self._token
 
@@ -401,11 +430,17 @@
         m2 = P(masks[1]) if masks is not None else None
         tr = int(training)
 
-        L("eav_dense_softmax_bwd", P(dprobs), P(probs), P(ws.p3), wd, P(g["dense.weight"]), P(g["dense.bias"]),
-          P(ws.dp3), B, NF, nb, st)
         b3 = P(ws.bn3)
+        if training and self._head_fused(T2):
+            L("eav_bn_elu_pool_bwd_reduce_dense", P(dprobs), P(probs), P(ws.p3), wd, P(g["dense.weight"]), P(g["dense.bias"]),
+              P(ws.dp3), P(ws.u3), b3, P(ws.part_pb), B, 64, T2, 8, nb, drop, seed2, m2, cnt, st)
+        else:
+            L("eav_dense_softmax_bwd", P(dprobs), P(probs), P(ws.p3), wd, P(g["dense.weight"]), P(g["dense.bias"]),
+              P(ws.dp3), B, NF, nb, st)
+            if training:
+                L("eav_bn_elu_pool_bwd_reduce", P(ws.dp3), P(ws.u3), b3, P(ws.part_pb), B, 64, T2, 8, drop, seed2, m2, cnt,
+                  st)
         if training:
-            L("eav_bn_elu_pool_bwd_reduce", P(ws.dp3), P(ws.u3), b3, P(ws.part_pb), B, 64, T2, 8, drop, seed2, m2, cnt, st)
             L("eav_bn_bwd_finalize", P(ws.part_pb), B, 64, float(B * T2), tr, P(g["separableBN.weight"]),
               P(g["separableBN.bias"]), b3 + 4 * 256, b3 + 4 * 320, st)
             L("eav_bn_elu_pool_bwd_apply", P(ws.dp3), P(ws.u3), b3, b3 + 4 * 256, P(ws.du3), B, 64, T2, 8, drop, seed2, m2,
@@ -415,15 +450,18 @@
               cnt, st)
             L("eav_bn_bwd_finalize", P(ws.part_pb), B, 64, float(B * T2), tr, P(g["separableBN.weight"]),
               P(g["separableBN.bias"]), b3 + 4 * 256, b3 + 4 * 320, st)
+        side = self._fork(ws.du3.device) if self._overlapped() and self._use_conv_fft(B) else None
+        wst = st if side is None else side.cuda_stream
+        WL = L if side is None else _lib.call
         if self._use_conv_fft(B):
             L("eav_conv64_fft_fwd", P(ws.du3), P(self.separableConv.weight), P(ws.dp2), None, P(ws.c64_ws), B, T2, 2, st)
         else:
             L("eav_conv64_fwd", P(ws.du3), P(ws.wTb), P(ws.dp2), None, B, T2, 8, st)
         if self._use_conv_fft(B):
-            L("eav_conv64_fft_wgrad", P(ws.du3), P(g["separableConv.weight"]), P(ws.c64_ws), B, T2, st)
-        else:
-            L("eav_conv64_wgrad", P(ws.du3), P(ws.p2), P(ws.part_cw), B, T2, 7, st)
-            L("eav_reduce_partials", P(ws.part_cw), ws.np_cw, 65536, 65536, 1.0, P(g["separableConv.weight"]), st)
+            WL("eav_conv64_fft_wgrad", P(ws.du3), P(g["separableConv.weight"]), P(ws.c64_ws), B, T2, wst)
+        else:
+            WL("eav_conv64_wgrad", P(ws.du3), P(ws.p2), P(ws.part_cw), B, T2, 7, wst)
+            WL("eav_reduce_partials", P(ws.part_cw), ws.np_cw, 65536, 65536, 1.0, P(g["separableConv.weight"]), wst)
         b2 = P(ws.bn2)
         b1 = P(ws.bn1)
         if training:
@@ -456,6 +494,8 @@
                 L("eav_eegnet_fir_wgrad", P(x), P(ws.y1) if training else None, P(ws.g1), b1, P(ws.part_fw), B, C, S, K,
                   st)
             L("eav_reduce_partials", P(ws.part_fw), ws.np_fw, 8 * K, 8 * K, 1.0, P(g["firstConv.weight"]), st)
+        if side is not None:
+            self._join(side)
         named = dict(self.named_parameters())
         return [g[k].view(named[k].shape) if named[k].requires_grad else None for k in _PARAM_ORDER]
 
diff --git a/include/eav_hip.h b/include/eav_hip.h
--- a/include/eav_hip.h
+++ b/include/eav_hip.h
@@ -73,6 +73,13 @@
 int eav_bn_elu_pool_bwd_eval(const float* dp, const float* u, const float* bn, float* du, float* part , int B,
                              int CH, int T, int P, float drop_p, uint64_t seed, const uint8_t* mask,
                              const uint64_t* seed_dev, void* stream);
+int eav_bn_elu_pool_fwd_dense(const float* in, const float* bn, float* out, const float* w, float* part_logit, int B,
+                              int CH, int T, int P, int NC, float drop_p, uint64_t seed, const uint8_t* mask,
+                              const uint64_t* seed_dev, void* stream);
+int eav_bn_elu_pool_bwd_reduce_dense(const float* dprobs, const float* probs, const float* feat, const float* w, float* dw,
+                                     float* dbias, float* dp, const float* u, const float* bn, float* part ,
+                                     int B, int CH, int T, int P, int NC, float drop_p, uint64_t seed, const uint8_t* mask,
+                                     const uint64_t* seed_dev, void* stream);
 
 int eav_conv64_prep_weights(const float* w , float* wT_fwd , float* wT_bwd, void* stream);
 int eav_eegnet_step_prologue(const float* w, float* wT_fwd, float* wT_bwd, int64_t* c0, int64_t* c1, int64_t* c2,
@@ -85,6 +92,7 @@
 int eav_conv64_fft_nparts(int B, int T);
 int eav_conv64_fft_fwd(const float* in, const float* w, float* out, float* stat_part, float* ws, int B, int T, int bwd,
                        void* stream);
+int eav_conv64_fft_spectra(const float* w, float* ws, void* stream);
 int eav_conv64_fft_wgrad(const float* du, float* dW, float* ws, int B, int T, void* stream);
 int eav_conv64_wgrad_nparts(int B, int T);
 int eav_conv64_wgrad(const float* du, const float* in, float* part, int B, int T, int padl, void* stream);
@@ -113,10 +121,14 @@
 int eav_dwt_bwd(const float* dd3, const float* a, const float* wdw, float* da, float* w_part, int B, int C2, int T,
                 int K2, void* stream);
 
+int eav_dense_max_classes(void);
 int eav_dense_softmax_fwd(const float* in, const float* w, const float* bias, float* logits, float* probs, int B,
                           int NF, int NC, void* stream);
 int eav_dense_softmax_bwd(const float* dout, const float* probs, const float* in, const float* w, float* dw,
                           float* dbias, float* din, int B, int NF, int NC, void* stream);
+int eav_dense_finish_softmax_renorm(const float* part, const float* bias, float* logits, float* probs, int B, int CH,
+                                    int NC, float* w_a, int rows_a, int cols_a, float* w_b, int rows_b, int cols_b,
+                                    float maxnorm, void* stream);
 int eav_ce_fwd_bwd(const float* in, const int64_t* y, float* loss, float* din, int* ncorrect, int* bad_label, int B,
                    int NC, void* stream);
 int eav_scale_by_scalar(float* v, const float* scalar, int64_t n, void* stream);
```
